# diku-kmc/kleenexlang

Hardware: AMD Instinct MI355X
Metric: input GB/s + % HBM-read roofline, apache_log.kex over 10 GiB synthetic log (higher is better)
Workload: dtype u8

## Files before the change

kleenexlang_amd/csrc/engine/kx_dfkernels.inc:

```

struct DfDev {
  const uint32_t* img; uint32_t words;
  uint32_t off_pool, deadh, esch, starth, K, C;
  const uint16_t* start_of_state;
  uint32_t orig_c4, hshift;
  uint32_t short_consts, debug;
  uint32_t nstates;
  uint32_t J;
  uint32_t wide;
  const uint4* sl_fmap;
  const uint32_t* sl_back; const uint8_t* sl_nleaves; const uint8_t* sl_fin_leaf; const uint8_t* sl_cls;
  const uint32_t* sl_pcoff; const uint8_t* sl_pcpool; const uint32_t* sl_pend; const uint32_t* sl_defoff; const uint32_t* sl_defpc; const uint16_t* sl_q;
  uint32_t sl_Lm, sl_npc, sl_on;
};
constexpr uint32_t DFREC_HOLE = 0xFFFF0000u, DF_HOLE_MAX = 4096, DF_HOLE_FIRST = 1024, DF_SL_LEAVES = 32;
struct __attribute__((aligned(16))) DfRec { uint32_t hh, cum, info, kc; };
constexpr uint32_t DFREC_OWN = 0x80000000u;

struct DfLds {
  const uint8_t* base; uint32_t csh;
  __device__ __forceinline__ uint32_t c8(uint32_t byte) const { return (uint32_t)base[byte] << csh; }
  __device__ __forceinline__ uint2 ent(uint32_t a) const { return *reinterpret_cast<const uint2*>(base + a); }
};
__device__ __forceinline__ DfLds df_stage(const DfDev& D, uint32_t* smem) {
  for (uint32_t i = threadIdx.x; i < D.words; i += blockDim.x) smem[i] = D.img[i];
  __syncthreads();
  return DfLds{reinterpret_cast<const uint8_t*>(smem), D.wide ? 3u : 0u};
}

__device__ __forceinline__ void df_run_piece(const uint32_t (&w)[16], uint32_t& h, uint32_t& mid, uint32_t& lenA, uint32_t& len, const DfLds& L) {
  uint32_t c[8], cn[8], sum = 0;
  static_for<0, 8>([&](auto ic) { constexpr int i = decltype(ic)::value; c[i] = L.c8(BYTE_AT_DEP(w, i, h)); });
  static_for<0, PIECE / 8>([&](auto gc) {
    constexpr int g = decltype(gc)::value;
    if constexpr (g + 1 < PIECE / 8)
      static_for<0, 8>([&](auto ic) { constexpr int i = decltype(ic)::value; cn[i] = L.c8(BYTE_AT_DEP(w, 8 * (g + 1) + i, h)); });
    static_for<0, 8>([&](auto ic) {
      constexpr int i = decltype(ic)::value;
      const uint2 e = L.ent(h + c[i]);
      h = e.x & 0xFFFFu; sum += e.y >> 24; tie(h, sum);
    });
    if constexpr (g == HALF / 8 - 1) { mid = h; lenA = sum; }
    if constexpr (g + 1 < PIECE / 8)
      static_for<0, 8>([&](auto ic) { constexpr int i = decltype(ic)::value; c[i] = cn[i]; });
  });
  len = sum;
}

__device__ __forceinline__ uint64_t df_own_start(uint32_t j, uint64_t n, uint64_t seg, int first_known, const uint64_t* __restrict__ seg_pos,
                                                 const uint16_t* __restrict__ seg_state, const DfDev& D) {
  if (j == 0 && first_known) return 0;
  const uint64_t p = seg_pos[j];
  if (p == UNSYNC) return UNSYNC;
  const uint32_t q = (((uint32_t)seg_state[j] << D.hshift) - OFF_FWD) / D.orig_c4;
  if (q >= D.nstates || D.start_of_state[q] == 0xFFFFu) return UNSYNC;
  const uint64_t b = (p + D.K + D.J + 63) & ~63ull;
  const uint64_t lim = ((uint64_t)j + 1) * seg < n ? ((uint64_t)j + 1) * seg : n;
  return b < lim ? b : UNSYNC;
}

struct DfSlowIO {
  const uint8_t* in; uint64_t n, a, end; uint32_t h0, last, is_last;
  uint32_t h_behind; uint32_t* side; uint32_t side_cap; Flags* flags; const uint8_t* lds; uint32_t clsh; uint8_t* lmap; uint32_t max_steps;
  uint32_t base, nd, h_next; uint64_t e_out;
};
__device__ __noinline__ int df_slow_resolve(DfSlowIO& io, const DfDev& D) {
  const uint8_t* __restrict__ in = io.in;
  const uint64_t n = io.n, a = io.a, end = io.end;
  const uint32_t h0 = io.h0;
  const bool last = io.last != 0, is_last = io.is_last != 0;
  uint32_t* side = io.side; const uint32_t side_cap = io.side_cap; Flags* flags = io.flags;
  if (!D.sl_on || !side) return 1;
  const uint32_t C = D.C, Lm = D.sl_Lm, K = D.K, NONE = D.sl_npc << 1;
  const uint32_t i0 = (h0 - 256u) / (C * 8u);
  uint32_t q = D.sl_q[i0];
  const uint32_t nd = D.sl_defoff[i0 + 1] - D.sl_defoff[i0];
  const uint64_t hard = a + io.max_steps < n ? a + io.max_steps : n;
  const uint32_t need = nd + K + (uint32_t)(hard - a) + 64u;
  const uint32_t base = atomicAdd(&flags->side_used, need);
  if ((uint64_t)base + need > side_cap) return 1;
  uint32_t* const E = side + base;
  uint32_t* const R = E + nd + K;
  for (uint32_t d = 0; d < nd; ++d) E[d] = 0x80000000u | (D.sl_defpc[D.sl_defoff[i0] + d] << 1);
  uint8_t *M = io.lmap, *M2 = io.lmap + 32;
  uint16_t qb[DF_HOLE_MAX / 64 + 2];
  uint32_t nl = D.sl_nleaves[q];
  for (uint32_t l = 0; l < DF_SL_LEAVES; ++l) M[l] = (uint8_t)l;
  uint64_t t = a, anchor = a, prev = a, inw = 0;
  auto back_to = [&](uint64_t from, uint64_t to, uint32_t leaf) {
    uint64_t u = to;
    while (u > from) {
      const uint32_t cnt = u - from < 8 ? (uint32_t)(u - from) : 8u;
      uint32_t rr[8];
#pragma unroll
      for (uint32_t k2 = 0; k2 < 8; ++k2) rr[k2] = k2 < cnt ? R[u - 1 - k2 - a] : 0u;
#pragma unroll
      for (uint32_t k2 = 0; k2 < 8; ++k2) if (k2 < cnt) {
        const uint32_t e = D.sl_back[(size_t)rr[k2] * Lm + leaf];
        R[u - 1 - k2 - a] = ((e >> 8) & 1u) | ((e >> 9) << 1);
        leaf = e & 0xFFu;
      }
      u -= cnt;
    }
    return leaf;
  };
  bool pend_done = false;
  auto anchor_known = [&](uint32_t leaf) {
    if (anchor == a) { for (uint32_t jj = 0; jj < K; ++jj) E[nd + jj] = D.sl_pend[((size_t)i0 * K + jj) * Lm + leaf]; pend_done = true; }
    else back_to(prev, anchor, leaf);
  };
  auto agree_at = [&](uint64_t tt, uint32_t nlv) -> bool {
    uint32_t l0 = 0, l1 = 0, l2 = 0, l3 = 0, nlive = 0;
    for (uint32_t l = 0; l < nlv; ++l) if (M[l] != 0xFFu) {
      if (nlive == 4) return false;
      if (nlive == 0) l0 = l1 = l2 = l3 = l; else if (nlive == 1) l1 = l; else if (nlive == 2) l2 = l; else l3 = l;
      ++nlive;
    }
    if (nlive == 0) return false;
    const uint32_t lv[1] = {l0};
    if (nlive > 1) {
      uint32_t cur[4] = {l0, l1, l2, l3};
      for (uint64_t u = tt; u-- > prev;) {
        const uint32_t* row = D.sl_back + (size_t)R[u - a] * Lm;
        const uint32_t e0 = row[cur[0]], e1 = row[cur[1]], e2 = row[cur[2]], e3 = row[cur[3]];
        if ((e0 >> 8) != (e1 >> 8) || (e0 >> 8) != (e2 >> 8) || (e0 >> 8) != (e3 >> 8)) return false;
        cur[0] = e0 & 0xFFu; cur[1] = e1 & 0xFFu; cur[2] = e2 & 0xFFu; cur[3] = e3 & 0xFFu;
      }
      if (!pend_done)
        for (uint32_t jj = 0; jj < K; ++jj) {
          const uint32_t* pr = D.sl_pend + ((size_t)i0 * K + jj) * Lm;
          if (pr[cur[0]] != pr[cur[1]] || pr[cur[0]] != pr[cur[2]] || pr[cur[0]] != pr[cur[3]]) return false;
        }
    }
    const uint32_t la = back_to(prev, tt, lv[0]);
    if (!pend_done) { for (uint32_t jj = 0; jj < K; ++jj) E[nd + jj] = D.sl_pend[((size_t)i0 * K + jj) * Lm + la]; pend_done = true; }
    return true;
  };
  uint64_t e_out = 0; int mode = 0;
  for (;;) {
    if (((t - a) & 63u) == 0) qb[(t - a) >> 6] = (uint16_t)q;
    if (t >= hard) {
      if (t != n) return 3;
      if (!is_last) return 1;
      if (D.sl_fin_leaf[q] == 0xFFu) { atomicMin(&flags->fail_pos, (unsigned long long)n); return 2; }
      const uint32_t fl = D.sl_fin_leaf[q];
      const uint32_t la = back_to(anchor, n, fl);
      anchor_known(la);
      if (last) { mode = 3; e_out = n; } else { mode = 2; e_out = end; }
      break;
    }
    if ((t & 7u) == 0 || t == a) {
      const uint64_t a8 = t & ~7ull;
      if (a8 + 8 <= n) { const uint2 w8 = *reinterpret_cast<const uint2*>(in + a8); inw = (uint64_t)w8.x | ((uint64_t)w8.y << 32); }
      else { inw = 0; for (uint64_t i = a8; i < n; ++i) inw |= (uint64_t)in[i] << (8 * (i - a8)); }
    }
    const uint32_t c = (uint32_t)io.lds[(uint32_t)(inw >> (8 * (t & 7u))) & 0xFFu] >> io.clsh;
    const uint4* fm = D.sl_fmap + ((size_t)q * C + c) * 3;
    const uint4 f0 = fm[0], f1 = fm[1], f2v = fm[2];
    const uint32_t nq = f0.x & 0xFFFFu;
    if (nq == 0xFFFFu) { atomicMin(&flags->fail_pos, (unsigned long long)t); return 2; }
    const uint32_t r = f0.y;
    R[t - a] = r;
    const uint32_t nnl = f0.x >> 16;
    uint32_t v = 0xFFu; bool same = true;
    const uint32_t par[8] = {f1.x, f1.y, f1.z, f1.w, f2v.x, f2v.y, f2v.z, f2v.w};
#pragma unroll
    for (uint32_t l = 0; l < DF_SL_LEAVES; ++l) {
      const uint32_t pl = (par[l >> 2] >> (8 * (l & 3u))) & 0xFFu;
      const uint32_t x = l >= nnl || pl == 0xFFu ? 0xFFu : M[pl];
      if (l < nnl) M2[l] = (uint8_t)x;
      if (x != 0xFFu) { if (v == 0xFFu) v = x; else same = same && x == v; }
    }
    { uint8_t* tmp = M; M = M2; M2 = tmp; }
    q = nq; nl = nnl; ++t;
    if ((!same || v == 0xFFu) && ((t - a) & 63u) == 0 && t + PIECE <= end && D.start_of_state[q] != 0xFFFFu && agree_at(t, nl)) {
      qb[(t - a) >> 6] = (uint16_t)q;
      mode = 1; e_out = t;
      break;
    }
    if (!same || v == 0xFFu) continue;
    anchor_known(v);
    const uint64_t decided = anchor;
    prev = anchor; anchor = t;
    for (uint32_t l = 0; l < DF_SL_LEAVES; ++l) M[l] = (uint8_t)l;
    const uint64_t e = decided & ~63ull;
    if (e > a && e + PIECE <= end && D.start_of_state[qb[(e - a) >> 6]] != 0xFFFFu) { mode = 1; e_out = e; break; }
    if (!last && decided + K >= end) { mode = 2; e_out = end; break; }
  }
  (void)nl;
  uint32_t h_next = h0;
  if (mode == 1) h_next = D.start_of_state[qb[(e_out - a) >> 6]];
  if (mode == 3) {
    if (D.start_of_state[q] == 0xFFFFu) return 1;
    h_next = D.start_of_state[q];
  }
  if (mode == 2) {
    for (uint64_t u = end - K; u < end; ++u) if (u >= a) R[u - a] = NONE; else E[nd + K - (a - u)] = NONE;
    const uint32_t ix = (io.h_behind - 256u) / (C * 8u);
    uint32_t due = D.sl_defoff[ix + 1] - D.sl_defoff[ix];
    for (uint32_t idx = nd + K + (uint32_t)(end - K - a); due && idx-- > 0;) {
      const uint32_t pc = (E[idx] >> 1) & 0x3FFFFFFFu;
      if (pc < D.sl_npc && D.sl_pcoff[pc + 1] > D.sl_pcoff[pc]) { E[idx] = (E[idx] & 0x80000001u) | NONE; --due; }
    }
    if (due) return 1;
  }
  io.base = base; io.nd = nd; io.h_next = h_next; io.e_out = e_out;
  return 0;
}

template <int BT, uint32_t DF_STAGE, int MINW, bool SLOW>
__global__ __launch_bounds__(BT, MINW) void k_dforward(const uint8_t* __restrict__ in, uint64_t n, uint64_t seg, uint32_t nseg, int first_known,
                           const uint64_t* __restrict__ seg_pos, const uint16_t* __restrict__ seg_state,
                           DfRec* __restrict__ rec, uint32_t* __restrict__ own, uint32_t* __restrict__ spill, Flags* flags,
                           uint32_t* __restrict__ side, uint32_t side_cap, int is_last, DfDev D) {
  extern __shared__ __attribute__((aligned(16))) uint32_t smem[];
  DfLds L = df_stage(D, smem);
  uint4* lrec = reinterpret_cast<uint4*>(smem + ((D.words + 3) & ~3u)) + (size_t)threadIdx.x * DF_STAGE;
  const uint32_t k = blockIdx.x * blockDim.x + threadIdx.x;
  const uint32_t lane = threadIdx.x & 63;
  const uint64_t B = k < nseg ? df_own_start(k, n, seg, first_known, seg_pos, seg_state, D) : UNSYNC;
  bool alive = B != UNSYNC;
  const uint32_t dead = D.deadh, esc = D.esch;
  auto warm = [&](uint32_t jj, uint64_t Bj) -> uint32_t {
    if (jj == 0 && first_known) return D.starth;
    uint32_t hw = D.start_of_state[(((uint32_t)seg_state[jj] << D.hshift) - OFF_FWD) / D.orig_c4];
    for (uint64_t pw = seg_pos[jj]; pw < Bj;) {
      const uint2 v = *reinterpret_cast<const uint2*>(in + (pw & ~7ull));
      const uint64_t x = (uint64_t)v.x | ((uint64_t)v.y << 32);
      for (uint32_t b = (uint32_t)pw & 7u; b < 8u && pw < Bj; ++b, ++pw) hw = L.ent(hw + L.c8((uint32_t)(x >> (8 * b)) & 0xFFu)).x & 0xFFFFu;
    }
    if (hw == esc && jj == k) atomicAdd(&flags->warm_esc, 1u);
    return hw == esc || hw == dead ? 0xFFFFFFFFu : hw;
  };
  uint32_t h = dead, h_behind = 0;
  if (alive) { h = warm(k, B); if (h == 0xFFFFFFFFu) { alive = false; h = dead; } }
  uint32_t j = k + 1;
  uint64_t end = n;
  if (alive) for (; j < nseg; ++j) {
    const uint64_t b = df_own_start(j, n, seg, first_known, seg_pos, seg_state, D);
    if (b == UNSYNC) continue;
    h_behind = warm(j, b);
    if (h_behind != 0xFFFFFFFFu) { end = b; break; }
  }
  const bool last = alive && j >= nseg;
  uint64_t pos = alive ? B : 0;
  if (alive) atomicMin(&flags->df_first_own, (unsigned long long)B);
  bool failed = !alive;
  if (!alive) { end = 0; pos = 0; }
  uint32_t m = (uint32_t)(pos / seg), cum = 0, flag = DFREC_OWN;
  uint64_t block_end = ((uint64_t)m + 1) * seg;
  auto fail_in = [&](uint32_t h0, uint64_t p0, uint32_t plen) -> int {
    uint32_t hh = h0;
    for (uint32_t t = 0; t < plen; ++t) {
      const uint32_t nh = L.ent(hh + L.c8(in[p0 + t])).x & 0xFFFFu;
      if (nh == dead) { atomicMin(&flags->fail_pos, (unsigned long long)(p0 + t)); failed = true; return 1; }
      if (nh == esc) return 2;
      hh = nh;
    }
    failed = true;
    return 1;
  };
  uint32_t nst = 0; uint64_t gfirst = 0;
  auto flush_group = [&]() {
    uint4* dst = reinterpret_cast<uint4*>(rec + gfirst);
    for (uint32_t i = 0; i < nst; ++i) dst[i] = lrec[(gfirst + i) & (DF_STAGE - 1)];
    nst = 0;
  };
  const bool coop = !(D.debug & 256u);
  bool in_trip = false;
  auto stage_rec = [&](uint64_t pc, uint4 r) {
    if (nst == 0) gfirst = pc;
    lrec[pc & (DF_STAGE - 1)] = r; ++nst;
    if (!in_trip && (pc & (DF_STAGE - 1)) == DF_STAGE - 1) flush_group();
  };
  uint4* const lrec_wave = reinterpret_cast<uint4*>(smem + ((D.words + 3) & ~3u)) + (size_t)(threadIdx.x & ~63u) * DF_STAGE;
  auto coop_flush = [&]() {
    const bool full = nst == DF_STAGE && (gfirst & (DF_STAGE - 1)) == 0;
    const uint32_t glo = (uint32_t)gfirst, ghi = (uint32_t)(gfirst >> 32) | (full ? 0u : 0x80000000u);
    const uint32_t team = lane / DF_STAGE * DF_STAGE, r = lane % DF_STAGE;
    static_for<0, (int)DF_STAGE>([&](auto ic) {
      constexpr uint32_t i = decltype(ic)::value;
      const uint32_t slo = (uint32_t)__shfl((int)glo, (int)(team + i)), shi = (uint32_t)__shfl((int)ghi, (int)(team + i));
      if (!(shi & 0x80000000u)) {
        const uint64_t g = ((uint64_t)shi << 32) | slo;
        reinterpret_cast<uint4*>(rec + g)[r] = lrec_wave[(size_t)(team + i) * DF_STAGE + r];
      }
    });
    if (full) nst = 0;
  };
  auto cross = [&]() { if (pos == block_end) { (flag ? own : spill)[m] = cum; cum = 0; flag = 0; ++m; block_end += seg; } };
  uint32_t kc_sum = 0, kc_max = 0, kc_n = 0;
  auto slow = [&](const uint64_t a, const uint32_t h0) -> int {
    flush_group();
    DfSlowIO io{in, n, a, end, h0, last ? 1u : 0u, (uint32_t)is_last, h_behind, side, side_cap, flags, L.base, D.wide ? 0u : 3u, reinterpret_cast<uint8_t*>(lrec), DF_HOLE_FIRST, 0, 0, 0, 0};
    {
      int rc = df_slow_resolve(io, D);
      if (rc == 3) { io.max_steps = DF_HOLE_MAX; rc = df_slow_resolve(io, D); }
      if (rc) return rc == 3 ? 1 : rc;
    }
    const uint32_t base = io.base, nd = io.nd, K = D.K;
    const uint64_t e_out = io.e_out;
    const uint32_t* const E = side + base;
    const uint64_t pend = (e_out + 63) & ~63ull;
    uint32_t idx = 0;
    for (uint64_t pp = a; pp < pend; pp += PIECE) {
      cross();
      const bool first = pp == a;
      const uint32_t steps = (uint32_t)((e_out - pp) < PIECE ? e_out - pp : PIECE);
      const uint32_t cnt = first ? nd + K + steps : steps;
      uint32_t len = 0;
      for (uint32_t x = 0; x < cnt; ++x) {
        const uint32_t ee = E[idx + x], pc = (ee >> 1) & 0x3FFFFFFFu;
        len += (ee & 1u) + (pc < D.sl_npc ? D.sl_pcoff[pc + 1] - D.sl_pcoff[pc] : 0u);
      }
      if (len > 0xFFFFu) return 1;
      rec[pp >> 6] = DfRec{base + idx, cum, len | flag, DFREC_HOLE | (first ? 0x8000u : 0u) | cnt};
      idx += cnt; cum += len; pos = pp + steps;
    }
    h = io.h_next;
    atomicAdd(&flags->slow_steps, (uint32_t)(e_out - a));
    return 0;
  };
  bool need_slow = false;
  auto run_slow = [&]() {
    need_slow = false;
    int r = 1;
    if constexpr (SLOW) r = slow(pos, h);
    if (r) { if (r == 1) atomicAdd(&flags->df_esc, 1u); failed = true; }
  };
  auto do_piece = [&](const uint32_t (&w)[16]) -> bool {
    cross();
    const uint32_t h0 = h;
    uint32_t mid, sumA, sum = 0;
    if (D.wide) piece_dfrun1w(w, h, mid, sumA, sum); else piece_dfrun1(w, h, mid, sumA, sum);
    if (h == dead || h == esc) {
      if (fail_in(h0, pos, PIECE) == 2) { need_slow = true; h = h0; }
      return false;
    }
    const uint32_t kA = (sumA & 0xFFu) >> 2, kB = (sum & 0xFFu) >> 2;
    kc_sum += kA + kB; kc_max = kA + kB > kc_max ? kA + kB : kc_max; ++kc_n;
    stage_rec(pos >> 6, make_uint4(h0 | (mid << 16), cum, (sumA >> 8) | flag, kA | (kB << 8)));
    cum += sum >> 8; pos += PIECE;
    return true;
  };
  auto single_piece = [&]() {
    uint32_t w[16];
    load_piece(in, n, pos, w);
    do_piece(w);
  };
  for (;;) {
  if (need_slow) run_slow();
  while (!failed && !need_slow && pos + PIECE <= end && (pos & (8 * PIECE - 1))) single_piece();
  for (;;) {
    const bool can = !failed && !need_slow && pos + 8 * PIECE <= end && !(pos & (8 * PIECE - 1));
    if (!__any(can) || __any(need_slow)) break;
    uint32_t line[8];
    {
      const uint32_t mine = can ? (uint32_t)(pos >> 7) : 0xFFFFFFFFu;
      static_for<0, 8>([&](auto ic) { constexpr int i = decltype(ic)::value; line[i] = __shfl(mine, (int)((lane & ~7u) + i)); });
    }
    auto issue = [&](uint32_t k2, uint4 (&dst)[8]) {
      static_for<0, 8>([&](auto ic) {
        constexpr int i = decltype(ic)::value;
        const uint64_t ln = line[i] != 0xFFFFFFFFu ? line[i] : 0u;
        dst[i] = *reinterpret_cast<const uint4*>(in + ((ln + k2) << 7) + (lane & 7u) * 16);
      });
    };
    uint4 v[8];
    issue(0, v);
    bool died = false;
    in_trip = coop;
#pragma nounroll
    for (uint32_t k2 = 0; k2 < 4; ++k2) {
      transpose8(v, lane);
      uint32_t wa[16], wb[16];
      static_for<0, 8>([&](auto ic) {
        constexpr int w = decltype(ic)::value;
        uint32_t (&dst)[16] = w < 4 ? wa : wb;
        dst[4 * (w & 3)] = v[w].x; dst[4 * (w & 3) + 1] = v[w].y; dst[4 * (w & 3) + 2] = v[w].z; dst[4 * (w & 3) + 3] = v[w].w;
      });
      bool go = can && !died;
      if (go && !do_piece(wa)) { died = true; go = false; }
      if (k2 < 3) issue(k2 + 1, v);
      if (go && !do_piece(wb)) died = true;
      if (coop && ((k2 + 1) * 2) % DF_STAGE == 0) coop_flush();
    }
    in_trip = false;
  }
  if (!__any(!failed && (need_slow || pos + 8 * PIECE <= end))) break;
  }
  if (!alive) return;
  for (;;) {
  if (need_slow) run_slow();
  while (!failed && !need_slow && pos + PIECE <= end) single_piece();
  if (need_slow) continue;
  if (!failed && pos < end) {
    cross();
    const uint32_t plen = (uint32_t)(end - pos), h0 = h;
    uint32_t mid = h, lenA = 0, len = 0, kA = 0, kc = 0;
    for (uint32_t t = 0; t < plen; ++t) {
      if (t == HALF) { mid = h; lenA = len; kA = kc; }
      const uint2 e = L.ent(h + L.c8(in[pos + t]));
      h = e.x & 0xFFFFu; len += e.y >> 24; kc += (e.y >> 23) & 1u;
    }
    if (plen <= HALF) { mid = h; lenA = len; kA = kc; }
    if (h == dead || h == esc) {
      if (fail_in(h0, pos, plen) == 2) { h = h0; need_slow = true; continue; }
    }
    else { stage_rec(pos >> 6, make_uint4(h0 | (mid << 16), cum, lenA | flag, kA | ((kc - kA) << 8))); cum += len; pos = end; }
  }
  break;
  }
  flush_group();
  if (failed) return;
  (flag ? own : spill)[m] = cum;
  if (last) flags->end_state = h;
  if (kc_n) { if ((k & 15u) == 0) { atomicAdd(&flags->emit_ksum, kc_sum); atomicAdd(&flags->emit_kn, kc_n); } atomicMax(&flags->emit_kmax, kc_max); }
}

__global__ void k_dhead(const uint8_t* __restrict__ in, uint64_t n, uint64_t seg, uint64_t head_len, uint32_t h,
                        DfRec* __restrict__ rec, uint32_t* __restrict__ own, uint32_t* __restrict__ spill, Flags* flags, DfDev D) {
  extern __shared__ __attribute__((aligned(16))) uint32_t smem[];
  DfLds L = df_stage(D, smem);
  if (blockIdx.x || threadIdx.x) return;
  const uint32_t dead = D.deadh, esc = D.esch;
  uint32_t m = 0, cum = 0;
  uint64_t block_end = seg;
  for (uint64_t pos = 0; pos < head_len;) {
    if (pos == block_end) { spill[m] = cum; cum = 0; ++m; block_end += seg; }
    const uint32_t plen = (uint32_t)(head_len - pos < PIECE ? head_len - pos : PIECE);
    const uint32_t h0 = h;
    uint32_t mid = h, lenA = 0, len = 0, kA = 0, kc = 0;
    for (uint32_t t = 0; t < plen; ++t) {
      if (t == HALF) { mid = h; lenA = len; kA = kc; }
      const uint2 e = L.ent(h + L.c8(in[pos + t]));
      const uint32_t nh = e.x & 0xFFFFu;
      if (nh == dead) { atomicMin(&flags->fail_pos, (unsigned long long)(pos + t)); return; }
      if (nh == esc) { flags->df_esc = 1; return; }
      h = nh; len += e.y >> 24; kc += (e.y >> 23) & 1u;
    }
    if (plen <= HALF) { mid = h; lenA = len; kA = kc; }
    if (kc > 0) atomicMax(&flags->emit_kmax, kc);
    rec[pos >> 6] = DfRec{h0 | (mid << 16), cum, lenA, kA | ((kc - kA) << 8)};
    cum += len; pos += plen;
  }
  spill[m] = cum;
  if (head_len == n) flags->end_state = h;
}

__global__ void k_dlen(uint32_t nblk, const uint32_t* __restrict__ own, const uint32_t* __restrict__ spill, uint32_t* __restrict__ len,
                       unsigned long long* __restrict__ wsum) {
  __shared__ unsigned long long red[1024];
  const uint32_t m = blockIdx.x * blockDim.x + threadIdx.x;
  uint32_t mylen = 0;
  if (m < nblk) { mylen = own[m] + spill[m]; len[m] = mylen; }
  red[threadIdx.x] = mylen;
  __syncthreads();
  for (uint32_t s = blockDim.x >> 1; s > 0; s >>= 1) {
    if (threadIdx.x < s) red[threadIdx.x] += red[threadIdx.x + s];
    __syncthreads();
  }
  if (threadIdx.x == 0) wsum[blockIdx.x] = red[0];
}

template <bool GENERAL>
__global__ void k_dmap(const uint8_t* __restrict__ in, uint64_t n, uint32_t q_in, uint64_t cap, uint8_t* __restrict__ map_out,
                       uint32_t* __restrict__ status, DevTables T) {
  extern __shared__ __attribute__((aligned(16))) uint32_t smem[];
  Lds L = stage_tables<GENERAL>(T, smem);
  if (blockIdx.x || threadIdx.x) return;
  __shared__ uint8_t M[2][256];
  const uint32_t C = T.nclasses;
  uint32_t h = (OFF_FWD + q_in * C * 4) >> T.hshift, cur = 0;
  uint32_t nl = T.nleaves[q_in];
  for (uint32_t l = 0; l < nl; ++l) M[0][l] = (uint8_t)l;
  uint64_t pos = 0;
  bool constant = nl == 1, dead = false;
  while (pos < n && pos < cap && !constant && !dead) {
    const uint64_t a8 = pos & ~7ull;
    uint64_t x = 0;
    if (a8 + 8 <= n) { const uint2 v = *reinterpret_cast<const uint2*>(in + a8); x = (uint64_t)v.x | ((uint64_t)v.y << 32); }
    else for (uint64_t i = a8; i < n; ++i) x |= (uint64_t)in[i] << (8 * (i - a8));
    for (uint32_t b = (uint32_t)pos & 7u; b < 8u && pos < n && pos < cap && !constant; ++b, ++pos) {
      const uint32_t e = L.next(h, (uint32_t)(x >> (8 * b)) & 0xFFu);
      const uint32_t nh = e & 0xFFFFu;
      if (nh == T.deadh) { dead = true; break; }
      const uint32_t row = L.ra(e >> 16);
      const uint32_t nq = ((nh << T.hshift) - OFF_FWD) / (C * 4);
      const uint32_t nnl = T.nleaves[nq];
      constant = true;
      for (uint32_t l = 0; l < nnl; ++l) {
        const uint32_t p = (L.w(row + l * 4) >> 2) & 0xFFu;
        M[cur ^ 1][l] = M[cur][p < nl ? p : 0];
        constant = constant && M[cur ^ 1][l] == M[cur ^ 1][0];
      }
      cur ^= 1; h = nh; nl = nnl;
    }
  }
  for (uint32_t l = 0; l < 256; ++l) map_out[l] = constant ? M[cur][0] : l < nl ? M[cur][l] : 0;
  *status = constant ? 1u : pos >= n ? 2u : 0u;
}

template <int S>
__device__ __forceinline__ uint32_t df_byte_src(const uint32_t (&w)[16], uint32_t wp) {
  if constexpr (S >= 0) return w[S >> 2] >> ((S & 3) * 8);
  else return wp >> ((4 + S) * 8);
}

__device__ __forceinline__ void put_bytes3(uint32_t r, uint32_t d, uint32_t v) {
  uint32_t t; unsigned long long sv;
  asm volatile("s_mov_b64 %[sv], exec\n"
               "v_cmpx_lt_u32_e32 vcc, 0, %[r]\n"
               "ds_write_b8 %[d], %[v]\n"
               "v_cmpx_lt_u32_e32 vcc, 1, %[r]\n"
               "v_lshrrev_b32 %[t], 8, %[v]\n"
               "ds_write_b8 %[d], %[t] offset:1\n"
               "v_cmpx_lt_u32_e32 vcc, 2, %[r]\n"
               "ds_write_b8_d16_hi %[d], %[v] offset:2\n"
               "s_mov_b64 exec, %[sv]\n"
               : [t] "=&v"(t), [sv] "=&s"(sv) : [r] "v"(r), [d] "v"(d), [v] "v"(v) : "vcc", "memory");
}
__device__ __forceinline__ void put_dwords4(uint32_t m, uint32_t d, const uint32_t (&w)[4]) {
  unsigned long long sv;
  asm volatile("s_mov_b64 %[sv], exec\n"
               "v_cmpx_lt_u32_e32 vcc, 0, %[m]\n"
               "ds_write_b32 %[d], %[w0]\n"
               "v_cmpx_lt_u32_e32 vcc, 1, %[m]\n"
               "ds_write_b32 %[d], %[w1] offset:4\n"
               "v_cmpx_lt_u32_e32 vcc, 2, %[m]\n"
               "ds_write_b32 %[d], %[w2] offset:8\n"
               "v_cmpx_lt_u32_e32 vcc, 3, %[m]\n"
               "ds_write_b32 %[d], %[w3] offset:12\n"
               "s_mov_b64 exec, %[sv]\n"
               : [sv] "=&s"(sv) : [m] "v"(m), [d] "v"(d), [w0] "v"(w[0]), [w1] "v"(w[1]), [w2] "v"(w[2]), [w3] "v"(w[3]) : "vcc", "memory");
}

#ifndef KX_PRIO_CONSTANTS
#define KX_PRIO_CONSTANTS 2
#endif
#ifndef KX_PRIO_FLUSH
#define KX_PRIO_FLUSH 1
#endif
constexpr int HALF_BYTES = HALF;

template <int CONSTS>
__device__ __forceinline__ void df_step_gen(uint32_t& h, uint32_t byte_now, uint32_t byte_out, uint64_t& o, uint8_t* __restrict__ dst,
                                            const DfLds& L, const DfDev& D) {
  const uint2 e = L.ent(h + L.c8(byte_now));
  h = e.x & 0xFFFFu;
  const uint32_t cp = E_COPY(e.y), dl = e.y >> 24;
  if (cp) dst[o] = (uint8_t)byte_out;
  if (dl > cp) { const uint32_t src = D.off_pool + (E_AID(e.y) << 4); for (uint32_t i = 0; i < dl - cp; ++i) dst[o + cp + i] = L.base[src + i]; }
  o += dl;
}

template <int WAVES, int K, bool HALF = false>
__global__ __launch_bounds__(WAVES * 64) void k_demit(const uint8_t* __restrict__ in, uint64_t n, uint64_t blk, uint64_t blk_inv,
                                                      uint64_t npieces_total, const DfRec* __restrict__ rec,
                                                      const uint32_t* __restrict__ spill, const unsigned long long* __restrict__ off,
                                                      Flags* __restrict__ flags, uint32_t stgb, uint32_t jbytes, uint32_t maxcnt,
                                                      uint8_t* __restrict__ out, const uint32_t* __restrict__ side, DfDev D) {
  extern __shared__ __attribute__((aligned(16))) uint32_t smem[];
  DfLds L = df_stage(D, smem);
  if ((uint32_t)(uintptr_t)smem != 0u) __builtin_trap();
  constexpr int NB = HALF ? HALF_BYTES : PIECE, NW = NB / 4;
  const uint32_t wave = threadIdx.x >> 6, lane = threadIdx.x & 63;
  const uint32_t stga = ((D.words + 3) & ~3u) * 4 + wave * (stgb + 16 + jbytes);
  uint8_t* stg = (uint8_t*)smem + stga;
  const uint32_t jarea = stga + stgb + 16;
  const uint64_t nunits = HALF ? npieces_total * 2 : npieces_total;
  const uint64_t nwi = (nunits + 63) / 64;
  const uint64_t oend_all = flags->total_len;
  const uint64_t one_piece_blocks = (uint64_t)__builtin_amdgcn_readfirstlane(blk == (uint64_t)PIECE ? 1 : 0);
  struct Operands { uint32_t w[NW]; uint32_t wp; uint4 r; uint64_t off0; uint32_t sp0; uint4 r1; uint64_t off1; uint32_t sp1; };
  auto request = [&](uint64_t it_, Operands& o) {
    if (it_ >= nwi) return;
    const uint64_t u = it_ * 64 + lane;
    const bool ok = u < nunits;
    const uint64_t pc = HALF ? u >> 1 : u;
    const uint64_t ustart = ok ? (HALF ? pc * PIECE + (u & 1) * HALF_BYTES : pc * PIECE) : n;
    if constexpr (HALF) {
      if (ustart + HALF_BYTES <= n) {
        const uint4* p = reinterpret_cast<const uint4*>(in + ustart);
        const uint4 v0 = p[0], v1 = p[1];
        o.w[0] = v0.x; o.w[1] = v0.y; o.w[2] = v0.z; o.w[3] = v0.w; o.w[4] = v1.x; o.w[5] = v1.y; o.w[6] = v1.z; o.w[7] = v1.w;
      } else {
#pragma unroll
        for (int i = 0; i < NW; ++i) {
          uint32_t x = 0;
#pragma unroll
          for (int bb = 0; bb < 4; ++bb) { const uint64_t a = ustart + 4 * i + bb; if (a < n) x |= (uint32_t)in[a] << (8 * bb); }
          o.w[i] = x;
        }
      }
    } else load_piece(in, n, ustart, o.w);
    o.wp = *reinterpret_cast<const uint32_t*>(ok && ustart >= 4 ? in + ustart - 4 : reinterpret_cast<const uint8_t*>(D.img));
    const uint64_t pc0 = ok ? pc : 0;
    const uint64_t m0 = __umul64hi(pc0, blk_inv) + pc0 * one_piece_blocks;
    o.r = *reinterpret_cast<const uint4*>(rec + pc0);
    o.off0 = off[m0]; o.sp0 = spill[m0];
    {
      const uint64_t pc1 = pc0 + 1 < npieces_total ? pc0 + 1 : pc0, m1 = __umul64hi(pc1, blk_inv) + pc1 * one_piece_blocks;
      o.r1 = *reinterpret_cast<const uint4*>(rec + pc1); o.off1 = off[m1]; o.sp1 = spill[m1];
    }
  };
  Operands nx, cur;
  request((uint64_t)blockIdx.x * WAVES + wave, nx);
  cur = nx;
  unsigned long long tk[6] = {0, 0, 0, 0, 0, 0};
  auto stamp = [&]() -> unsigned long long {
    if (!(D.debug & 64u)) return 0ull;
    asm volatile("s_waitcnt vmcnt(0) lgkmcnt(0)" ::: "memory");
    return __builtin_amdgcn_s_memtime();
  };
  for (uint64_t it = (uint64_t)blockIdx.x * WAVES + wave; it < nwi; it += (uint64_t)gridDim.x * WAVES) {
    const unsigned long long t0 = stamp();
    const uint64_t unit = it * 64 + lane;
    const bool valid = unit < nunits;
    const uint64_t piece = HALF ? unit >> 1 : unit;
    const uint32_t half = HALF ? (uint32_t)unit & 1u : 0u;
    const uint64_t ustart = piece * PIECE + half * HALF_BYTES;
    const int plen = valid ? (int)(n <= ustart ? 0 : n - ustart < (uint64_t)NB ? n - ustart : NB) : 0;
    uint32_t w[NW];
#pragma unroll
    for (int i = 0; i < NW; ++i) w[i] = cur.w[i];
    const uint32_t wp = cur.wp, lenA = cur.r.z & 0xFFFFu;
    const uint32_t kA = HALF ? (half ? (cur.r.w >> 8) & 0xFFu : cur.r.w & 0xFFu) : cur.r.w & 0xFFu, kB = HALF ? 0u : (cur.r.w >> 8) & 0xFFu;
    const uint32_t hh = HALF ? (half ? cur.r.x >> 16 : cur.r.x & 0xFFFFu) : cur.r.x;
    uint64_t ostart = valid ? cur.off0 + cur.r.y + ((cur.r.z & DFREC_OWN) ? cur.sp0 : 0u) + (half ? lenA : 0u) : oend_all;
    const uint64_t onext63 = piece + 1 < npieces_total ? cur.off1 + cur.r1.y + ((cur.r1.z & DFREC_OWN) ? cur.sp1 : 0u) : oend_all;
    uint64_t oend;
    {
      const uint32_t lo = (uint32_t)__builtin_amdgcn_update_dpp(0, (int)(uint32_t)ostart, 0x130, 0xF, 0xF, false);
      const uint32_t hi = (uint32_t)__builtin_amdgcn_update_dpp(0, (int)(uint32_t)(ostart >> 32), 0x130, 0xF, 0xF, false);
      oend = lane == 63 ? onext63 : ((uint64_t)hi << 32) | lo;
      if (!valid) oend = oend_all;
    }
    const unsigned long long vmask = __ballot(valid);
    const uint32_t nvalid = (uint32_t)__popcll(vmask);
    uint32_t first = 0;
    bool taken = false;
    unsigned long long t2 = stamp();
    tk[0] += t2 - t0;
    if (valid && (cur.r.w & DFREC_HOLE) == DFREC_HOLE && half == 0) {
      const uint32_t cntE = cur.r.w & 0x7FFFu;
      uint64_t u = (cur.r.w & 0x8000u) ? piece * PIECE - K : piece * PIECE, o = ostart;
      for (uint32_t x = 0; x < cntE; ++x) {
        const uint32_t ee = side[cur.r.x + x], pc = (ee >> 1) & 0x3FFFFFFFu;
        if (ee & 1u) out[o++] = in[u];
        if (pc < D.sl_npc) for (uint32_t b = D.sl_pcoff[pc]; b < D.sl_pcoff[pc + 1]; ++b) out[o++] = D.sl_pcpool[b];
        if (!(ee >> 31)) ++u;
      }
    }
    while (first < nvalid) {
      if (first == 0) request(it + (uint64_t)gridDim.x * WAVES, nx);
      const uint64_t gs = wave_read64(ostart, first);
      const uint64_t abase = gs & ~15ull;
      const bool hole = (cur.r.w & DFREC_HOLE) == DFREC_HOLE;
      const bool fits = valid && lane >= first && (oend - abase) <= (uint64_t)stgb && plen == NB && !hole;
      const unsigned long long fm = __ballot(fits) >> first;
      uint32_t cnt = fm == ~0ull ? 64u - first : (uint32_t)__builtin_ctzll(~fm);
      if (cnt > maxcnt) cnt = maxcnt;
      if (cnt == 0) {
        if (lane == first && hole) {
        } else
        if (lane == first) {
          uint32_t h = hh & 0xFFFFu;
          uint64_t o = ostart;
          for (int t = 0; t < plen; ++t) {
            const int ts = t - K;
            const uint32_t bn = (w[t >> 2] >> ((t & 3) * 8)) & 0xFFu;
            const uint32_t bo_ = ts >= 0 ? (w[ts >> 2] >> ((ts & 3) * 8)) & 0xFFu : (wp >> ((4 + ts) * 8)) & 0xFFu;
            df_step_gen<0>(h, bn, bo_, o, out, L, D);
          }
        }
        first += 1;
        continue;
      }
      const uint32_t lastl = first + cnt - 1;
      const bool active = lane >= first && lane <= lastl;
      const uint32_t o0 = stga + (uint32_t)(ostart - abase);
      const bool inplace = jbytes == 0;
      const uint32_t need = active ? (kA + kB) * 4u : 0u;
      const uint32_t incl = wave_scan_incl(need);
      const uint32_t jtotal = (uint32_t)__builtin_amdgcn_readlane((int)incl, 63);
      const bool jfit = !inplace && jtotal <= jbytes;
      const unsigned long long t3 = stamp();
      tk[2] += t3 - t2;
      if (active && jfit) {
        uint32_t oA = o0, pA = jarea + incl - need;
        if constexpr (HALF) {
          if (D.wide) { if constexpr (K == 1) piece_dfwalk1cw_k1(w, wp, hh & 0xFFFFu, oA, pA); else piece_dfwalk1cw_k2(w, wp, hh & 0xFFFFu, oA, pA); }
          else { if constexpr (K == 1) piece_dfwalk1c_k1(w, wp, hh & 0xFFFFu, oA, pA); else piece_dfwalk1c_k2(w, wp, hh & 0xFFFFu, oA, pA); }
        } else {
          uint32_t oB = o0 + lenA, pB = pA + 4u * kA;
          if (D.wide) {
            if constexpr (K == 1) piece_dfwalk2cw_k1(w, wp, hh & 0xFFFFu, oA, hh >> 16, oB, pA, pB);
            else piece_dfwalk2cw_k2(w, wp, hh & 0xFFFFu, oA, hh >> 16, oB, pA, pB);
          } else {
            if constexpr (K == 1) piece_dfwalk2c_k1(w, wp, hh & 0xFFFFu, oA, hh >> 16, oB, pA, pB);
            else piece_dfwalk2c_k2(w, wp, hh & 0xFFFFu, oA, hh >> 16, oB, pA, pB);
          }
        }
      }
      uint32_t njobs = jfit ? jtotal >> 2 : 0u;
      if (!jfit) {
        if (!inplace && lane == first) atomicAdd(&flags->emit_ovf, cnt);
        if (active) {
          for (int ch = 0; ch < (HALF ? 1 : 2); ++ch) {
            uint32_t h = ch ? hh >> 16 : hh & 0xFFFFu;
            uint64_t o = (uint64_t)(o0 - stga) + (ch ? lenA : 0u);
            for (int t = ch * HALF_BYTES; t < (ch + 1) * HALF_BYTES; ++t) {
              const int ts = t - K;
              const uint32_t bn = (w[t >> 2] >> ((t & 3) * 8)) & 0xFFu;
              const uint32_t bo_ = ts >= 0 ? (w[ts >> 2] >> ((ts & 3) * 8)) & 0xFFu : (wp >> ((4 + ts) * 8)) & 0xFFu;
              df_step_gen<1>(h, bn, bo_, o, stg, L, D);
            }
          }
        }
      }
      wave_lds_fence();
      const unsigned long long t4 = stamp();
      tk[3] += t4 - t3;
      __builtin_amdgcn_s_setprio(KX_PRIO_CONSTANTS);
      for (uint32_t j0 = 0; j0 < njobs; j0 += 64) {
        const uint32_t j = j0 + lane;
        uint32_t l = 0, d = 0, off0 = 0;
        if (j < njobs) {
          const uint32_t jw = *reinterpret_cast<const uint32_t*>((const uint8_t*)smem + jarea + 4 * j);
          const uint32_t e = *reinterpret_cast<const uint32_t*>(L.base + (jw & 0xFFFFu) + 4);
          const uint32_t cp = E_COPY(e);
          l = (e >> 24) - cp;
          d = stga + (((jw >> 16) - stga) & 0xFFFFu) + cp;
          off0 = D.off_pool + (E_AID(e) << 4);
        }
        const uint32_t tob = (0u - d) & 3u, nh = l < tob ? l : tob, rem = l - nh;
        const uint32_t src = off0 + nh * ((l + 15u) & ~15u), d1 = d + nh;
        const uint32_t v0 = *reinterpret_cast<const uint32_t*>(L.base + off0);
        uint4 wv = *reinterpret_cast<const uint4*>(L.base + src);
        put_bytes3(nh, d, v0);
        for (uint32_t base = 0;; base += 16) {
          const uint32_t left = rem > base ? rem - base : 0u, m = left >> 2 < 4u ? left >> 2 : 4u;
          const uint32_t w4[4] = {wv.x, wv.y, wv.z, wv.w};
          put_dwords4(m, d1 + base, w4);
          const uint32_t nt = left < 16u ? left & 3u : 0u;
          const uint32_t tw = m == 0 ? wv.x : m == 1 ? wv.y : m == 2 ? wv.z : wv.w;
          put_bytes3(nt, d1 + base + 4u * m, tw);
          if (!__any(rem > base + 16u)) break;
          wv = *reinterpret_cast<const uint4*>(L.base + src + base + 16u);
        }
      }
      wave_lds_fence();
      __builtin_amdgcn_s_setprio(KX_PRIO_FLUSH);
      const unsigned long long t5 = stamp();
      tk[4] += t5 - t4;
      if (lastl + 1 >= nvalid) { cur = nx; taken = true; }
      const uint64_t ge = wave_read64(oend, lastl);
      const uint64_t fs = (gs + 15) & ~15ull, fe = ge & ~15ull;
      if (fs >= fe) {
        for (uint64_t x = gs + lane; x < ge; x += 64) out[x] = stg[x - abase];
      } else {
        if (gs + lane < fs) out[gs + lane] = stg[gs + lane - abase];
        if (fe + lane < ge) out[fe + lane] = stg[fe + lane - abase];
        for (uint64_t x = fs + (uint64_t)lane * 16; x < fe; x += 1024)
          *reinterpret_cast<uint4*>(out + x) = *reinterpret_cast<const uint4*>(stg + (x - abase));
      }
      wave_lds_fence();
      __builtin_amdgcn_s_setprio(0);
      t2 = stamp();
      tk[5] += t2 - t5;
      first = lastl + 1;
    }
    if (!taken) cur = nx;
  }
  if ((D.debug & 64u) && lane == 0)
    for (int i = 0; i < 6; ++i) atomicAdd(&flags->dbg[i], tk[i]);
}
```

kleenexlang_amd/csrc/engine/kx_engine.hip:

```cpp
#include <hip/hip_runtime.h>
#include <fcntl.h>
#include <sys/stat.h>
#include <unistd.h>

#include <cerrno>
#include <condition_variable>
#include <cstdint>
#include <algorithm>
#include <deque>
#include <mutex>
#include <chrono>
#include <thread>
#include <cstdio>
#include <cstdlib>
#include <cstring>
#include <string>
#include <type_traits>
#include <vector>

#include "../../../include/kxhip.h"
#include "../../../include/kxp_format.h"
#include "kx_delayed.h"

namespace {
// ... 1528 lines not shown
                             uint8_t* __restrict__ out) {
  const unsigned long long o = offs[blockIdx.x], len = offs[blockIdx.x + 1] - o;
  const uint8_t* src = tmp + chunks[blockIdx.x].start;
  for (unsigned long long i = threadIdx.x; i < len; i += blockDim.x) out[o + i] = src[i];
}

__global__ void k_copy_bytes(uint8_t* __restrict__ d, const uint8_t* __restrict__ s, unsigned long long n) {
  const unsigned long long tid = (unsigned long long)blockIdx.x * blockDim.x + threadIdx.x, nt = (unsigned long long)gridDim.x * blockDim.x;
  if ((((uintptr_t)d | (uintptr_t)s) & 15u) == 0) {
    const unsigned long long n16 = n >> 4;
    for (unsigned long long i = tid; i < n16; i += nt) reinterpret_cast<uint4*>(d)[i] = reinterpret_cast<const uint4*>(s)[i];
    for (unsigned long long i = (n16 << 4) + tid; i < n; i += nt) d[i] = s[i];
  } else for (unsigned long long i = tid; i < n; i += nt) d[i] = s[i];
}

#include "kx_batch.inc"
#include "kx_batch_actions.inc"
#include "kx_records.inc"
#include "kx_records_quoted.inc"
#include "kx_records_escaped.inc"
#include "kx_records_rs.inc"
#include "kx_fields.inc"
#include "kx_field_list.inc"

struct Stage {
  uint32_t nstates = 0, nclasses = 0, q0 = 0, maxleaves = 1;
  std::vector<uint8_t> h_nleaves, h_fin_leaf;
  std::vector<uint32_t> h_init_off, h_init_len;
  std::vector<uint8_t> h_pool;
  void* d_all = nullptr;
  DevTables T{};
  size_t lds_bytes = 0;
  size_t sync_lds_bytes = 0;
  uint32_t emit_nup = 1;
  uint32_t max_const_len = 0;
  bool general = false;
  bool big = false;
  uint32_t handleOf(uint32_t state) const { return (OFF_FWD + state * nclasses * 4) >> (big ? 2 : 0); }
  uint32_t stateOf(uint32_t handle) const { return ((handle << (big ? 2 : 0)) - OFF_FWD) / (nclasses * 4); }
  bool act = false; uint32_t act_regs = 0;
  void* d_all_alt = nullptr; DevTables Talt{}; bool has_alt = false; int use_alt = 0;
  kxdf::DfBuild df; DfDev D{}; void* d_df = nullptr; void* d_slow = nullptr; bool has_df = false;
  uint32_t df_streak = 0, df_skip = 0;
  bool df_slow_armed = false;
  bool df_given_up = false;
  std::vector<uint32_t> df_pc_off, df_pc_len;
  std::string df_why;
};

struct Arena {
  char* base = nullptr; size_t cap = 0, used = 0;
  int reserve(size_t bytes) {
    if (bytes <= cap) return 0;
    if (base) (void)hipFree(base);
    base = nullptr; cap = 0;
    size_t want = bytes + bytes / 8 + (1 << 20);
    HIPCHECK(hipMalloc((void**)&base, want));
    cap = want;
    return 0;
  }
  void reset() { used = 0; }
  template <typename Ty> Ty* take(size_t count) {
    used = (used + 255) & ~(size_t)255;
    Ty* p = reinterpret_cast<Ty*>(base + used);
    used += count * sizeof(Ty);
    return p;
  }
};

}

struct ActionRunner {
  const kx_config* cfg = nullptr;
  ActState* d_st = nullptr; uint8_t *scratch = nullptr, *heap = nullptr;
  size_t scap = 0, hcap = 0, live = 0; uint32_t nregs = 0;
  ~ActionRunner() { if (d_st) (void)hipFree(d_st); if (scratch) (void)hipFree(scratch); if (heap) (void)hipFree(heap); freeBufs(); }
  int reset() {
    HIPCHECK(hipMemset(d_st, 0, sizeof(ActState)));
    const unsigned long long caps[2] = {scap, hcap};
    HIPCHECK(hipMemcpy(&d_st->scratch_cap, &caps[0], 8, hipMemcpyHostToDevice));
    HIPCHECK(hipMemcpy(&d_st->heap_cap, &caps[1], 8, hipMemcpyHostToDevice));
    live = 0;
    return 0;
  }
  int init(uint32_t regs) {
    nregs = regs; scap = hcap = (size_t)1 << 20;
    HIPCHECK(hipMalloc((void**)&d_st, sizeof(ActState)));
    HIPCHECK(hipMemset(d_st, 0, sizeof(ActState)));
    HIPCHECK(hipMalloc((void**)&scratch, scap)); HIPCHECK(hipMalloc((void**)&heap, hcap));
    const unsigned long long caps[2] = {scap, hcap};
    HIPCHECK(hipMemcpy(&d_st->scratch_cap, &caps[0], 8, hipMemcpyHostToDevice));
    HIPCHECK(hipMemcpy(&d_st->heap_cap, &caps[1], 8, hipMemcpyHostToDevice));
    return 0;
  }
  size_t slack() const { return live + 16; }
  static int grow(uint8_t*& buf, size_t& cap, size_t used, size_t want) {
    size_t nc = cap * 2 > want ? cap * 2 : want;
    uint8_t* nb = nullptr;
    HIPCHECK(hipMalloc((void**)&nb, nc));
    if (used) HIPCHECK(hipMemcpy(nb, buf, used, hipMemcpyDeviceToDevice));
    (void)hipFree(buf);
    buf = nb; cap = nc;
    return 0;
  }
  struct DBuf { void* p = nullptr; size_t cap = 0; };
  DBuf b_summ, b_pre, b_cuts, b_chunks, b_states, b_offs, b_tmp, b_pscr, b_pheap, b_flag, b_lres, b_gpart, b_gpre;
  static int ensureBuf(DBuf& b, size_t bytes) {
    if (b.cap >= bytes) return 0;
    if (b.p) (void)hipFree(b.p);
    b.p = nullptr; b.cap = 0;
    HIPCHECK(hipMalloc(&b.p, bytes + bytes / 8 + 4096));
    b.cap = bytes + bytes / 8 + 4096;
    return 0;
  }
  void freeBufs() { for (int k = 0; k < 2; ++k) if (h_pin[k]) (void)hipHostFree(h_pin[k]); for (DBuf* b : {&b_summ, &b_pre, &b_cuts, &b_chunks, &b_states, &b_offs, &b_tmp, &b_pscr, &b_pheap, &b_flag, &b_lres, &b_gpart, &b_gpre}) if (b->p) (void)hipFree(b->p); }
  void* h_pin[2] = {nullptr, nullptr}; size_t h_pin_cap[2] = {0, 0};
  int ensurePin(int k, size_t bytes) {
    if (h_pin_cap[k] >= bytes) return 0;
    if (h_pin[k]) (void)hipHostFree(h_pin[k]);
    h_pin[k] = nullptr; h_pin_cap[k] = 0;
    HIPCHECK(hipHostMalloc(&h_pin[k], bytes + bytes / 4 + 4096, hipHostMallocDefault));
    h_pin_cap[k] = bytes + bytes / 4 + 4096;
    return 0;
  }
  uint32_t par_chunks = 0;
  bool no_lanes = false;

  int run(const uint8_t* d_in, size_t n, uint8_t* d_out, size_t* out_len, hipStream_t stream) {
    par_chunks = 0;
    static const kx_config defaults{};
    const kx_config& C = cfg ? *cfg : defaults;
    const size_t par_min = C.act_par_min ? (size_t)C.act_par_min : ((size_t)1 << 20);
    if (n < par_min || n < 4 * (size_t)ACT_BLK || nregs > 32 || (C.force & KX_FORCE_ACT_SEQ)) return run_seq(d_in, n, d_out, out_len, stream);
    ActState h;
    HIPCHECK(hipMemcpyAsync(&h, d_st, sizeof(ActState), hipMemcpyDeviceToHost, stream));
    HIPCHECK(hipStreamSynchronize(stream));
    if (h.carry_n) return run_seq(d_in, n, d_out, out_len, stream);
    unsigned long long mask0 = 0;
    for (uint32_t r = 0; r < 256; ++r) if (h.reg[r].len) { if (r >= 64) return run_seq(d_in, n, d_out, out_len, stream); mask0 |= 1ull << r; }
    const bool dbg = getenv("KX_DEBUG") != nullptr;
    auto tick = [&]() { if (dbg) (void)hipStreamSynchronize(stream); return std::chrono::steady_clock::now(); };
    auto msSince = [](std::chrono::steady_clock::time_point a, std::chrono::steady_clock::time_point b) { return std::chrono::duration<double, std::milli>(b - a).count(); };
    const auto t_begin = tick();
    const uint32_t nblk = (uint32_t)((n + ACT_BLK - 1) / ACT_BLK);
    int rc = ensureBuf(b_summ, (size_t)nblk * sizeof(ActSumm)); if (rc) return rc;
    rc = ensureBuf(b_pre, (size_t)nblk * sizeof(ActSumm)); if (rc) return rc;
    rc = ensureBuf(b_flag, 16); if (rc) return rc;
    HIPCHECK(hipMemsetAsync(b_flag.p, 0, 16, stream));
    hipLaunchKernelGGL(k_act_summary, dim3((nblk + 255) / 256), dim3(256), 0, stream, d_in, (unsigned long long)n, nblk, (ActSumm*)b_summ.p,
                       (unsigned long long*)b_flag.p + 1);
    if (nblk >= (C.act_prefix3_min ? C.act_prefix3_min : 65536u)) {
      const uint32_t ng = (nblk + 63) / 64;
      rc = ensureBuf(b_gpart, (size_t)ng * sizeof(ActSumm)); if (rc) return rc;
      rc = ensureBuf(b_gpre, (size_t)ng * sizeof(ActSumm)); if (rc) return rc;
      hipLaunchKernelGGL(k_act_wave_reduce, dim3(ng), dim3(64), 0, stream, nblk, (const ActSumm*)b_summ.p, (ActSumm*)b_gpart.p);
      hipLaunchKernelGGL(k_act_prefix, dim3(1), dim3(1024), 0, stream, ng, (const ActSumm*)b_gpart.p, (int32_t)h.depth, mask0, (ActSumm*)b_gpre.p);
      hipLaunchKernelGGL(k_act_wave_scan, dim3(ng), dim3(64), 0, stream, nblk, (const ActSumm*)b_summ.p, (const ActSumm*)b_gpre.p, (ActSumm*)b_pre.p);
    } else
    hipLaunchKernelGGL(k_act_prefix, dim3(1), dim3(1024), 0, stream, nblk, (const ActSumm*)b_summ.p, (int32_t)h.depth, mask0, (ActSumm*)b_pre.p);
    unsigned long long ntok_sample = 0;
    HIPCHECK(hipMemcpyAsync(&ntok_sample, (unsigned long long*)b_flag.p + 1, 8, hipMemcpyDeviceToHost, stream));
    HIPCHECK(hipStreamSynchronize(stream));
    const auto t_summ = tick();
    const double bytes_per_token = ntok_sample ? (double)((nblk + 63) / 64) * ACT_BLK / (double)ntok_sample : 1e9;
    const bool lanes = !no_lanes && nregs <= LANE_REGS && (C.act_lanes ? C.act_lanes == 2 : bytes_per_token < 24.0);
    size_t want = C.act_chunk ? (size_t)C.act_chunk : (lanes ? 2048 : 4096);
    const size_t slots = lanes ? (size_t)8192 * 64 : 8192;
    if (want < (n + slots - 1) / slots) want = (n + slots - 1) / slots;
    want = (want + ACT_BLK - 1) / ACT_BLK * ACT_BLK;
    rc = ensurePin(0, (n / want + 4) * 8); if (rc) return rc;
    unsigned long long* cuts = (unsigned long long*)h_pin[0];
    uint32_t ncut = 0;
    cuts[ncut++] = ACT_BLK;
    for (unsigned long long t = want; t + ACT_BLK < n; t += want) cuts[ncut++] = t;
    if (n > 6 * (size_t)ACT_BLK && cuts[ncut - 1] < n - 4 * ACT_BLK) cuts[ncut++] = n - 4 * ACT_BLK;
    if (ncut < 3) return run_seq(d_in, n, d_out, out_len, stream);
    rc = ensureBuf(b_cuts, (size_t)ncut * 8); if (rc) return rc;
    HIPCHECK(hipMemcpyAsync(b_cuts.p, cuts, (size_t)ncut * 8, hipMemcpyHostToDevice, stream));
    const auto t_up = tick();
    hipLaunchKernelGGL(k_act_cuts, dim3((ncut + 63) / 64), dim3(64), 0, stream, d_in, (unsigned long long)n, nblk, (const ActSumm*)b_pre.p,
                       ncut, 16u, (unsigned long long*)b_cuts.p);
    HIPCHECK(hipGetLastError());
    HIPCHECK(hipMemcpyAsync(cuts, b_cuts.p, (size_t)ncut * 8, hipMemcpyDeviceToHost, stream));
    HIPCHECK(hipStreamSynchronize(stream));
    std::vector<unsigned long long> bnd{0};
    for (uint32_t i = 0; i < ncut; ++i) { const unsigned long long c = cuts[i]; if (c != ~0ull && c > bnd.back() && c < n) bnd.push_back(c); }
    bnd.push_back(n);
    const size_t K = bnd.size() - 1;
    if (K < 3) return run_seq(d_in, n, d_out, out_len, stream);
    const auto t_cuts = tick();
    size_t ol0 = 0;
    rc = run_seq(d_in, (size_t)bnd[1], d_out, &ol0, stream);
    if (rc) return rc;
    const auto t_first = tick();
    const uint32_t M = (uint32_t)(K - 2);
    rc = ensurePin(1, (size_t)M * sizeof(ActChunk)); if (rc) return rc;
    ActChunk* ch = (ActChunk*)h_pin[1];
    for (uint32_t i = 0; i < M; ++i) ch[i] = ActChunk{bnd[i + 1], bnd[i + 2] - bnd[i + 1]};
    rc = ensureBuf(b_chunks, (size_t)M * sizeof(ActChunk)); if (rc) return rc;
    rc = ensureBuf(lanes ? b_lres : b_states, (size_t)M * (lanes ? sizeof(ActLaneOut) : sizeof(ActState))); if (rc) return rc;
    rc = ensureBuf(b_offs, ((size_t)M + 1) * 8); if (rc) return rc;
    rc = ensureBuf(b_tmp, n); if (rc) return rc;
    rc = ensureBuf(b_pscr, n + 64 * (size_t)M + 64); if (rc) return rc;
    rc = ensureBuf(b_pheap, 2 * n + 1024 * (size_t)M + 1024); if (rc) return rc;
    HIPCHECK(hipMemcpyAsync(b_chunks.p, ch, (size_t)M * sizeof(ActChunk), hipMemcpyHostToDevice, stream));
    HIPCHECK(hipMemsetAsync(b_flag.p, 0, 4, stream));
    if (lanes) {
      hipLaunchKernelGGL(k_actions_lanes, dim3((M + 63) / 64), dim3(64), 0, stream, d_in, M, (const ActChunk*)b_chunks.p, (uint8_t*)b_pscr.p,
                         (uint8_t*)b_pheap.p, (uint8_t*)b_tmp.p, nregs, (ActLaneOut*)b_lres.p, (uint32_t*)b_flag.p);
      hipLaunchKernelGGL(k_act_lane_offsets, dim3(1), dim3(1024), 0, stream, M, (const ActLaneOut*)b_lres.p, (unsigned long long*)b_offs.p);
    } else {
      HIPCHECK(hipMemsetAsync(b_states.p, 0, (size_t)M * sizeof(ActState), stream));
      hipLaunchKernelGGL(k_act_init, dim3((M + 255) / 256), dim3(256), 0, stream, M, (const ActChunk*)b_chunks.p, (ActState*)b_states.p);
      hipLaunchKernelGGL(k_actions_chunks, dim3(M), dim3(64), 0, stream, d_in, (const ActChunk*)b_chunks.p, (ActState*)b_states.p,
                         (uint8_t*)b_pscr.p, (uint8_t*)b_pheap.p, (uint8_t*)b_tmp.p, nregs, (uint32_t*)b_flag.p);
      hipLaunchKernelGGL(k_act_offsets, dim3(1), dim3(64), 0, stream, M, (const ActState*)b_states.p, (unsigned long long*)b_offs.p);
    }
    HIPCHECK(hipGetLastError());
    uint32_t bad = 0; unsigned long long mid = 0;
    HIPCHECK(hipMemcpyAsync(&bad, b_flag.p, 4, hipMemcpyDeviceToHost, stream));
    HIPCHECK(hipMemcpyAsync(&mid, (unsigned long long*)b_offs.p + M, 8, hipMemcpyDeviceToHost, stream));
    HIPCHECK(hipStreamSynchronize(stream));
    if (bad) {
      size_t rest = 0;
      if (lanes) { no_lanes = true; rc = run(d_in + bnd[1], n - (size_t)bnd[1], d_out + ol0, &rest, stream); no_lanes = false; }
      else rc = run_seq(d_in + bnd[1], n - (size_t)bnd[1], d_out + ol0, &rest, stream);
      *out_len = ol0 + rest;
      return rc;
    }
    const auto t_chunks = tick();
    hipLaunchKernelGGL(k_act_gather, dim3(M), dim3(lanes ? 64 : 256), 0, stream, (const ActChunk*)b_chunks.p, (const unsigned long long*)b_offs.p,
                       (const uint8_t*)b_tmp.p, d_out + ol0);
    HIPCHECK(hipGetLastError());
    const auto t_gather = tick();
    size_t olt = 0;
    rc = run_seq(d_in + bnd[K - 1], n - (size_t)bnd[K - 1], d_out + ol0 + (size_t)mid, &olt, stream);
    *out_len = ol0 + (size_t)mid + olt;
    par_chunks = M;
    if (dbg) {
      const auto t_end = tick();
      fprintf(stderr, "[kx] actions: %u chunks of about %zu bytes in parallel (one %s each, %.1f bytes per token), %zu + %zu bytes on the stream's own state; ms: summaries %.2f, wanted cuts up %.2f, cuts %.2f, first %.2f, chunks %.2f, gather %.2f, last %.2f\n",
              M, want, lanes ? "lane" : "wave", bytes_per_token, (size_t)bnd[1], n - (size_t)bnd[K - 1], msSince(t_begin, t_summ), msSince(t_summ, t_up), msSince(t_up, t_cuts), msSince(t_cuts, t_first), msSince(t_first, t_chunks), msSince(t_chunks, t_gather), msSince(t_gather, t_end));
    }
    return rc;
  }

  int run_seq(const uint8_t* d_in, size_t n, uint8_t* d_out, size_t* out_len, hipStream_t stream) {
    size_t pos = 0, olen = 0;
    for (;;) {
      hipLaunchKernelGGL(k_actions, dim3(1), dim3(64), 0, stream, d_in + pos, (unsigned long long)(n - pos), d_st, scratch, heap, d_out + olen, nregs);
      HIPCHECK(hipGetLastError());
      ActState h;
      HIPCHECK(hipMemcpyAsync(&h, d_st, offsetof(ActState, frame_start), hipMemcpyDeviceToHost, stream));
      HIPCHECK(hipStreamSynchronize(stream));
      pos += h.consumed; olen += h.out_len;
      live = h.scratch_len + h.heap_len;
      if (h.status == 0) break;
      if (h.status == 3) return setErr(KX_E_ARG, "register redirections nested deeper than 64");
      if (h.status == 1) {
        int rc = grow(scratch, scap, h.scratch_len, h.scratch_len + (n - pos) + h.heap_len + 4096);
        if (rc) return rc;
        const unsigned long long c = scap;
        HIPCHECK(hipMemcpy(&d_st->scratch_cap, &c, 8, hipMemcpyHostToDevice));
      } else {
        int rc = grow(heap, hcap, h.heap_len, h.heap_len * 2 + 2 * h.scratch_len + 4096);
        if (rc) return rc;
        const unsigned long long c = hcap;
        HIPCHECK(hipMemcpy(&d_st->heap_cap, &c, 8, hipMemcpyHostToDevice));
      }
    }
    *out_len = olen;
    return 0;
  }
};

struct kx_program {
  std::vector<Stage> stages;
  void* actbuf[2][2] = {{nullptr, nullptr}, {nullptr, nullptr}};
  size_t actcap[2][2] = {{0, 0}, {0, 0}};
  kx_config cfg = [] { kx_config c{}; c.block_threads = 512; return c; }();
  std::vector<Arena*> arenas;
  void* stagebuf[2] = {nullptr, nullptr};
  size_t stagecap[2] = {0, 0};
  hipEvent_t ev[KX_NKERNELS + 1] = {};
  bool have_events = false;
  int ncu = 256;
  std::vector<ActionRunner*> act_runners;
  BatchWs* batch = nullptr;
  FieldWs* fields = nullptr;
  FieldListWs* field_list = nullptr;
};

struct kx_shard {
  kx_program* prog; Stage* st; uint32_t stage; Arena* arena = nullptr;
  const DevTables* T = nullptr;
  const uint8_t* in; uint64_t n; int is_first, is_last; hipStream_t stream;
  uint64_t seg; uint32_t nseg, nblk, Lc, ngroups;
  uint64_t* seg_pos; uint16_t* seg_state; uint16_t* chk; Flags* flags;
  uint8_t *bs_start, *bs_merged, *bs_mstart, *E, *d_map; uint32_t *bs_len, *len, *d_const, *ctot;
  PieceRec* prec; uint16_t* merge_piece;
  unsigned long long *off, *wsum, *woff;
  Flags hflags{}; uint64_t head_len = 0; bool have_end = false; uint64_t out_len = 0; uint32_t init_shift = 0, init_leaf = 0;
  uint32_t df_qin = 0;
  bool df = false; DfRec* dfrec = nullptr; uint32_t *df_own = nullptr, *df_spill = nullptr, *side = nullptr; uint32_t side_cap = 0; std::vector<uint8_t> df_tail; uint64_t df_body = 0;
  uint32_t endId() const {
    if (!df) return st->stateOf(hflags.end_state);
    const uint32_t i = st->df.indexOf(hflags.end_state);
    return i < st->df.states.size() ? st->df.states[i].q : st->q0;
  }
  kx_stats stats{};
};

namespace {

size_t pad4(size_t x) { return (x + 3) & ~(size_t)3; }

thread_local int g_force_jl = -1;

int parseStage(const uint8_t*& c, const uint8_t* end, Stage& S, const kx_config& cfg, bool dry = false) {
  if (end < c || (size_t)(end - c) < 64) return setErr(KX_E_BLOB, "truncated stage header");
  uint32_t h[16];
  memcpy(h, c, 64); c += 64;
  if (h[0] != KXP_STAGE_MAGIC) return setErr(KX_E_BLOB, "bad stage magic");
  const uint32_t nstates = h[1], C = h[2], q0 = h[3], nactions = h[5], nops = h[6], nconsts = h[7], cpl = h[8];
  const uint32_t Lm = h[9], nback = h[10], npc = h[11], pcpl = h[12], nsync = h[13];
  const size_t sc = (size_t)nstates * C;
  {
    const unsigned long long need = 256ull + pad4(sc * 2) + sc * 4 + (unsigned long long)nstates * 4 + ((unsigned long long)nactions + 1) * 4 +
                                    (unsigned long long)nops * 8 + ((unsigned long long)nconsts + 1) * 4 + pad4(cpl) + sc * 4 + 2 * pad4(nstates) +
                                    (unsigned long long)nback * Lm * 4 + ((unsigned long long)npc + 1) * 4 + pad4(pcpl) + (unsigned long long)Lm * 4 +
                                    (unsigned long long)nsync * C * 4 + (unsigned long long)nsync * 4;
    if (nstates > 0xFFFFu || C > 256 || Lm > 256 || need > (unsigned long long)(end - c)) return setErr(KX_E_BLOB, "truncated stage body");
  }
  const uint8_t* cls = c; c += 256;
  const uint16_t* delta = (const uint16_t*)c; c += pad4(sc * 2);
  c += sc * 4;
  c += (size_t)nstates * 4;
  c += ((size_t)nactions + 1) * 4;
  c += (size_t)nops * 8;
  c += ((size_t)nconsts + 1) * 4; c += pad4(cpl);
  const uint32_t* pback = (const uint32_t*)c; c += sc * 4;
  const uint8_t* nleaves = c; c += pad4(nstates);
  const uint8_t* fin_leaf = c; c += pad4(nstates);
  const uint32_t* back = (const uint32_t*)c; c += (size_t)nback * Lm * 4;
  const uint32_t* pcoff = (const uint32_t*)c; c += ((size_t)npc + 1) * 4;
  const uint8_t* pcpool = c; c += pad4(pcpl);
  const uint32_t* init_const = (const uint32_t*)c; c += (size_t)Lm * 4;
  const uint32_t* sync_next = (const uint32_t*)c; c += (size_t)nsync * C * 4;
  const uint32_t* sync_state = (const uint32_t*)c; c += (size_t)nsync * 4;
  if (c > end) return setErr(KX_E_BLOB, "truncated stage body");
  const bool has_tbl = (h[15] & KXP_STAGE_HAS_TABLES) != 0;
  uint32_t ntables = 0; const uint8_t* tables = nullptr;
  if (has_tbl) {
    if ((size_t)(end - c) < 4) return setErr(KX_E_BLOB, "truncated symbol tables");
    memcpy(&ntables, c, 4); c += 4;
    if (ntables == 0 || ntables > KXP_MAX_TABLES || (size_t)(end - c) < (size_t)ntables * 256) return setErr(KX_E_BLOB, "truncated symbol tables");
    tables = c; c += (size_t)ntables * 256;
  }
  auto pcOf = [&](uint32_t e) { return has_tbl ? (e >> 9) & 0x7FFFu : e >> 9; };
  auto tbOf = [&](uint32_t e) { return has_tbl ? e >> 24 : 0u; };
  if (q0 >= nstates) return setErr(KX_E_BLOB, "start state out of range");
  for (size_t i = 0; i < sc; ++i) {
    if (delta[i] != KXP_NO_STATE && delta[i] >= nstates) return setErr(KX_E_BLOB, "transition target out of range");
    if (delta[i] != KXP_NO_STATE && pback[i] >= nback) return setErr(KX_E_BLOB, "backward row out of range");
  }
  for (uint32_t i = 0; i <= npc; ++i) if (pcoff[i] > pcpl || (i && pcoff[i] < pcoff[i - 1])) return setErr(KX_E_BLOB, "path constant pool offsets out of order");
  for (size_t i = 0; i < (size_t)nback * Lm; ++i) if (back[i] != KXP_DEAD_LEAF && (pcOf(back[i]) >= npc || (back[i] & 0xFF) >= Lm || tbOf(back[i]) > ntables || (tbOf(back[i]) && !((back[i] >> 8) & 1)))) return setErr(KX_E_BLOB, "backward entry out of range");
  for (uint32_t j = 0; j < Lm; ++j) if (init_const[j] >= npc) return setErr(KX_E_BLOB, "initial constant out of range");
  for (uint32_t q = 0; q < nstates; ++q)
    if (nleaves[q] == 0 || nleaves[q] > Lm || (fin_leaf[q] != KXP_NO_LEAF && fin_leaf[q] >= nleaves[q])) return setErr(KX_E_BLOB, "leaf count out of range");
  for (int b = 0; b < 256; ++b) if (cls[b] >= C) return setErr(KX_E_BLOB, "byte class out of range");
  for (size_t i = 0; i < (size_t)nsync * C; ++i) if (sync_next[i] != KXP_SYNC_UNKNOWN && sync_next[i] >= nsync) return setErr(KX_E_BLOB, "synchronising automaton target out of range");
  for (uint32_t i = 0; i < nsync; ++i) if (sync_state[i] < KXP_SYNC_UNKNOWN && sync_state[i] >= nstates) return setErr(KX_E_BLOB, "synchronising automaton state out of range");
  if (nstates == 0 || C == 0 || Lm == 0 || Lm > 254 || (size_t)(nstates + 1) * C * 4 + OFF_FWD > 0x3FFF0)
    return setErr(KX_E_BLOB, "program outside engine limits (states x classes > 256 KiB, or more than 254 leaves)");

  S.nstates = nstates; S.nclasses = C; S.q0 = q0; S.maxleaves = Lm;
  S.act = (h[15] & 1u) != 0; S.act_regs = h[15] >> 8;
  uint32_t xlat_tb = 0; bool tblmode = false;
  if (has_tbl) {
    bool any = false, plain = false, several = false;
    for (size_t i = 0; i < (size_t)nback * Lm; ++i) {
      if (back[i] == KXP_DEAD_LEAF || !((back[i] >> 8) & 1)) continue;
      const uint32_t tb = tbOf(back[i]);
      if (!tb) plain = true;
      else { if (any && tb != xlat_tb) several = true; any = true; xlat_tb = tb; }
    }
    tblmode = any && (plain || several || (cfg.force & KX_FORCE_TBLMODE));
    if (!any || tblmode) xlat_tb = 0;
    if (tblmode) {
      uint32_t top = 0;
      for (size_t i = 0; i < (size_t)nback * Lm; ++i) if (back[i] != KXP_DEAD_LEAF && tbOf(back[i]) > top) top = tbOf(back[i]);
      if (top > 7) return setErr(KX_E_BLOB, "program outside engine limits (more than 7 symbol tables beside plain copies)");
      S.general = true;
    }
  }
  if (S.act && S.act_regs > KXP_MAX_ACTION_REGS) return setErr(KX_E_BLOB, "too many action registers");
  if (S.act && has_tbl) return setErr(KX_E_BLOB, "symbol tables in a stage with register actions (a table could write the escape byte)");
  std::vector<uint32_t> apoff(npc + 1, 0);
  std::vector<uint8_t> apool;
  for (uint32_t pc = 0; pc < npc; ++pc) {
    apoff[pc] = (uint32_t)apool.size();
    apool.insert(apool.end(), pcpool + pcoff[pc], pcpool + pcoff[pc + 1]);
    apool.resize((apool.size() + 15) & ~(size_t)15, 0);
  }
  apoff[npc] = (uint32_t)apool.size();
  apool.resize(apool.size() + 16, 0);
  {
    kxdf::DfInput di{nstates, C, q0, Lm, nback, npc, cls, delta, pback, nleaves, back, pcoff, pcpool, init_const, apoff.data(), apool.data(), (uint32_t)apool.size(), has_tbl};
    S.has_df = false;
    auto acceptable = [&](const kxdf::DfBuild& b) { return (uint64_t)b.nesc_start * 4 <= (uint64_t)b.ntrans_start || cfg.delayed_form == 2; };
    if (cfg.delayed_form == 1) S.df_why = "switched off (kx_config::delayed_form = 1)";
    else if (nstates > 0 && C > 0 && Lm > 0 && Lm <= 254) {
      const uint32_t k0 = cfg.delay;
      auto build = [&](uint32_t K, kxdf::DfBuild& b) {
        std::string w = "-";
        if (cfg.merge_window) { const uint32_t J = cfg.merge_window - 1; if (J) w = kxdf::buildDelayed(di, K, J, 40 * 1024, b); }
        else
          for (uint32_t J : {8u, 6u, 4u, 3u, 2u, 1u}) {
            b = kxdf::DfBuild();
            w = kxdf::buildDelayed(di, K, J, 40 * 1024, b);
            if (w.empty() && !b.capped && b.img.size() * 4 + 64 * 1024 <= 80 * 1024) break;
            w = "-";
          }
        if (!w.empty() || b.capped) { b = kxdf::DfBuild(); w = kxdf::buildDelayed(di, K, 0, 40 * 1024, b); }
        return w;
      };
      if (k0 == 1 || k0 == 2) S.df_why = build(k0, S.df);
      else {
        kxdf::DfBuild b1, b2;
        const std::string w1 = build(1, b1);
        if (w1.empty() && b1.nesc_start == 0) { S.df = std::move(b1); S.df_why = w1; }
        else {
          const std::string w2 = build(2, b2);
          if (w2.empty() && (acceptable(b2) || !w1.empty() || !acceptable(b1))) { S.df = std::move(b2); S.df_why = w2; }
          else { S.df = std::move(b1); S.df_why = w1; }
        }
      }
      if (S.df_why.empty() && !acceptable(S.df)) S.df_why = "too many contexts that need more lookahead";
      S.has_df = S.df_why.empty();
    }
    S.df_pc_off.assign(apoff.begin(), apoff.begin() + npc); S.df_pc_len.resize(npc);
    for (uint32_t pc = 0; pc < npc; ++pc) S.df_pc_len[pc] = pcoff[pc + 1] - pcoff[pc];
  }
  std::vector<uint32_t> aid_of(npc, 0), adesc(2, 0);
  std::vector<uint32_t> rowoff(nback), ent, wlen;
  bool too_many_actions = false;
  bool inl = false;
  {
    size_t one = 0, longer = 0; bool anywide = false;
    for (size_t i = 0; i < (size_t)nback * Lm; ++i) {
      if (back[i] == KXP_DEAD_LEAF) continue;
      const uint32_t cl = pcoff[pcOf(back[i]) + 1] - pcoff[pcOf(back[i])];
      if (cl == 1) ++one; else if (cl > 1) ++longer;
      anywide = anywide || cl + ((back[i] >> 8) & 1) >= 127;
    }
    inl = (cfg.inline_consts ? cfg.inline_consts == 2 : one > 0 && one >= longer) && !tblmode && !anywide && C <= 64 && Lm <= 64 && !(cfg.force & KX_FORCE_BIG);
  }
  bool jl = false;
  {
    bool anywide = false;
    for (size_t i = 0; i < (size_t)nback * Lm; ++i)
      if (back[i] != KXP_DEAD_LEAF) anywide = anywide || pcoff[pcOf(back[i]) + 1] - pcoff[pcOf(back[i])] + ((back[i] >> 8) & 1) >= 127;
    jl = (g_force_jl >= 0 ? g_force_jl != 0 : cfg.job_stride == 2) && !inl && !tblmode && !xlat_tb && !anywide && C <= 64 && Lm <= 64 && apoff[npc] <= 64 * 16 && !(cfg.force & KX_FORCE_BIG);
  }
  bool direct = false;
  {
    bool anywide = false;
    for (size_t i = 0; i < (size_t)nback * Lm; ++i)
      if (back[i] != KXP_DEAD_LEAF) anywide = anywide || pcoff[pcOf(back[i]) + 1] - pcoff[pcOf(back[i])] + ((back[i] >> 8) & 1) >= 127;
    direct = !inl && !jl && !tblmode && !xlat_tb && !anywide && C <= 64 && apoff[npc] < (1u << 17) && !(cfg.disable & KX_OFF_DIRECT);
  }
  auto pushEnt = [&](uint32_t parent, uint32_t copy, uint32_t dlen, uint32_t pc, uint32_t tb = 0) {
    if (jl) {
      if (dlen - copy > S.max_const_len) S.max_const_len = dlen - copy;
      ent.push_back((copy ? 0u : 1u) | (parent << 2) | (dlen > copy ? ((apoff[pc] >> 4) << 10) | (4u << 16) : 0u) | (dlen << 24));
      wlen.push_back(dlen);
      return;
    }
    if (inl) {
      if (dlen == copy + 1) { ent.push_back((copy ? 0u : 1u) | (parent << 2) | ((uint32_t)pcpool[pcoff[pc]] << 16) | (dlen << 24)); wlen.push_back(dlen); return; }
      uint32_t aid = 0;
      if (dlen > copy) {
        if (!aid_of[pc]) { aid_of[pc] = (uint32_t)adesc.size() / 2; adesc.push_back(apoff[pc]); adesc.push_back(dlen - copy); }
        aid = aid_of[pc];
        if (aid >= (1u << 12)) too_many_actions = true;
      }
      if (dlen - copy > S.max_const_len) S.max_const_len = dlen - copy;
      ent.push_back((copy ? 0u : 1u) | (parent << 2) | 0x8000u | ((aid & 0x1Fu) << 10) | (((aid >> 5) & 0x7Fu) << 16) | (dlen > copy ? 1u << 23 : 0u) | (dlen << 24));
      wlen.push_back(dlen);
      return;
    }
    const bool wide = dlen >= 127;
    if (wide) S.general = true;
    if (dlen - copy > S.max_const_len) S.max_const_len = dlen - copy;
    uint32_t aid = 0;
    if (dlen > copy) {
      if (!aid_of[pc]) { aid_of[pc] = (uint32_t)adesc.size() / 2; adesc.push_back(apoff[pc]); adesc.push_back(dlen - copy); }
      aid = direct ? apoff[pc] >> 4 : aid_of[pc];
      if (aid >= (tblmode ? 1u << 10 : 1u << 13)) too_many_actions = true;
    }
    ent.push_back((copy ? 0u : 1u) | (parent << 2) | ((aid & 0x1FFFu) << 10) | (tblmode ? (tb & 7u) << 20 : 0u) | (dlen > copy ? 1u << 23 : 0u) | ((wide ? 127u : dlen) << 24));
    wlen.push_back(dlen);
  };
  const uint32_t off_fwd = OFF_FWD, fwd_bytes = (nstates + 1) * C * 4;
  const uint32_t off_ent = off_fwd + fwd_bytes;
  size_t ent_words = 2 * (size_t)Lm, pool_bytes = apool.size(), nconst_used = 0;
  for (uint32_t b = 0; b < nback; ++b) {
    uint32_t rl = 1;
    for (uint32_t j = 0; j < Lm; ++j) if (back[(size_t)b * Lm + j] != KXP_DEAD_LEAF) rl = j + 1;
    ent_words += rl;
  }
  nconst_used = npc;
  const bool big = (cfg.force & KX_FORCE_BIG) != 0  || (size_t)off_ent + ent_words * 4 > 65532 || (size_t)off_ent + ent_words * 4 + pool_bytes + 8 * (nconst_used + 1) + 64 + (size_t)ntables * 256 > 150 * 1024;
  if (big) { S.general = true; inl = false; }
  if (big || S.general) { jl = false; direct = false; }
  S.big = big;
  const uint32_t rpad = big ? 4u : 1u;
  for (uint32_t b = 0; b < nback; ++b) {
    uint32_t rl = 1;
    for (uint32_t j = 0; j < Lm; ++j) if (back[(size_t)b * Lm + j] != KXP_DEAD_LEAF) rl = j + 1;
    while (ent.size() % rpad) pushEnt(0, 0, 0, 0);
    rowoff[b] = (uint32_t)ent.size();
    for (uint32_t j = 0; j < rl; ++j) {
      uint32_t e = back[(size_t)b * Lm + j];
      if (e == KXP_DEAD_LEAF) { pushEnt(0, 0, 0, 0); continue; }
      uint32_t parent = e & 0xFF, copy = (e >> 8) & 1, pc = pcOf(e);
      uint32_t clen = pcoff[pc + 1] - pcoff[pc];
      if (clen + copy >= (1u << 23)) return setErr(KX_E_BLOB, "path constant too long");
      pushEnt(parent, copy, clen + copy, pc, tbOf(e));
    }
  }
  if (too_many_actions) return setErr(KX_E_BLOB, inl ? "internal: inline-constant layout with more than 4095 longer constants (KX_INL=0 loads the program)" : tblmode ? "program outside engine limits (more than 1023 distinct path constants beside symbol tables)" : "program has more than 8191 distinct path constants");
  for (uint32_t b = 0; b < nback; ++b) {
    const uint32_t rl = (b + 1 < nback ? rowoff[b + 1] : (uint32_t)ent.size()) - rowoff[b];
    for (uint32_t j = 0; j < rl && j < Lm; ++j) {
      uint32_t& e = ent[rowoff[b] + j];
      if (back[(size_t)b * Lm + j] == KXP_DEAD_LEAF) continue;
      const uint32_t pl = (e >> 2) & 0xFFu;
      if (pl >= rl || pl >= Lm || back[(size_t)b * Lm + pl] == KXP_DEAD_LEAF) continue;
      const uint32_t ep = ent[rowoff[b] + pl];
      if (!inl && ((ep >> 2) & 0xFFu) == pl && (ep & 1u) == 0 && ((ep >> (jl ? 18 : 23)) & 1u) == 0 && (ep >> 24) == 1u) e |= 2u;
    }
  }
  while (ent.size() % rpad) pushEnt(0, 0, 0, 0);
  const uint32_t nullrow_idx = (uint32_t)ent.size();
  for (uint32_t j = 0; j < Lm; ++j) pushEnt(j, 0, 0, 0);
  for (uint32_t j = 0; j < Lm; ++j) pushEnt(0, 0, 0, 0);
  if (!big && (size_t)off_ent + ent.size() * 4 > 65532) return setErr(KX_E_BLOB, "internal: table sizing");
  if (big && ent.size() * 4 > 0xFFFF0u)
    return setErr(KX_E_BLOB, "program outside engine limits (path table > 1 MiB)");
  const uint32_t hshift = big ? 2u : 0u, rshift = big ? 4u : 0u, rbase = big ? off_ent : 0u;
  const uint32_t deadh = (off_fwd + nstates * C * 4) >> hshift;
  auto rowHandle = [&](uint32_t row_word) { return big ? (row_word * 4) >> 4 : off_ent + row_word * 4; };
  const uint32_t cshift = C <= 64 ? 0u : 2u;
  if (cshift) S.general = true;
  std::vector<uint32_t> packed(OFF_FWD / 4 + (size_t)(nstates + 1) * C);
  for (int b = 0; b < 256; ++b) ((uint8_t*)packed.data())[b] = (uint8_t)(cshift ? cls[b] : cls[b] * 4);
  {
    uint32_t* fwd = packed.data() + OFF_FWD / 4;
    for (uint32_t q = 0; q < nstates; ++q)
      for (uint32_t k = 0; k < C; ++k) {
        uint16_t d = delta[(size_t)q * C + k];
        fwd[(size_t)q * C + k] = d == KXP_NO_STATE ? deadh
                                 : (((off_fwd + (uint32_t)d * C * 4) >> hshift) | (rowHandle(rowoff[pback[(size_t)q * C + k]]) << 16));
      }
    for (uint32_t k = 0; k < C; ++k) fwd[(size_t)nstates * C + k] = deadh;
  }
  std::vector<uint16_t> pairtab;
  uint32_t pair_magic = 0;
  {
    const uint64_t CC = (uint64_t)C * C, rows = (uint64_t)nstates + 1;
    bool ok = !S.general && !big && !(cfg.disable & KX_OFF_PAIR) && rows * CC <= 65535 && off_ent <= PAIR_CLS2 && C <= 63;
    if (ok) {
      pair_magic = (uint32_t)((1ull << 32) / CC) + 1;
      for (uint64_t q = 0; q < rows && ok; ++q) ok = (uint32_t)((q * CC * pair_magic) >> 32) == q;
    }
    if (ok) {
      pairtab.assign((rows * CC + 1) & ~(uint64_t)1, (uint16_t)(nstates * CC));
      for (uint32_t q = 0; q < nstates; ++q)
        for (uint32_t c1 = 0; c1 < C; ++c1) {
          const uint16_t d1 = delta[(size_t)q * C + c1];
          if (d1 == KXP_NO_STATE) continue;
          for (uint32_t c2 = 0; c2 < C; ++c2) {
            const uint16_t d2 = delta[(size_t)d1 * C + c2];
            if (d2 != KXP_NO_STATE) pairtab[((size_t)q * C + c1) * C + c2] = (uint16_t)(d2 * CC);
          }
        }
    }
  }
  packed.insert(packed.end(), ent.begin(), ent.end());
  packed.resize((packed.size() + 3) & ~(size_t)3, 0);
  const uint32_t off_pool = (uint32_t)packed.size() * 4;
  packed.resize(packed.size() + apool.size() / 4, 0);
  memcpy((char*)packed.data() + off_pool, apool.data(), apool.size());
  const uint32_t off_adesc = (uint32_t)packed.size() * 4;
  packed.insert(packed.end(), adesc.begin(), adesc.end());
  packed.resize((packed.size() + 3) & ~(size_t)3, 0);
  const uint32_t off_tbl = (uint32_t)packed.size() * 4;
  if (ntables) { packed.resize(packed.size() + (size_t)ntables * 64, 0); memcpy((char*)packed.data() + off_tbl, tables, (size_t)ntables * 256); }
  const uint32_t off_cls = 0;
  S.lds_bytes = big ? 0 : packed.size() * 4;
  if (S.lds_bytes > 150 * 1024) return setErr(KX_E_BLOB, "internal: table sizing (LDS budget)");
  const uint32_t nullrow = rowHandle(nullrow_idx);

  S.h_nleaves.assign(nleaves, nleaves + nstates); S.h_nleaves.push_back(1);
  S.h_fin_leaf.assign(fin_leaf, fin_leaf + nstates); S.h_fin_leaf.push_back(KXP_NO_LEAF);
  S.h_pool = apool;
  S.h_init_off.resize(Lm); S.h_init_len.resize(Lm);
  for (uint32_t j = 0; j < Lm; ++j) { S.h_init_off[j] = apoff[init_const[j]]; S.h_init_len[j] = pcoff[init_const[j] + 1] - pcoff[init_const[j]]; }

  if (nsync == 0 || nsync >= 0xFFF0) return setErr(KX_E_BLOB, "bad synchronising automaton");
  std::vector<uint32_t> newid(nsync);
  uint32_t nmulti = 0;
  for (uint32_t i = 0; i < nsync; ++i) if (sync_state[i] == KXP_SYNC_MULTI) newid[i] = nmulti++;
  { uint32_t t = nmulti; for (uint32_t i = 0; i < nsync; ++i) if (sync_state[i] != KXP_SYNC_MULTI) newid[i] = t++; }
  std::vector<uint16_t> sync16(((size_t)(nsync + 1) * (C + 1) + 1) & ~(size_t)1, 0);
  for (uint32_t i = 0; i < nsync; ++i) {
    const bool multi = sync_state[i] == KXP_SYNC_MULTI;
    for (uint32_t k = 0; k < C; ++k) {
      uint32_t nx = sync_next[(size_t)i * C + k];
      sync16[(size_t)newid[i] * C + k] = (uint16_t)(!multi ? newid[i] : nx == KXP_SYNC_UNKNOWN ? nsync : newid[nx]);
    }
    uint32_t st = sync_state[i];
    sync16[(size_t)(nsync + 1) * C + newid[i]] = (uint16_t)(st == KXP_SYNC_MULTI ? 0xFFFF : st == KXP_SYNC_EMPTY ? 0xFFFE : st);
  }
  for (uint32_t k = 0; k < C; ++k) sync16[(size_t)nsync * C + k] = (uint16_t)nsync;
  sync16[(size_t)(nsync + 1) * C + nsync] = 0xFFFD;
  const size_t sync_bytes = sync16.size() * 2;
  S.sync_lds_bytes = sync_bytes + 256 <= 64 * 1024 ? sync_bytes + 256 : 0;

  auto al = [](size_t x) { return (x + 255) & ~(size_t)255; };
  size_t o_packed = 0, o_cls = o_packed + al(packed.size() * 4), o_nl = o_cls + 256, o_fl = o_nl + al(nstates + 1),
         o_sn = o_fl + al(nstates + 1), o_io = o_sn + al(sync_bytes),
         o_il = o_io + al(Lm * 4), o_wl = o_il + al(Lm * 4), o_pr = o_wl + al(wlen.size() * 4), total = o_pr + al(pairtab.size() * 2);
  std::vector<uint8_t> img(total, 0);
  memcpy(&img[o_packed], packed.data(), packed.size() * 4);
  memcpy(&img[o_cls], cls, 256);
  memcpy(&img[o_nl], S.h_nleaves.data(), nstates + 1);
  memcpy(&img[o_fl], S.h_fin_leaf.data(), nstates + 1);
  memcpy(&img[o_sn], sync16.data(), sync_bytes);
  memcpy(&img[o_io], S.h_init_off.data(), Lm * 4);
  memcpy(&img[o_il], S.h_init_len.data(), Lm * 4);
  memcpy(&img[o_wl], wlen.data(), wlen.size() * 4);
  if (!pairtab.empty()) memcpy(&img[o_pr], pairtab.data(), pairtab.size() * 2);
  if (dry) return 0;
  HIPCHECK(hipMalloc(&S.d_all, total));
  HIPCHECK(hipMemcpy(S.d_all, img.data(), total, hipMemcpyHostToDevice));
  char* d = (char*)S.d_all;
  DevTables& T = S.T;
  T.packed = (const uint32_t*)(d + o_packed); T.packed_words = (uint32_t)packed.size();
  T.off_ent = off_ent; T.off_pool = off_pool; T.off_cls = off_cls;
  T.pair = (const uint32_t*)(d + o_pr); T.pair_words = (uint32_t)(pairtab.size() / 2); T.pair_magic = pair_magic;
  T.wlen = (const uint32_t*)(d + o_wl); T.off_adesc = off_adesc; T.naid = (uint32_t)adesc.size() / 2;
  T.nstates = nstates; T.nclasses = C; T.off_fwd = off_fwd; T.q0h = (off_fwd + q0 * C * 4) >> hshift; T.maxleaves = Lm; T.deadh = deadh; T.nullrow = nullrow; T.cshift = cshift;
  T.big = big ? 1u : 0u; T.hshift = hshift; T.rshift = rshift; T.rbase = rbase; T.stage_words = big ? 0u : (uint32_t)packed.size();
  T.cls = (const uint8_t*)(d + o_cls); T.nleaves = (const uint8_t*)(d + o_nl); T.fin_leaf = (const uint8_t*)(d + o_fl);
  T.sync16 = (const uint16_t*)(d + o_sn); T.nsync = nsync; T.sync_multi = nmulti; T.sync_words = (uint32_t)(sync_bytes / 4);
  T.init_off = (const uint32_t*)(d + o_io); T.init_len = (const uint32_t*)(d + o_il);
  T.off_tbl = off_tbl; T.xlat = xlat_tb ? off_tbl + ((xlat_tb - 1) << 8) : 0u; T.tblmode = tblmode ? 1u : 0u; T.aid_mask = tblmode ? 0x3FFu : 0x1FFFu; T.inl = inl && !big && !S.general ? 1u : 0u;
  T.jl = jl ? 1u : 0u; T.direct = direct ? 1u : 0u; T.short_consts = S.max_const_len <= 16 && !(cfg.disable & KX_OFF_CMPX) ? 1u : 0u;
  T.debug = cfg.debug_flags;
  if (S.has_df) {
    const size_t ib = (S.df.img.size() * 4 + 255) & ~(size_t)255;
    HIPCHECK(hipMalloc(&S.d_df, ib + (size_t)nstates * 2 + 16));
    HIPCHECK(hipMemcpy(S.d_df, S.df.img.data(), S.df.img.size() * 4, hipMemcpyHostToDevice));
    HIPCHECK(hipMemcpy((char*)S.d_df + ib, S.df.start_of_state.data(), (size_t)nstates * 2, hipMemcpyHostToDevice));
    DfDev& D = S.D;
    D.img = (const uint32_t*)S.d_df; D.words = (uint32_t)S.df.img.size();
    D.off_pool = S.df.off_pool; D.deadh = S.df.deadh; D.esch = S.df.esch; D.starth = S.df.starth; D.K = S.df.K; D.C = C;
    D.start_of_state = (const uint16_t*)((char*)S.d_df + ib);
    D.orig_c4 = C * 4; D.hshift = hshift; D.nstates = nstates; D.J = S.df.J;
    uint32_t mx = 0; for (uint32_t pc = 0; pc < npc; ++pc) mx = S.df_pc_len[pc] > mx ? S.df_pc_len[pc] : mx;
    D.short_consts = mx <= 16 && !(cfg.disable & KX_OFF_CMPX) ? 1u : 0u; D.debug = T.debug; D.wide = S.df.wide ? 1u : 0u;
    D.sl_on = 0;
    if (Lm <= 32 && !(cfg.disable & KX_OFF_SLOW)) {
      const uint32_t nP = S.df.nP, K = S.df.K;
      std::vector<uint32_t> pend((size_t)nP * K * Lm, 0), defoff(nP + 1, 0), defpc;
      std::vector<uint16_t> stq(nP);
      for (uint32_t i = 0; i < nP; ++i) {
        const kxdf::DfState& st = S.df.states[i];
        stq[i] = (uint16_t)st.q;
        for (uint32_t j = 0; j < K; ++j)
          for (uint32_t l = 0; l < Lm; ++l) pend[((size_t)i * K + j) * Lm + l] = st.pend[j].size() == 1 ? st.pend[j][0] : l < st.pend[j].size() ? st.pend[j][l] : st.pend[j][0];
        for (const auto& d : st.def) defpc.push_back(d.first);
        defoff[i + 1] = (uint32_t)defpc.size();
      }
      defpc.push_back(0);
      auto al = [](size_t x) { return (x + 255) & ~(size_t)255; };
      std::vector<uint32_t> fwd2(sc * 12, 0xFFFFFFFFu);
      for (size_t i = 0; i < sc; ++i) {
        uint32_t* f = &fwd2[12 * i];
        f[2] = f[3] = 0;
        if (delta[i] == KXP_NO_STATE) { f[0] = 0xFFFFu; f[1] = 0; continue; }
        f[0] = (uint32_t)delta[i] | ((uint32_t)nleaves[delta[i]] << 16); f[1] = pback[i];
        uint8_t* par = (uint8_t*)(f + 4);
        for (uint32_t l = 0; l < nleaves[delta[i]] && l < 32; ++l) { const uint32_t e = back[(size_t)pback[i] * Lm + l]; par[l] = e == KXP_DEAD_LEAF ? 0xFF : (uint8_t)(e & 0xFF); }
      }
      const size_t o_delta = 0, o_pback = o_delta + al(sc * 48), o_back = o_pback, o_pcoff = o_back + al((size_t)nback * Lm * 4),
                   o_pool = o_pcoff + al(((size_t)npc + 1) * 4), o_pend = o_pool + al(pcpl + 16), o_doff = o_pend + al(pend.size() * 4),
                   o_dpc = o_doff + al(defoff.size() * 4), o_q = o_dpc + al(defpc.size() * 4), tot = o_q + al((size_t)nP * 2);
      std::vector<uint8_t> sl(tot, 0);
      memcpy(&sl[o_delta], fwd2.data(), sc * 48); memcpy(&sl[o_back], back, (size_t)nback * Lm * 4);
      memcpy(&sl[o_pcoff], pcoff, ((size_t)npc + 1) * 4); memcpy(&sl[o_pool], pcpool, pcpl);
      memcpy(&sl[o_pend], pend.data(), pend.size() * 4); memcpy(&sl[o_doff], defoff.data(), defoff.size() * 4);
      memcpy(&sl[o_dpc], defpc.data(), defpc.size() * 4); memcpy(&sl[o_q], stq.data(), (size_t)nP * 2);
      HIPCHECK(hipMalloc(&S.d_slow, tot));
      HIPCHECK(hipMemcpy(S.d_slow, sl.data(), tot, hipMemcpyHostToDevice));
      const char* b0 = (const char*)S.d_slow;
      D.sl_fmap = (const uint4*)(b0 + o_delta); D.sl_back = (const uint32_t*)(b0 + o_back);
      D.sl_pcoff = (const uint32_t*)(b0 + o_pcoff); D.sl_pcpool = (const uint8_t*)(b0 + o_pool); D.sl_pend = (const uint32_t*)(b0 + o_pend);
      D.sl_defoff = (const uint32_t*)(b0 + o_doff); D.sl_defpc = (const uint32_t*)(b0 + o_dpc); D.sl_q = (const uint16_t*)(b0 + o_q);
      D.sl_nleaves = T.nleaves; D.sl_fin_leaf = T.fin_leaf; D.sl_cls = T.cls;
      D.sl_Lm = Lm; D.sl_npc = npc; D.sl_on = 1;
    }
  }
  return 0;
}

int setLds(const void* fn, size_t bytes) {
  HIPCHECK(hipFuncSetAttribute(fn, hipFuncAttributeMaxDynamicSharedMemorySize, (int)bytes));
  return 0;
}

float evMs(hipEvent_t a, hipEvent_t b) { float ms = 0; (void)hipEventElapsedTime(&ms, a, b); return ms; }

}

extern "C" {

const char* kx_last_error(void) { return g_err.c_str(); }
void kx_internal_set_error(const char* m) { g_err = m ? m : ""; }

int kx_validate(const void* blob, size_t blob_len) {
  if (!blob) return setErr(KX_E_ARG, "null argument");
  const uint8_t* b = (const uint8_t*)blob;
  if (blob_len < 20 || memcmp(b, KXP_MAGIC, 8)) return setErr(KX_E_BLOB, "not a KXP blob");
  uint32_t ver, ns, il;
  memcpy(&ver, b + 8, 4); memcpy(&ns, b + 12, 4); memcpy(&il, b + 16, 4);
  if (ver != KXP_VERSION || ns == 0 || ns > 64) return setErr(KX_E_BLOB, "unsupported KXP version");
  if ((unsigned long long)20 + pad4(il) > blob_len) return setErr(KX_E_BLOB, "truncated blob header");
  const uint8_t* c = b + 20 + pad4(il);
  for (uint32_t s = 0; s < ns; ++s) {
    Stage S;
    static const kx_config defaults{};
    int rc = parseStage(c, b + blob_len, S, defaults, true);
    if (rc) return rc;
  }
  return 0;
}

static int parseOneStage(const void* blob, size_t blob_len, uint32_t stage, const kx_config* cfgp, Stage& S) {
  static const kx_config defaults{};
  const kx_config& cfg = cfgp ? *cfgp : defaults;
  if (!blob) return setErr(KX_E_ARG, "null argument");
  const uint8_t* b = (const uint8_t*)blob;
  if (blob_len < 20 || memcmp(b, KXP_MAGIC, 8)) return setErr(KX_E_BLOB, "not a KXP blob");
  uint32_t ver, ns, il;
  memcpy(&ver, b + 8, 4); memcpy(&ns, b + 12, 4); memcpy(&il, b + 16, 4);
  if (ver != KXP_VERSION || ns == 0 || ns > 64) return setErr(KX_E_BLOB, "unsupported KXP version");
  if ((unsigned long long)20 + pad4(il) > blob_len) return setErr(KX_E_BLOB, "truncated blob header");
  if (stage >= ns) return setErr(KX_E_ARG, "no such stage");
  const uint8_t* c = b + 20 + pad4(il);
  for (uint32_t st = 0; st <= stage; ++st) {
    Stage T;
    int rc = parseStage(c, b + blob_len, st == stage ? S : T, cfg, true);
    if (rc) return rc;
  }
  return 0;
}

int kx_df_describe(const void* blob, size_t blob_len, uint32_t stage, kx_df_info* info, void* image, size_t image_cap) {
  return kx_df_describe_cfg(blob, blob_len, stage, nullptr, info, image, image_cap);
}

int kx_df_describe_cfg(const void* blob, size_t blob_len, uint32_t stage, const kx_config* cfg, kx_df_info* info, void* image, size_t image_cap) {
  if (!info) return setErr(KX_E_ARG, "null argument");
  Stage S;
  int rc = parseOneStage(blob, blob_len, stage, cfg, S);
  if (rc) return rc;
  memset(info, 0, sizeof *info);
  info->available = S.has_df ? 1u : 0u;
  snprintf(info->reason, sizeof info->reason, "%s", S.df_why.c_str());
  if (S.df.nP) {
    info->delay = S.df.K; info->nstates = S.df.nP; info->nclasses = S.df.C; info->image_bytes = (uint32_t)S.df.img.size() * 4;
    info->off_pool = S.df.off_pool; info->start_handle = S.df.starth; info->dead_handle = S.df.deadh; info->escape_handle = S.df.esch;
    info->transitions = S.df.ntrans; info->escapes = S.df.nesc; info->transitions_start = S.df.ntrans_start; info->escapes_start = S.df.nesc_start;
    info->merge_window = S.df.J;
    if (image) memcpy(image, S.df.img.data(), image_cap < S.df.img.size() * 4 ? image_cap : S.df.img.size() * 4);
  }
  return 0;
}

int kx_df_pending(const void* blob, size_t blob_len, uint32_t stage, uint32_t state, uint32_t slot, uint32_t* sst_state,
                  uint32_t* kinds, uint32_t* n_out) {
  return kx_df_pending_cfg(blob, blob_len, stage, nullptr, state, slot, sst_state, kinds, n_out);
}

int kx_df_pending_cfg(const void* blob, size_t blob_len, uint32_t stage, const kx_config* cfg, uint32_t state, uint32_t slot,
                      uint32_t* sst_state, uint32_t* kinds, uint32_t* n_out) {
  if (!kinds || !n_out || !sst_state) return setErr(KX_E_ARG, "null argument");
  Stage S;
  int rc = parseOneStage(blob, blob_len, stage, cfg, S);
  if (rc) return rc;
  if (state >= S.df.states.size() || slot >= S.df.K) return setErr(KX_E_ARG, "no such product state / slot");
  const kxdf::Slot& g = S.df.states[state].pend[slot];
  *sst_state = S.df.states[state].q;
  *n_out = (uint32_t)g.size();
  for (size_t i = 0; i < g.size() && i < KX_MAX_LEAVES; ++i) kinds[i] = g[i];
  return 0;
}

int kx_df_deferred(const void* blob, size_t blob_len, uint32_t stage, const kx_config* cfg, uint32_t state, void* bytes, size_t cap, size_t* n_out) {
  if (!n_out || (cap && !bytes)) return setErr(KX_E_ARG, "null argument");
  Stage S;
  int rc = parseOneStage(blob, blob_len, stage, cfg, S);
  if (rc) return rc;
  if (state >= S.df.states.size()) return setErr(KX_E_ARG, "no such product state");
  std::string t;
  for (const auto& d : S.df.states[state].def)
    if (d.first < S.df_pc_len.size()) t.append((const char*)S.h_pool.data() + S.df_pc_off[d.first], S.df_pc_len[d.first]);
  *n_out = t.size();
  if (cap) memcpy(bytes, t.data(), t.size() < cap ? t.size() : cap);
  return 0;
}

int kx_df_start_of_state(const void* blob, size_t blob_len, uint32_t stage, const kx_config* cfg, uint32_t sst_state, uint32_t* handle) {
  if (!handle) return setErr(KX_E_ARG, "null argument");
  Stage S;
  int rc = parseOneStage(blob, blob_len, stage, cfg, S);
  if (rc) return rc;
  if (sst_state >= S.df.start_of_state.size()) return setErr(KX_E_ARG, "no such state");
  *handle = S.df.start_of_state[sst_state];
  return 0;
}

int kx_stage_delayed_form(const kx_program* p, uint32_t stage) {
  if (!p || stage >= p->stages.size()) return 0;
  const Stage& S = p->stages[stage];
  return !S.has_df ? 0 : S.df_given_up ? 3 : S.df_skip ? 2 : 1;
}

void kx_stage_reset_delayed_form(kx_program* p, uint32_t stage) {
  if (!p || stage >= p->stages.size()) return;
  p->stages[stage].df_streak = 0; p->stages[stage].df_skip = 0; p->stages[stage].df_given_up = false; p->stages[stage].df_slow_armed = false;
}

static bool sameLoadFields(const kx_config& a, const kx_config& b) {
  const uint32_t load_off = KX_OFF_DIRECT | KX_OFF_PAIR | KX_OFF_CMPX | KX_OFF_SLOW, load_force = KX_FORCE_BIG | KX_FORCE_TBLMODE;
  return a.delayed_form == b.delayed_form && a.delay == b.delay && a.merge_window == b.merge_window && a.inline_consts == b.inline_consts &&
         a.job_stride == b.job_stride && (a.disable & load_off) == (b.disable & load_off) && (a.force & load_force) == (b.force & load_force) &&
         a.debug_flags == b.debug_flags;
}
static int checkConfig(kx_config& c) {
  if (c.block_threads == 0) c.block_threads = 512;
  if (c.segment_bytes % PIECE || c.segment_bytes > MAX_SEG || c.block_threads % 64 || c.block_threads > 1024 ||
      (c.block_threads & (c.block_threads - 1)))
    return setErr(KX_E_ARG, "segment_bytes: multiple of 64 (≤ 256 KiB); block_threads: power of two in [64, 1024]");
  if (c.delayed_form > 2 || c.delay > 2 || c.merge_window > 64 || c.inline_consts > 2 || c.job_stride > 2 || c.emit_half > 2 || c.emit_inplace > 2 ||
      c.act_lanes > 2 || c.df_backoff > 1 || (c.emit_waves && c.emit_waves != 4 && c.emit_waves != 8 && c.emit_waves != 12 && c.emit_waves != 16) ||
      c.batch_actions > 2 || c.reserved[0] || c.reserved[1] || c.reserved[2])
    return setErr(KX_E_ARG, "kx_config: a field is outside its range (include/kxhip.h)");
  return 0;
}

int kx_load(const void* blob, size_t blob_len, kx_program** prog) { return kx_load_config(blob, blob_len, nullptr, prog); }

int kx_load_config(const void* blob, size_t blob_len, const kx_config* cfgp, kx_program** prog) {
  if (!blob || !prog) return setErr(KX_E_ARG, "null argument");
  kx_config lc{};
  if (cfgp) lc = *cfgp;
  { int rc = checkConfig(lc); if (rc) return rc; }
  const uint8_t* b = (const uint8_t*)blob;
  if (blob_len < 20 || memcmp(b, KXP_MAGIC, 8)) return setErr(KX_E_BLOB, "not a KXP blob");
  uint32_t ver, ns, il;
  memcpy(&ver, b + 8, 4); memcpy(&ns, b + 12, 4); memcpy(&il, b + 16, 4);
  if (ver != KXP_VERSION || ns == 0 || ns > 64) return setErr(KX_E_BLOB, "unsupported KXP version");
  if ((unsigned long long)20 + pad4(il) > blob_len) return setErr(KX_E_BLOB, "truncated blob header");
  int ndev = 0;
  if (hipGetDeviceCount(&ndev) != hipSuccess || ndev == 0)
    return setErr(KX_E_HIP, "no HIP device available: the engine has no CPU fallback");
  const uint8_t* c = b + 20 + pad4(il);
  auto* p = new kx_program;
  p->cfg = lc;
  p->stages.resize(ns);
  for (uint32_t s = 0; s < ns; ++s) {
    const uint8_t* c0 = c;
    int rc = parseStage(c, b + blob_len, p->stages[s], lc);
    if (rc) { kx_free(p); return rc; }
    Stage& S = p->stages[s];
    if (lc.job_stride == 0 && !S.general && !S.big && !S.T.inl && !S.T.xlat && !S.T.jl) {
      Stage alt;
      g_force_jl = 1;
      const uint8_t* c1 = c0;
      rc = parseStage(c1, b + blob_len, alt, lc);
      g_force_jl = -1;
      if (rc == 0 && alt.T.jl && alt.lds_bytes <= S.lds_bytes && !alt.general) { S.d_all_alt = alt.d_all; S.Talt = alt.T; S.has_alt = true; alt.d_all = nullptr; }
      if (alt.d_all) (void)hipFree(alt.d_all);
      if (alt.d_df) (void)hipFree(alt.d_df);
      if (alt.d_slow) (void)hipFree(alt.d_slow);
    }
  }
  size_t lds = 0, slds = 0;
  for (auto& s : p->stages) { lds = s.lds_bytes > lds ? s.lds_bytes : lds; slds = s.sync_lds_bytes > slds ? s.sync_lds_bytes : slds; }
  hipDeviceProp_t prop;
  int dev = 0;
  if (hipGetDevice(&dev) == hipSuccess && hipGetDeviceProperties(&prop, dev) == hipSuccess) p->ncu = prop.multiProcessorCount;
  const size_t lds_cap = 160 * 1024;
  const size_t tab = (lds + 15) & ~(size_t)15;
  if (tab + 4 * (size_t)EMIT_WAVE_LDS_MIN > lds_cap) { kx_free(p); return setErr(KX_E_BLOB, "program tables leave no LDS for the output stage"); }
  int rc = setLds((const void*)k_forward<false>, 160 * 1024); if (rc) { kx_free(p); return rc; }
  rc = setLds((const void*)k_forward<true>, lds); if (rc) { kx_free(p); return rc; }
  rc = setLds((const void*)(k_forward<false, true>), 160 * 1024); if (rc) { kx_free(p); return rc; }
  rc = setLds((const void*)k_head<false>, lds); if (rc) { kx_free(p); return rc; }
  rc = setLds((const void*)k_head<true>, lds); if (rc) { kx_free(p); return rc; }
  rc = setLds((const void*)k_backlen<32, false>, tab + 1024 * 80); if (rc) { kx_free(p); return rc; }
  rc = setLds((const void*)k_backlen<32, true>, tab + 1024 * 80); if (rc) { kx_free(p); return rc; }
  rc = setLds((const void*)k_backlen<256, false>, tab + 1024 * 80); if (rc) { kx_free(p); return rc; }
  rc = setLds((const void*)k_backlen<256, true>, tab + 1024 * 80); if (rc) { kx_free(p); return rc; }
  rc = setLds((const void*)(k_backlen<32, false, true>), tab + 1024 * 80); if (rc) { kx_free(p); return rc; }
  rc = setLds((const void*)(k_backlen<256, false, true>), tab + 1024 * 80); if (rc) { kx_free(p); return rc; }
  rc = setLds((const void*)k_fixtail<false>, lds); if (rc) { kx_free(p); return rc; }
  rc = setLds((const void*)k_fixtail<true>, lds); if (rc) { kx_free(p); return rc; }
  if (slds) { rc = setLds((const void*)k_sync<true>, slds); if (rc) { kx_free(p); return rc; } }
  const size_t elds = lds_cap;
  bool anywide = false, anyext = false;
  for (auto& s : p->stages) { anywide = anywide || s.general; anyext = anyext || (!s.general && (s.T.inl || s.T.xlat)); }
#define KX_EMIT_ATTR(WV) (rc = setLds((const void*)k_emit<WV, false>, elds), rc = rc ? rc : (anywide ? setLds((const void*)k_emit<WV, true>, elds) : 0), \
                          rc = rc ? rc : (anyext ? setLds((const void*)k_emit<WV, false, true>, elds) : 0), \
                          rc ? rc : setLds((const void*)k_emit<WV, false, false, true>, elds))
  rc = KX_EMIT_ATTR(12); rc = rc ? rc : KX_EMIT_ATTR(8); rc = rc ? rc : KX_EMIT_ATTR(4);
#undef KX_EMIT_ATTR
  if (rc) { kx_free(p); return rc; }
  bool anydf = false;
  for (auto& s : p->stages) anydf = anydf || s.has_df;
  if (anydf) {
    rc = setLds((const void*)(k_dforward<512, 8, 4, false>), lds_cap); rc = rc ? rc : setLds((const void*)(k_dforward<512, 4, 4, false>), lds_cap);
    rc = rc ? rc : setLds((const void*)(k_dforward<512, 8, 4, true>), lds_cap); rc = rc ? rc : setLds((const void*)(k_dforward<512, 4, 4, true>), lds_cap); rc = rc ? rc : setLds((const void*)k_dhead, lds_cap);
    rc = rc ? rc : setLds((const void*)k_dmap<false>, 152 * 1024); rc = rc ? rc : setLds((const void*)k_dmap<true>, 152 * 1024);
#define KX_DEMIT_ATTR(WV) (rc = rc ? rc : setLds((const void*)k_demit<WV, 1>, lds_cap), rc = rc ? rc : setLds((const void*)k_demit<WV, 2>, lds_cap))
    KX_DEMIT_ATTR(16); KX_DEMIT_ATTR(12); KX_DEMIT_ATTR(8); KX_DEMIT_ATTR(4);
    rc = rc ? rc : setLds((const void*)(k_demit<12, 1, true>), lds_cap); rc = rc ? rc : setLds((const void*)(k_demit<12, 2, true>), lds_cap);
    rc = rc ? rc : setLds((const void*)(k_demit<16, 1, true>), lds_cap); rc = rc ? rc : setLds((const void*)(k_demit<16, 2, true>), lds_cap);
#undef KX_DEMIT_ATTR
    if (rc) { kx_free(p); return rc; }
  }
  *prog = p;
  return 0;
}

void kx_free(kx_program* p) {
  if (!p) return;
  for (auto& s : p->stages) { if (s.d_all) (void)hipFree(s.d_all); if (s.d_all_alt) (void)hipFree(s.d_all_alt); if (s.d_df) (void)hipFree(s.d_df); if (s.d_slow) (void)hipFree(s.d_slow); }
  for (Arena* a : p->arenas) { if (a->base) (void)hipFree(a->base); delete a; }
  for (int i = 0; i < 2; ++i) if (p->stagebuf[i]) (void)hipFree(p->stagebuf[i]);
  for (auto& a : p->actbuf) for (auto& b : a) if (b) (void)hipFree(b);
  for (ActionRunner* r : p->act_runners) delete r;
  delete p->batch;
  delete p->fields;
  delete p->field_list;
  if (p->have_events) for (auto& e : p->ev) (void)hipEventDestroy(e);
  delete p;
}

int kx_set_config(kx_program* p, const kx_config* cfg) {
  if (!p || !cfg) return setErr(KX_E_ARG, "null argument");
  kx_config c = *cfg;
  int rc = checkConfig(c);
  if (rc) return rc;
  if (!sameLoadFields(c, p->cfg)) return setErr(KX_E_ARG, "kx_set_config: a load-time field (delayed_form, delay, merge_window, inline_consts, job_stride, the load-time bits of disable / force, debug_flags) differs from what the program was loaded with: use kx_load_config");
  p->cfg = c;
  return 0;
}

uint32_t kx_num_stages(const kx_program* p) { return p ? (uint32_t)p->stages.size() : 0; }
int kx_stage_has_actions(const kx_program* p, uint32_t stage) { return p && stage < p->stages.size() && p->stages[stage].act ? 1 : 0; }

static int shardBegin(kx_program* p, uint32_t stage, const void* d_in, size_t n, int is_first, int is_last,
                      void* stream, kx_shard** out, bool internal) {
  if (!p || !out || stage >= p->stages.size()) return setErr(KX_E_ARG, "bad program/stage");
  if (!internal && p->stages[stage].act) return setErr(KX_E_ARG, "a stage with register actions cannot be sharded (kx_stage_has_actions)");
  if (n && (!d_in || ((uintptr_t)d_in & 15))) return setErr(KX_E_ARG, "input must be 16-byte aligned");
  if ((uint64_t)n >> 38) return setErr(KX_E_ARG, "a shard holds at most 256 GiB (piece indices are 32-bit); stream larger inputs in windows");
  auto* s = new kx_shard;
  s->prog = p; s->st = &p->stages[stage]; s->stage = stage;
  s->T = s->st->has_alt && s->st->use_alt ? &s->st->Talt : &s->st->T;
  s->in = (const uint8_t*)d_in; s->n = n; s->is_first = is_first; s->is_last = is_last; s->stream = (hipStream_t)stream;
  s->seg = p->cfg.segment_bytes;
  if (s->seg == 0) {
    const uint64_t slots = (uint64_t)p->ncu * 1024;
    const uint64_t m = (n + slots * 65536 - 1) / (slots * 65536) ? (n + slots * 65536 - 1) / (slots * 65536) : 1;
    s->seg = ((n + m * slots - 1) / (m * slots) + 511) & ~(uint64_t)511;
    if (s->seg < 4096) s->seg = 4096;
  }
  uint64_t ns = n ? (n + s->seg - 1) / s->seg : 1;
  if (ns > 0x7FFFFFF0ull) { delete s; return setErr(KX_E_ARG, "input too large for the configured segment size"); }
  s->nseg = (uint32_t)ns; s->nblk = s->nseg; s->Lc = s->st->maxleaves;
  const uint32_t bt = p->cfg.block_threads;
  s->ngroups = (s->nblk + bt - 1) / bt;
  if (p->arenas.empty()) p->arenas.push_back(new Arena);
  s->arena = p->arenas.back(); p->arenas.pop_back();
  Arena& A = *s->arena;
  s->df = s->st->has_df && n > 0;
  if (s->df && s->st->df_given_up) s->df = false;
  if (s->df && s->st->df_skip) { s->df = false; --s->st->df_skip; }
  s->side_cap = s->df && s->st->D.sl_on ? (uint32_t)(n / 8 < (1u << 22) ? (n / 8 > (1u << 18) ? n / 8 : (1u << 18)) : (1u << 22)) : 0u;
  size_t need = 4096 + (s->df ? (n / PIECE + 16) * sizeof(DfRec) + (size_t)s->nseg * 8 + 512 + (size_t)s->side_cap * 4 + 256 : 0) + (size_t)s->nseg * (8 + 2) + (n / HALF + 32) * 2 + sizeof(Flags) +
                (size_t)s->nblk * ((size_t)s->Lc * 5 + 3 + 4 + 8 + 2 + 4) + (size_t)s->ngroups * 16 + KX_MAX_LEAVES + 64 +
                (n / PIECE + 16) * 8 + 256 * 32;
  int rc = A.reserve(need);
  if (rc) { p->arenas.push_back(s->arena); delete s; return rc; }
  A.reset();
  s->seg_pos = A.take<uint64_t>(s->nseg); s->seg_state = A.take<uint16_t>(s->nseg);
  s->chk = A.take<uint16_t>(n / HALF + 32); s->flags = A.take<Flags>(1);
  s->bs_start = A.take<uint8_t>((size_t)s->nblk * s->Lc); s->bs_len = A.take<uint32_t>((size_t)s->nblk * s->Lc);
  s->bs_merged = A.take<uint8_t>(s->nblk); s->bs_mstart = A.take<uint8_t>(s->nblk); s->E = A.take<uint8_t>(s->nblk);
  s->len = A.take<uint32_t>(s->nblk); s->off = A.take<unsigned long long>(s->nblk);
  s->wsum = A.take<unsigned long long>(s->ngroups); s->woff = A.take<unsigned long long>(s->ngroups);
  s->d_map = A.take<uint8_t>(KX_MAX_LEAVES); s->d_const = A.take<uint32_t>(4);
  s->prec = A.take<PieceRec>(n / PIECE + 16);
  s->merge_piece = A.take<uint16_t>(s->nblk); s->ctot = A.take<uint32_t>(s->nblk);
  if (s->df) { s->dfrec = A.take<DfRec>(n / PIECE + 16); s->df_own = A.take<uint32_t>(s->nblk); s->df_spill = A.take<uint32_t>(s->nblk); s->side = s->side_cap ? A.take<uint32_t>(s->side_cap) : nullptr; }
  if (!p->have_events) {
    for (auto& e : p->ev) if (hipEventCreate(&e) != hipSuccess) { p->arenas.push_back(s->arena); delete s; return setErr(KX_E_HIP, "hipEventCreate failed"); }
    p->have_events = true;
  }
  s->stats.in_bytes = n;
  *out = s;
  return 0;
}

int kx_shard_begin(kx_program* p, uint32_t stage, const void* d_in, size_t n, int is_first, int is_last,
                   void* stream, kx_shard** out) {
  return shardBegin(p, stage, d_in, n, is_first, is_last, stream, out, false);
}

static int readFlags(kx_shard* s) {
  HIPCHECK(hipMemcpyAsync(&s->hflags, s->flags, sizeof(Flags), hipMemcpyDeviceToHost, s->stream));
  HIPCHECK(hipStreamSynchronize(s->stream));
  return 0;
}

static void fillFwd(kx_shard* s, kx_fwd_summary* out) {
  out->synced = s->have_end ? 1 : 0;
  out->end_state = s->have_end ? s->endId() : 0;
  out->head_len = s->head_len;
  out->fail_pos = s->hflags.fail_pos;
}

static int generalForward(kx_shard* s) {
  kx_program* p = s->prog; Stage& S = *s->st;
  const uint32_t bt = p->cfg.block_threads;
  const bool timing = p->cfg.collect_timing;
  const uint32_t grid = (s->nseg + bt - 1) / bt;
  if (timing) HIPCHECK(hipEventRecord(p->ev[1], s->stream));
  const size_t xoff = ((size_t)(*s->T).off_ent + 15) & ~(size_t)15;
  const size_t xoffp = (PAIR_TAB + (size_t)(*s->T).pair_words * 4 + 15) & ~(size_t)15;
  const bool coop_ok = !S.general && !(p->cfg.disable & KX_OFF_COOP);
  if (coop_ok && (*s->T).pair_words)
    hipLaunchKernelGGL((k_forward<false, true>), dim3((s->nseg + 1023) / 1024), dim3(1024), xoffp, s->stream, s->in, s->n, s->nseg,
                       s->seg_pos, s->seg_state, s->chk, s->flags, 1u, (*s->T));
  else if (coop_ok)
    hipLaunchKernelGGL((k_forward<false, false>), dim3(grid), dim3(bt), xoff, s->stream, s->in, s->n, s->nseg,
                       s->seg_pos, s->seg_state, s->chk, s->flags, 1u, (*s->T));
  else if ((*s->T).pair_words)
    hipLaunchKernelGGL((k_forward<false, true>), dim3((s->nseg + 1023) / 1024), dim3(1024), PAIR_TAB + (size_t)(*s->T).pair_words * 4, s->stream, s->in, s->n, s->nseg,
                       s->seg_pos, s->seg_state, s->chk, s->flags, 0u, (*s->T));
  else
  hipLaunchKernelGGL(S.general ? k_forward<true> : k_forward<false>, dim3(grid), dim3(bt), S.lds_bytes, s->stream, s->in, s->n, s->nseg, s->seg_pos,
                     s->seg_state, s->chk, s->flags, 0u, (*s->T));
  if (timing) HIPCHECK(hipEventRecord(p->ev[2], s->stream));
  HIPCHECK(hipGetLastError());
  int rc = readFlags(s);
  if (rc) return rc;
  if (timing) s->stats.kernel_ms[KX_K_FORWARD] = evMs(p->ev[1], p->ev[2]);
  s->stats.unsynced_segments = s->hflags.unsynced;
  if (s->is_first) { s->head_len = 0; s->have_end = true; }
  else {
    uint64_t hp = UNSYNC;
    if (s->hflags.first_synced != 0xFFFFFFFFu) HIPCHECK(hipMemcpy(&hp, s->seg_pos + s->hflags.first_synced, 8, hipMemcpyDeviceToHost));
    s->head_len = hp == UNSYNC ? s->n : hp;
    s->have_end = hp != UNSYNC;
  }
  return 0;
}

static int dfFallBack(kx_shard* s, const char* why, bool with_head) {
  Stage& S = *s->st;
  if (getenv("KX_DEBUG")) fprintf(stderr, "[kx] delayed form: %s; stage %u falls back to the general engine\n", why, s->stage);
  s->df = false;
  S.df_streak = S.df_streak < 6 ? S.df_streak + 1 : 6;
  S.df_skip = s->prog->cfg.df_backoff == 1 ? 0u : (1u << S.df_streak) - 1u;
  Flags init{}; init.fail_pos = NOFAIL; init.end_state = S.handleOf(S.q0);
  HIPCHECK(hipMemcpyAsync(s->flags, &init, 12, hipMemcpyHostToDevice, s->stream));
  HIPCHECK(hipMemsetAsync(&s->flags->emit_ovf, 0, offsetof(Flags, side_used) - offsetof(Flags, emit_ovf), s->stream));
  int rc = generalForward(s);
  if (rc) return rc;
  if (with_head && !s->is_first && s->head_len > 0) {
    hipLaunchKernelGGL(S.general ? k_head<true> : k_head<false>, dim3(1), dim3(64), S.lds_bytes, s->stream, s->in, s->n, s->head_len,
                       S.handleOf(s->df_qin), s->chk, s->flags, (*s->T));
    HIPCHECK(hipGetLastError());
    rc = readFlags(s);
    if (rc) return rc;
  } else if (with_head && !s->is_first && s->n == 0) s->hflags.end_state = S.handleOf(s->df_qin);
  if (with_head) {
    s->have_end = true;
    if (s->is_last && s->hflags.fail_pos == NOFAIL && S.h_fin_leaf[s->endId()] == KXP_NO_LEAF) s->hflags.fail_pos = s->n;
  }
  return 0;
}

int kx_shard_forward(kx_shard* s, kx_fwd_summary* out) {
  if (!s || !out) return setErr(KX_E_ARG, "null argument");
  kx_program* p = s->prog; Stage& S = *s->st;
  const uint32_t bt = p->cfg.block_threads;
  const bool timing = p->cfg.collect_timing;
  Flags init{}; init.fail_pos = NOFAIL; init.end_state = s->df ? S.df.starth : S.handleOf(S.q0); init.first_synced = 0xFFFFFFFFu; init.df_first_own = ~0ull;
  HIPCHECK(hipMemcpyAsync(s->flags, &init, sizeof(Flags), hipMemcpyHostToDevice, s->stream));
  if (s->n == 0) {
    s->hflags = init; s->head_len = 0; s->have_end = s->is_first != 0;
    fillFwd(s, out);
    return 0;
  }
  const uint32_t grid = (s->nseg + bt - 1) / bt;
  if (timing) HIPCHECK(hipEventRecord(p->ev[0], s->stream));
  if (S.sync_lds_bytes)
    hipLaunchKernelGGL((k_sync<true>), dim3(grid), dim3(bt), S.sync_lds_bytes, s->stream, s->in, s->n, s->seg, s->nseg,
                       s->is_first, s->seg_pos, s->seg_state, s->flags, (*s->T));
  else
    hipLaunchKernelGGL((k_sync<false>), dim3(grid), dim3(bt), 0, s->stream, s->in, s->n, s->seg, s->nseg, s->is_first,
                       s->seg_pos, s->seg_state, s->flags, (*s->T));
  if (timing) HIPCHECK(hipEventRecord(p->ev[1], s->stream));
  if (s->df) {
    HIPCHECK(hipMemsetAsync(s->df_own, 0, (size_t)s->nblk * 4, s->stream));
    HIPCHECK(hipMemsetAsync(s->df_spill, 0, (size_t)s->nblk * 4, s->stream));
    constexpr int DBT = 512;
    const size_t dimg = (((size_t)S.D.words + 3) & ~(size_t)3) * 4;
    auto launchForward = [&](bool slow) {
#define KX_LAUNCH_DFWD(ST, SL) hipLaunchKernelGGL((k_dforward<DBT, ST, 4, SL>), dim3((s->nseg + DBT - 1) / DBT), dim3(DBT), dimg + (size_t)DBT * ST * 16, s->stream, s->in, s->n, s->seg, s->nseg, \
                                                  s->is_first, s->seg_pos, s->seg_state, s->dfrec, s->df_own, s->df_spill, s->flags, s->side, s->side_cap, s->is_last, S.D)
      if (2 * (dimg + (size_t)DBT * 8 * 16) <= 160 * 1024) { if (slow) KX_LAUNCH_DFWD(8, true); else KX_LAUNCH_DFWD(8, false); }
      else { if (slow) KX_LAUNCH_DFWD(4, true); else KX_LAUNCH_DFWD(4, false); }
#undef KX_LAUNCH_DFWD
    };
    launchForward(S.df_slow_armed);
    if (timing) HIPCHECK(hipEventRecord(p->ev[2], s->stream));
    HIPCHECK(hipGetLastError());
    int rc = readFlags(s);
    if (rc) return rc;
    const uint64_t esc_lanes = (uint64_t)s->hflags.df_esc + s->hflags.warm_esc;
    if (s->hflags.df_esc && !S.df_slow_armed && S.D.sl_on && esc_lanes * 16 < s->nseg) {
      if (getenv("KX_DEBUG")) fprintf(stderr, "[kx] delayed form: an undecided context; stage %u arms the slow path of its forward pass\n", s->stage);
      S.df_slow_armed = true;
      Flags again = s->hflags; again.fail_pos = NOFAIL; again.end_state = S.df.starth; again.df_esc = 0; again.side_used = 0; again.slow_steps = 0;
      again.emit_kmax = again.emit_ksum = again.emit_kn = 0; again.df_first_own = ~0ull; again.warm_esc = 0;
      HIPCHECK(hipMemcpyAsync(s->flags, &again, sizeof(Flags), hipMemcpyHostToDevice, s->stream));
      HIPCHECK(hipMemsetAsync(s->df_own, 0, (size_t)s->nblk * 4, s->stream));
      HIPCHECK(hipMemsetAsync(s->df_spill, 0, (size_t)s->nblk * 4, s->stream));
      launchForward(true);
      if (timing) HIPCHECK(hipEventRecord(p->ev[2], s->stream));
      HIPCHECK(hipGetLastError());
      rc = readFlags(s);
      if (rc) return rc;
    }
    if (timing) s->stats.kernel_ms[KX_K_SYNC] = evMs(p->ev[0], p->ev[1]);
    if (getenv("KX_DEBUG") && s->hflags.slow_steps) fprintf(stderr, "[kx] delayed form: the slow path resolved %u input symbols in place (%u side entries handed out)\n", s->hflags.slow_steps, s->hflags.side_used);
    if ((uint64_t)s->hflags.slow_steps * 8 > s->n && s->n >= 4096) S.df_given_up = true;
    if (!s->hflags.df_esc) {
      if (timing) s->stats.kernel_ms[KX_K_FORWARD] = evMs(p->ev[1], p->ev[2]);
      s->stats.unsynced_segments = s->hflags.unsynced;
      if (s->is_first) { s->head_len = 0; s->have_end = true; }
      else { s->have_end = s->hflags.df_first_own != ~0ull; s->head_len = s->have_end ? s->hflags.df_first_own : s->n; }
      fillFwd(s, out);
      return 0;
    }
    if (esc_lanes >= 8 && esc_lanes * 16 >= s->nseg) S.df_given_up = true;
    rc = dfFallBack(s, S.df_given_up ? "the input leaves the form in (nearly) every segment: given up for this program" : "a context that the delay does not decide", false);
    if (rc) return rc;
    fillFwd(s, out);
    return 0;
  }
  int rc = generalForward(s);
  if (rc) return rc;
  if (timing) s->stats.kernel_ms[KX_K_SYNC] = evMs(p->ev[0], p->ev[1]);
  fillFwd(s, out);
  return 0;
}

int kx_shard_fix_head(kx_shard* s, uint32_t incoming_state, kx_fwd_summary* out) {
  if (!s || !out) return setErr(KX_E_ARG, "null argument");
  kx_program* p = s->prog; Stage& S = *s->st;
  if (!s->is_first && incoming_state > S.nstates) return setErr(KX_E_ARG, "incoming state out of range");
  s->df_qin = s->is_first ? S.q0 : incoming_state;
  if (s->df && !s->is_first) {
    const uint32_t hin = incoming_state < S.nstates ? S.df.start_of_state[incoming_state] : 0xFFFFu;
    if (hin == 0xFFFFu) { int rc = dfFallBack(s, "the incoming state is outside the table", false); if (rc) return rc; }
    else if (s->head_len > 0) {
      const bool timing = p->cfg.collect_timing;
      if (timing) HIPCHECK(hipEventRecord(p->ev[0], s->stream));
      hipLaunchKernelGGL(k_dhead, dim3(1), dim3(64), (size_t)S.D.words * 4 + 16, s->stream, s->in, s->n, s->seg, s->head_len, hin,
                         s->dfrec, s->df_own, s->df_spill, s->flags, S.D);
      if (timing) HIPCHECK(hipEventRecord(p->ev[1], s->stream));
      HIPCHECK(hipGetLastError());
      int rc = readFlags(s);
      if (rc) return rc;
      if (timing) s->stats.kernel_ms[KX_K_HEAD] = evMs(p->ev[0], p->ev[1]);
      if (s->hflags.df_esc) { rc = dfFallBack(s, "a context that the delay does not decide (head)", false); if (rc) return rc; }
    }
  }
  if (!s->df && !s->is_first && s->head_len > 0) {
    const bool timing = p->cfg.collect_timing;
    if (timing) HIPCHECK(hipEventRecord(p->ev[0], s->stream));
    hipLaunchKernelGGL(S.general ? k_head<true> : k_head<false>, dim3(1), dim3(64), S.lds_bytes, s->stream, s->in, s->n, s->head_len,
                       S.handleOf(incoming_state), s->chk, s->flags, (*s->T));
    if (timing) HIPCHECK(hipEventRecord(p->ev[1], s->stream));
    HIPCHECK(hipGetLastError());
    int rc = readFlags(s);
    if (rc) return rc;
    if (timing) s->stats.kernel_ms[KX_K_HEAD] = evMs(p->ev[0], p->ev[1]);
  } else if (!s->is_first && s->n == 0) {
    s->hflags.end_state = S.handleOf(incoming_state);
  }
  s->have_end = true;
  if (s->is_last && s->hflags.fail_pos == NOFAIL && S.h_fin_leaf[s->endId()] == KXP_NO_LEAF)
    s->hflags.fail_pos = s->n;
  fillFwd(s, out);
  return 0;
}

int kx_shard_backward(kx_shard* s, kx_bwd_summary* out) {
  if (!s || !out) return setErr(KX_E_ARG, "null argument");
  kx_program* p = s->prog; Stage& S = *s->st;
  memset(out, 0, sizeof *out);
  const uint32_t nle = S.h_nleaves[s->endId()];
  out->nleaves = nle;
  if (s->n == 0) {
    if (s->is_last && S.h_fin_leaf[s->endId()] != KXP_NO_LEAF) {
      out->constant = 1;
      for (uint32_t e = 0; e < nle; ++e) out->start_leaf[e] = S.h_fin_leaf[s->endId()];
    } else {
      out->constant = 0;
      for (uint32_t e = 0; e < nle; ++e) out->start_leaf[e] = (uint8_t)e;
    }
    return 0;
  }
  if (s->df) {
    if (s->is_first) return 0;
    const uint64_t cap = 1u << 16;
    hipLaunchKernelGGL(S.general ? k_dmap<true> : k_dmap<false>, dim3(1), dim3(256), S.lds_bytes, s->stream, s->in, s->n, s->df_qin, cap, s->d_map, s->d_const, (*s->T));
    HIPCHECK(hipGetLastError());
    uint32_t status = 0;
    HIPCHECK(hipMemcpyAsync(out->start_leaf, s->d_map, KX_MAX_LEAVES, hipMemcpyDeviceToHost, s->stream));
    HIPCHECK(hipMemcpyAsync(&status, s->d_const, 4, hipMemcpyDeviceToHost, s->stream));
    HIPCHECK(hipStreamSynchronize(s->stream));
    if (status == 2 && s->is_last && S.h_fin_leaf[s->endId()] != KXP_NO_LEAF) {
      if (getenv("KX_DEBUG")) fprintf(stderr, "[kx] delayed form: the last shard's start-leaf map stays open to the end of the input; taken at the final state's leaf\n");
      const uint8_t v = out->start_leaf[S.h_fin_leaf[s->endId()]];
      for (uint32_t e = 0; e < KX_MAX_LEAVES; ++e) out->start_leaf[e] = v;
      out->constant = 1;
      return 0;
    }
    if (status) { out->constant = status == 1 ? 1u : 0u; return 0; }
    int rc = dfFallBack(s, "the start-leaf map does not settle", true);
    if (rc) return rc;
  }
  uint32_t bt = p->cfg.block_threads;
  if (bt < 1024 && 2 * (((S.lds_bytes + 15) & ~(size_t)15) + (size_t)bt * 80) > 160 * 1024) bt = 1024;
  const uint32_t grid = (s->nblk + bt - 1) / bt;
  const bool timing = p->cfg.collect_timing;
  if (timing) HIPCHECK(hipEventRecord(p->ev[0], s->stream));
  const size_t blds = ((S.lds_bytes + 15) & ~(size_t)15) + (size_t)bt * 80;
#define KX_LAUNCH_BACKLEN(MC, WD, ...)                                                                             \
  hipLaunchKernelGGL((k_backlen<MC, WD, ##__VA_ARGS__>), dim3(grid), dim3(bt), blds, s->stream, s->in, s->n, s->seg, s->nblk, s->chk, \
                     s->flags, s->is_last, s->bs_start, s->bs_len, s->bs_merged, s->bs_mstart, s->Lc, s->prec,        \
                     s->merge_piece, s->ctot, (*s->T))
  if (s->Lc <= 32) { if (S.general) KX_LAUNCH_BACKLEN(32, true); else if ((*s->T).jl) KX_LAUNCH_BACKLEN(32, false, true); else KX_LAUNCH_BACKLEN(32, false); }
  else { if (S.general) KX_LAUNCH_BACKLEN(256, true); else if ((*s->T).jl) KX_LAUNCH_BACKLEN(256, false, true); else KX_LAUNCH_BACKLEN(256, false); }
#undef KX_LAUNCH_BACKLEN
  if (timing) HIPCHECK(hipEventRecord(p->ev[1], s->stream));
  HIPCHECK(hipGetLastError());
  if (!s->is_first) {
    hipLaunchKernelGGL(k_shard_map, dim3(1), dim3(64), 0, s->stream, s->nblk, nle, s->bs_start, s->bs_merged,
                       s->bs_mstart, s->Lc, s->d_map, s->d_const);
    HIPCHECK(hipMemcpyAsync(out->start_leaf, s->d_map, nle, hipMemcpyDeviceToHost, s->stream));
    HIPCHECK(hipMemcpyAsync(&out->constant, s->d_const, 4, hipMemcpyDeviceToHost, s->stream));
  }
  HIPCHECK(hipStreamSynchronize(s->stream));
  if (timing) s->stats.kernel_ms[KX_K_BACKLEN] = evMs(p->ev[0], p->ev[1]);
  return 0;
}

int kx_shard_resolve(kx_shard* s, uint32_t end_leaf, uint64_t* out_len) {
  if (!s || !out_len) return setErr(KX_E_ARG, "null argument");
  kx_program* p = s->prog; Stage& S = *s->st;
  if (s->is_last) end_leaf = S.h_fin_leaf[s->endId()];
  if (end_leaf >= S.h_nleaves[s->endId()]) return setErr(KX_E_ARG, "end leaf out of range");
  if (s->n == 0) {
    s->init_shift = s->is_first ? S.h_init_len[end_leaf] : 0;
    s->out_len = s->init_shift;
    *out_len = s->out_len;
    s->init_leaf = end_leaf;
    return 0;
  }
  const uint32_t bt = p->cfg.block_threads;
  const bool timing = p->cfg.collect_timing;
  if (s->df) {
    if (timing) HIPCHECK(hipEventRecord(p->ev[0], s->stream));
    hipLaunchKernelGGL(k_dlen, dim3(s->ngroups), dim3(bt), 0, s->stream, s->nblk, s->df_own, s->df_spill, s->len, s->wsum);
    hipLaunchKernelGGL(k_scan_groups, dim3(1), dim3(1024), 0, s->stream, s->ngroups, s->wsum, s->woff, s->flags);
    hipLaunchKernelGGL(k_scan_blocks, dim3(s->ngroups), dim3(bt), 0, s->stream, s->nblk, s->len, s->woff, s->off);
    if (timing) HIPCHECK(hipEventRecord(p->ev[1], s->stream));
    HIPCHECK(hipGetLastError());
    const uint32_t K = S.df.K;
    uint8_t lastb[kxdf::DF_MAX_K] = {0, 0, 0, 0};
    const uint32_t nb = s->n < K ? (uint32_t)s->n : K;
    HIPCHECK(hipMemcpyAsync(lastb + (K - nb), s->in + (s->n - nb), nb, hipMemcpyDeviceToHost, s->stream));
    int rc = readFlags(s);
    if (rc) return rc;
    if (timing) s->stats.kernel_ms[KX_K_RESOLVE] = evMs(p->ev[0], p->ev[1]);
    if (S.df.indexOf(s->hflags.end_state) >= S.df.states.size()) return setErr(KX_E_ARG, "internal: the shard did not end in a state of the delayed form");
    const kxdf::DfState& E = S.df.states[S.df.indexOf(s->hflags.end_state)];
    s->df_tail.clear();
    for (const auto& d : E.def)
      if (d.first < S.df_pc_len.size()) s->df_tail.insert(s->df_tail.end(), S.h_pool.begin() + S.df_pc_off[d.first], S.h_pool.begin() + S.df_pc_off[d.first] + S.df_pc_len[d.first]);
    for (uint32_t j = 0; j < K; ++j) {
      const kxdf::Slot& g = E.pend[j];
      const kxdf::Kind kd = g.size() == 1 ? g[0] : g[end_leaf < g.size() ? end_leaf : 0];
      if (kd & 1u) s->df_tail.push_back(lastb[j]);
      const uint32_t pc = kd >> 1;
      if (pc < S.df_pc_len.size()) s->df_tail.insert(s->df_tail.end(), S.h_pool.begin() + S.df_pc_off[pc], S.h_pool.begin() + S.df_pc_off[pc] + S.df_pc_len[pc]);
    }
    s->init_shift = 0; s->init_leaf = 0;
    s->df_body = s->hflags.total_len;
    s->out_len = s->df_body + s->df_tail.size();
    *out_len = s->out_len;
    return 0;
  }
  if (timing) HIPCHECK(hipEventRecord(p->ev[0], s->stream));
  hipLaunchKernelGGL(k_resolve_leaf, dim3(s->ngroups), dim3(bt), 0, s->stream, s->nblk, end_leaf, s->bs_start, s->bs_merged, s->bs_mstart, s->Lc, s->E);
  hipLaunchKernelGGL(k_resolve, dim3(s->ngroups), dim3(bt), 0, s->stream, s->nblk, s->E, s->bs_len, s->Lc, s->len, s->wsum);
  hipLaunchKernelGGL(k_scan_groups, dim3(1), dim3(1024), 0, s->stream, s->ngroups, s->wsum, s->woff, s->flags);
  hipLaunchKernelGGL(k_scan_blocks, dim3(s->ngroups), dim3(bt), 0, s->stream, s->nblk, s->len, s->woff, s->off);
  if (S.general)
    hipLaunchKernelGGL((k_fixtail<true>), dim3(s->ngroups), dim3(bt), S.lds_bytes, s->stream, s->in, s->n, s->seg, s->nblk,
                       s->chk, s->E, s->len, s->merge_piece, s->ctot, s->prec, s->flags, (*s->T));
  else
    hipLaunchKernelGGL((k_fixtail<false>), dim3(s->ngroups), dim3(bt), S.lds_bytes, s->stream, s->in, s->n, s->seg, s->nblk,
                       s->chk, s->E, s->len, s->merge_piece, s->ctot, s->prec, s->flags, (*s->T));
  if (timing) HIPCHECK(hipEventRecord(p->ev[1], s->stream));
  HIPCHECK(hipGetLastError());
  uint8_t e0 = 0;
  HIPCHECK(hipMemcpyAsync(&e0, s->E, 1, hipMemcpyDeviceToHost, s->stream));
  int rc = readFlags(s);
  if (rc) return rc;
  if (timing) s->stats.kernel_ms[KX_K_RESOLVE] = evMs(p->ev[0], p->ev[1]);
  s->init_shift = 0;
  if (s->is_first) {
    uint8_t l0 = 0;
    HIPCHECK(hipMemcpy(&l0, s->bs_start + (size_t)e0, 1, hipMemcpyDeviceToHost));
    s->init_shift = S.h_init_len[l0];
    s->init_leaf = l0;
  }
  s->out_len = s->hflags.total_len + s->init_shift;
  *out_len = s->out_len;
  return 0;
}

int kx_shard_emit(kx_shard* s, void* d_out, size_t cap) {
  if (!s) return setErr(KX_E_ARG, "null argument");
  kx_program* p = s->prog; Stage& S = *s->st;
  if (cap < s->out_len || (s->out_len && !d_out)) return setErr(KX_E_CAPACITY, "output buffer too small");
  if ((uintptr_t)d_out & 15) return setErr(KX_E_ARG, "output buffer must be 16-byte aligned");
  s->stats.out_bytes = s->out_len;
  if (s->n == 0) {
    if (s->init_shift) {
      uint32_t leaf = s->init_leaf;
      HIPCHECK(hipMemcpyAsync(d_out, S.h_pool.data() + S.h_init_off[leaf], s->init_shift, hipMemcpyHostToDevice, s->stream));
      HIPCHECK(hipStreamSynchronize(s->stream));
    }
    return 0;
  }
  const bool timing = p->cfg.collect_timing;
  const uint64_t npieces = (s->n + PIECE - 1) / PIECE;
  const uint64_t nwi = (npieces + 63) / 64;
  if (s->df) {
    const size_t lds_cap = 160 * 1024, tab = ((size_t)S.D.words * 4 + 15) & ~(size_t)15;
    int W = 12;
    { const int v = (int)p->cfg.emit_waves; if (v == 4 || v == 8 || v == 12 || v == 16) W = v; }
    const size_t per_wave = ((lds_cap - tab) / W) & ~(size_t)63;
    const double olen = 64.0 * (double)s->out_len / (double)s->n;
    const uint32_t kmax = s->hflags.emit_kmax < 64 ? s->hflags.emit_kmax : 64;
    double kper = s->hflags.emit_kn ? 1.1 * (double)s->hflags.emit_ksum / (double)s->hflags.emit_kn + 1.0 : (double)kmax + 1;
    if (kper > kmax + 1) kper = kmax + 1;
    size_t stgb = 0, jbytes = 0; uint32_t maxcnt = 64;
    auto plan = [&](double ol, double kp) {
      for (uint32_t R = 1; R <= 64; ++R) {
        const uint32_t c = (64 + R - 1) / R;
        size_t st = (((size_t)(c * ol * 1.05) + 64) + 63) & ~(size_t)63, jb = ((size_t)(c * kp + 16) * 4 + 63) & ~(size_t)63;
        if (st < 1024) st = 1024;
        if (st + 16 + jb <= per_wave || c == 1) { maxcnt = c; jbytes = jb; stgb = per_wave - 16 - jb; break; }
      }
    };
    plan(olen, kper);
    bool halfmode = maxcnt <= 32 && (W == 12 || W == 16);
    if (p->cfg.emit_half) halfmode = p->cfg.emit_half == 2 && (W == 12 || W == 16);
    if (halfmode) plan(olen / 2, kper / 2 + 0.5);
    if (stgb > 49152) stgb = 49152;
    stgb &= ~(size_t)15;
    const uint64_t nwi_df = halfmode ? (npieces * 2 + 63) / 64 : nwi;
    const uint64_t wantg = (nwi_df + W - 1) / W;
    const uint32_t grid = (uint32_t)(wantg < (uint64_t)p->ncu ? wantg : (uint64_t)p->ncu);
    const size_t elds = tab + (size_t)W * (stgb + 16 + jbytes);
    const uint64_t ppb = s->seg / PIECE, blk_inv = ppb > 1 ? ~0ull / ppb + 1 : 0;
    if (timing) HIPCHECK(hipEventRecord(p->ev[0], s->stream));
#define KX_LAUNCH_DEMIT(WV, KK)                                                                                                    \
  hipLaunchKernelGGL((k_demit<WV, KK>), dim3(grid), dim3(WV * 64), elds, s->stream, s->in, s->n, s->seg, blk_inv, npieces, s->dfrec, \
                     s->df_spill, s->off, s->flags, (uint32_t)stgb, (uint32_t)jbytes, maxcnt, (uint8_t*)d_out, s->side, S.D)
#define KX_LAUNCH_DEMIT_K(WV) do { if (S.df.K == 1) KX_LAUNCH_DEMIT(WV, 1); else KX_LAUNCH_DEMIT(WV, 2); } while (0)
#define KX_LAUNCH_DEMIT_H(WV, KK)                                                                                                    \
  hipLaunchKernelGGL((k_demit<WV, KK, true>), dim3(grid), dim3(WV * 64), elds, s->stream, s->in, s->n, s->seg, blk_inv, npieces, s->dfrec, \
                     s->df_spill, s->off, s->flags, (uint32_t)stgb, (uint32_t)jbytes, maxcnt, (uint8_t*)d_out, s->side, S.D)
    if (halfmode) {
      if (W == 16) { if (S.df.K == 1) KX_LAUNCH_DEMIT_H(16, 1); else KX_LAUNCH_DEMIT_H(16, 2); }
      else { if (S.df.K == 1) KX_LAUNCH_DEMIT_H(12, 1); else KX_LAUNCH_DEMIT_H(12, 2); }
    } else
    if (W == 16) KX_LAUNCH_DEMIT_K(16); else if (W == 12) KX_LAUNCH_DEMIT_K(12); else if (W == 8) KX_LAUNCH_DEMIT_K(8); else KX_LAUNCH_DEMIT_K(4);
#undef KX_LAUNCH_DEMIT_H
#undef KX_LAUNCH_DEMIT_K
#undef KX_LAUNCH_DEMIT
    if (timing) HIPCHECK(hipEventRecord(p->ev[1], s->stream));
    HIPCHECK(hipGetLastError());
    if (!s->df_tail.empty())
      HIPCHECK(hipMemcpyAsync((uint8_t*)d_out + s->df_body, s->df_tail.data(), s->df_tail.size(), hipMemcpyHostToDevice, s->stream));
    uint32_t ovf = 0;
    const bool debug = getenv("KX_DEBUG") != nullptr;
    if (timing || debug) HIPCHECK(hipMemcpyAsync(&ovf, &s->flags->emit_ovf, 4, hipMemcpyDeviceToHost, s->stream));
    HIPCHECK(hipStreamSynchronize(s->stream));
    if (timing) s->stats.kernel_ms[KX_K_EMIT] = evMs(p->ev[0], p->ev[1]);
    s->stats.emit_overflow_pieces = ovf;
    S.df_streak = 0;
    if (debug && (S.D.debug & 64u)) {
      Flags hf; HIPCHECK(hipMemcpy(&hf, s->flags, sizeof(Flags), hipMemcpyDeviceToHost));
      double tot = 0; for (int i = 0; i < 6; ++i) tot += (double)hf.dbg[i];
      fprintf(stderr, "[kx] emit timeline, delayed form (share of wave time): operands+logic %.3f round-logic %.3f walk %.3f constants %.3f flush %.3f; ticks/wave-iteration %.0f\n",
              hf.dbg[0] / tot, hf.dbg[2] / tot, hf.dbg[3] / tot, hf.dbg[4] / tot, hf.dbg[5] / tot, tot / (double)nwi);
    }
    if (debug) fprintf(stderr, "[kx] emit (delayed form, K=%u, %u product states, image %zu B)%s: W=%d stg=%zu jobs=%zu maxcnt=%u kmax=%u kavg=%.2f olen=%.1f overflow=%u of %llu pieces\n",
                       S.df.K, S.df.nP, (size_t)S.D.words * 4, halfmode ? ", a lane = half a piece" : "", W, stgb, jbytes, maxcnt, kmax, s->hflags.emit_kn ? (double)s->hflags.emit_ksum / s->hflags.emit_kn : -1.0, olen, ovf, (unsigned long long)npieces);
    return 0;
  }
  const size_t lds_cap = 160 * 1024, tab = (S.lds_bytes + 15) & ~(size_t)15;
  int W = tab + 12 * (size_t)EMIT_WAVE_LDS_MIN <= lds_cap ? 12 : tab + 8 * (size_t)EMIT_WAVE_LDS_MIN <= lds_cap ? 8 : 4;
  { const int v = (int)p->cfg.emit_waves; if ((v == 4 || v == 8 || v == 12) && v <= W) W = v; }
  const size_t per_wave = ((lds_cap - tab) / W) & ~(size_t)255;
  const double olen = 64.0 * (double)s->out_len / (double)(s->n ? s->n : 1);
  const uint32_t kmax = s->hflags.emit_kmax < 64 ? s->hflags.emit_kmax : 64;
  double kper = s->hflags.emit_kn ? 1.25 * (double)s->hflags.emit_ksum / (double)s->hflags.emit_kn + 1.5 : (double)kmax + 1;
  if (S.has_alt && s->hflags.emit_kn) S.use_alt = (double)s->hflags.emit_ksum / (double)s->hflags.emit_kn >= 12.0 ? 1 : 0;
  if (kper > kmax + 1) kper = kmax + 1;
  size_t stgb = 0, jbytes = 0; uint32_t maxcnt = 64, jslots = 0;
  const bool inplace = !S.big && (p->cfg.emit_inplace ? p->cfg.emit_inplace == 2 : S.max_const_len <= 4 && kper >= 24.0);
  for (uint32_t R = 1; R <= 64; ++R) {
    const uint32_t c = (64 + R - 1) / R;
    size_t st = (((size_t)(c * olen * 1.08) + 64) + 255) & ~(size_t)255, jb = inplace ? 0 : ((size_t)(c * kper + 16) * 4 + 255) & ~(size_t)255;
    if (st < 1024) st = 1024;
    uint32_t js = 0;
    if ((*s->T).jl && !inplace)
      jb = ((size_t)(c * (kper + 1.0) + 16) * 4 + 255) & ~(size_t)255;
    if (st + 16 + jb <= per_wave || c == 1) {
      maxcnt = c; jbytes = jb; jslots = js; stgb = per_wave - 16 - jb;
      break;
    }
  }
  if (p->cfg.emit_staging) { size_t v = (size_t)p->cfg.emit_staging & ~(size_t)255; if (v >= 1024 && v + 16 + jbytes <= per_wave) stgb = v; }
  if (stgb > 49152) stgb = 49152;
  stgb &= ~(size_t)15;
  uint64_t wantg = (nwi + W - 1) / W;
  const uint32_t grid = (uint32_t)(wantg < (uint64_t)p->ncu ? wantg : (uint64_t)p->ncu);
  const size_t elds = tab + (size_t)W * (stgb + 16 + jbytes);
  const uint64_t ppb = s->seg / PIECE, blk_inv = ppb > 1 ? ~0ull / ppb + 1 : 0;
  if (timing) HIPCHECK(hipEventRecord(p->ev[0], s->stream));
#define KX_LAUNCH_EMIT(WV, WD, EX, ...)                                                                              \
  hipLaunchKernelGGL((k_emit<WV, WD, EX, ##__VA_ARGS__>), dim3(grid), dim3(WV * 64), elds, s->stream, s->in, s->n, s->seg, blk_inv, npieces, s->chk, \
                     s->prec, s->ctot, s->off, s->flags, (uint32_t)stgb, (uint32_t)jbytes, maxcnt, jslots, s->init_shift, s->init_leaf, s->is_first, (uint8_t*)d_out, (*s->T))
  if ((*s->T).jl && !S.general) { if (W == 12) KX_LAUNCH_EMIT(12, false, false, true); else if (W == 8) KX_LAUNCH_EMIT(8, false, false, true); else KX_LAUNCH_EMIT(4, false, false, true); }
  else if (S.general) { if (W == 12) KX_LAUNCH_EMIT(12, true, false); else if (W == 8) KX_LAUNCH_EMIT(8, true, false); else KX_LAUNCH_EMIT(4, true, false); }
  else if ((*s->T).inl || (*s->T).xlat) { if (W == 12) KX_LAUNCH_EMIT(12, false, true); else if (W == 8) KX_LAUNCH_EMIT(8, false, true); else KX_LAUNCH_EMIT(4, false, true); }
  else { if (W == 12) KX_LAUNCH_EMIT(12, false, false); else if (W == 8) KX_LAUNCH_EMIT(8, false, false); else KX_LAUNCH_EMIT(4, false, false); }
#undef KX_LAUNCH_EMIT
  if (timing) HIPCHECK(hipEventRecord(p->ev[1], s->stream));
  HIPCHECK(hipGetLastError());
  uint32_t ovf = 0;
  const bool debug = getenv("KX_DEBUG") != nullptr;
  if (timing || debug) HIPCHECK(hipMemcpyAsync(&ovf, &s->flags->emit_ovf, 4, hipMemcpyDeviceToHost, s->stream));
  HIPCHECK(hipStreamSynchronize(s->stream));
  if (timing) s->stats.kernel_ms[KX_K_EMIT] = evMs(p->ev[0], p->ev[1]);
  s->stats.emit_overflow_pieces = ovf;
  if (debug && ((*s->T).debug & 64u)) {
    Flags hf; HIPCHECK(hipMemcpy(&hf, s->flags, sizeof(Flags), hipMemcpyDeviceToHost));
    double tot = 0; for (int i = 0; i < 6; ++i) tot += (double)hf.dbg[i];
    fprintf(stderr, "[kx] emit timeline (share of wave time): load+logic %.3f forward %.3f round-logic %.3f sweep %.3f constants %.3f flush %.3f; ticks/wave-iteration %.0f\n",
            hf.dbg[0] / tot, hf.dbg[1] / tot, hf.dbg[2] / tot, hf.dbg[3] / tot, hf.dbg[4] / tot, hf.dbg[5] / tot, tot / (double)nwi);
  }
  if (debug) fprintf(stderr, "[kx] emit: layout=%s next=%s ", (*s->T).jl ? "job-stride" : "vote-and-rank", S.has_alt ? (S.use_alt ? "job-stride" : "vote-and-rank") : "(fixed)");
  if (debug) fprintf(stderr, "[kx] emit: W=%d stg=%zu jobs=%zu maxcnt=%u kmax=%u kavg=%.2f olen=%.1f overflow=%u of %llu pieces\n", W, stgb, jbytes, maxcnt, kmax, s->hflags.emit_kn ? (double)s->hflags.emit_ksum / s->hflags.emit_kn : -1.0, olen, ovf, (unsigned long long)npieces);
  return 0;
}

void kx_shard_stats(kx_shard* s, kx_stats* st) {
  if (!s || !st) return;
  *st = s->stats;
  st->fail_pos = s->hflags.fail_pos; st->fail_stage = s->stage;
}

void kx_shard_end(kx_shard* s) {
  if (!s) return;
  if (s->arena) s->prog->arenas.push_back(s->arena);
  delete s;
}

static int runPipeline(kx_program* p, const void* d_in, size_t n, void* d_out, size_t cap, bool alloc_final,
                       void** d_final, size_t* out_len, kx_stats* stats, void* stream) {
  kx_stats total{}; total.fail_pos = NOFAIL; total.in_bytes = n;
  const void* cur = d_in; size_t curn = n;
  void* aligned_copy = nullptr;
  struct FreeOnExit { void*& p; ~FreeOnExit() { if (p) (void)hipFree(p); } } free_aligned{aligned_copy};
  if (n && ((uintptr_t)d_in & 15)) {
    HIPCHECK(hipMalloc(&aligned_copy, n));
    HIPCHECK(hipMemcpyAsync(aligned_copy, d_in, n, hipMemcpyDeviceToDevice, (hipStream_t)stream));
    cur = aligned_copy;
  }
  int rc = 0;
  const uint32_t ns = (uint32_t)p->stages.size();
  for (uint32_t st = 0; st < ns && rc == 0; ++st) {
    kx_shard* s = nullptr;
    const bool pdbg = getenv("KX_DEBUG") != nullptr;
    auto now = []() { return std::chrono::steady_clock::now(); };
    auto ms = [](std::chrono::steady_clock::time_point a, std::chrono::steady_clock::time_point b) { return std::chrono::duration<double, std::milli>(b - a).count(); };
    const auto pt0 = now();
    rc = shardBegin(p, st, cur, curn, 1, 1, stream, &s, true);
    if (rc) break;
    const auto pt1 = now();
    kx_fwd_summary fs; kx_bwd_summary bs; uint64_t ol = 0;
    rc = kx_shard_forward(s, &fs);
    if (!rc) rc = kx_shard_fix_head(s, 0, &fs);
    if (!rc && fs.fail_pos != NOFAIL) { total.fail_pos = fs.fail_pos; total.fail_stage = st; rc = KX_MATCH_ERROR; }
    const auto pt2 = now();
    if (!rc) rc = kx_shard_backward(s, &bs);
    const auto pt3 = now();
    if (!rc) rc = kx_shard_resolve(s, 0, &ol);
    if (pdbg) fprintf(stderr, "[kx] stage %u host wall: begin %.2f ms, forward %.2f, backward %.2f, resolve %.2f\n", st, ms(pt0, pt1), ms(pt1, pt2), ms(pt2, pt3), ms(pt3, now()));
    Stage& SG = p->stages[st];
    if (!rc && SG.act) {
      const int par = st & 1;
      auto ensure = [&](int k, size_t bytes) -> int {
        if (p->actcap[par][k] >= bytes) return 0;
        if (p->actbuf[par][k]) (void)hipFree(p->actbuf[par][k]);
        p->actbuf[par][k] = nullptr; p->actcap[par][k] = 0;
        if (hipMalloc(&p->actbuf[par][k], bytes + bytes / 8 + 4096) != hipSuccess) return setErr(KX_E_HIP, "hipMalloc(action buffers) failed");
        p->actcap[par][k] = bytes + bytes / 8 + 4096;
        return 0;
      };
      const bool adbg = getenv("KX_DEBUG") != nullptr;
      const auto at0 = std::chrono::steady_clock::now();
      rc = ensure(0, ol + 16);
      if (!rc) rc = kx_shard_emit(s, p->actbuf[par][0], p->actcap[par][0]);
      const auto at1 = std::chrono::steady_clock::now();
      size_t al = 0;
      if (!rc) {
        if (p->act_runners.size() < ns) p->act_runners.resize(ns, nullptr);
        ActionRunner*& ar = p->act_runners[st];
        if (!ar) { ar = new ActionRunner; ar->cfg = &p->cfg; rc = ar->init(SG.act_regs); if (rc) { delete ar; ar = nullptr; } }
        else rc = ar->reset();
        if (!rc) rc = ensure(1, ol + ar->slack());
        if (!rc) rc = ar->run((const uint8_t*)p->actbuf[par][0], ol, (uint8_t*)p->actbuf[par][1], &al, (hipStream_t)stream);
      }
      if (adbg) {
        const auto at2 = std::chrono::steady_clock::now();
        fprintf(stderr, "[kx] action stage %u: emit of the token stream %.2f ms (host wall), post-pass %.2f ms\n", st,
                std::chrono::duration<double, std::milli>(at1 - at0).count(), std::chrono::duration<double, std::milli>(at2 - at1).count());
      }
      if (!rc) {
        if (st + 1 == ns) {
          *out_len = al;
          void* dst = nullptr;
          if (alloc_final) { if (hipMalloc(d_final, al ? al : 16) != hipSuccess) rc = setErr(KX_E_HIP, "hipMalloc(output) failed"); dst = *d_final; }
          else { if (al > cap || (al && !d_out)) rc = setErr(KX_E_CAPACITY, "output buffer too small"); dst = d_out; }
          const auto ct0 = std::chrono::steady_clock::now();
          if (!rc && al) {
            hipLaunchKernelGGL(k_copy_bytes, dim3(p->ncu * 8), dim3(256), 0, (hipStream_t)stream, (uint8_t*)dst, (const uint8_t*)p->actbuf[par][1], (unsigned long long)al);
            HIPCHECK(hipGetLastError()); HIPCHECK(hipStreamSynchronize((hipStream_t)stream));
          }
          if (adbg) fprintf(stderr, "[kx] action stage %u: result to its place (%zu bytes, device to device) %.2f ms\n", st, al, std::chrono::duration<double, std::milli>(std::chrono::steady_clock::now() - ct0).count());
        }
        if (!rc) { cur = p->actbuf[par][1]; curn = al; ol = al; }
      }
    } else
    if (!rc) {
      void* dst = nullptr; size_t dcap = 0;
      if (st + 1 == ns) {
        *out_len = ol;
        if (alloc_final) {
          if (hipMalloc(d_final, ol ? ol : 16) != hipSuccess) rc = setErr(KX_E_HIP, "hipMalloc(output) failed");
          dst = *d_final; dcap = ol;
        } else {
          if (ol > cap || (ol && !d_out)) rc = setErr(KX_E_CAPACITY, "output buffer too small");
          dst = d_out; dcap = cap;
        }
      } else {
        int slot = st & 1;
        if (p->stagecap[slot] < ol + 16) {
          if (p->stagebuf[slot]) (void)hipFree(p->stagebuf[slot]);
          p->stagebuf[slot] = nullptr; p->stagecap[slot] = 0;
          if (hipMalloc(&p->stagebuf[slot], ol + ol / 8 + 4096) != hipSuccess) rc = setErr(KX_E_HIP, "hipMalloc(stage buffer) failed");
          else p->stagecap[slot] = ol + ol / 8 + 4096;
        }
        dst = p->stagebuf[slot]; dcap = p->stagecap[slot];
      }
      if (!rc) rc = kx_shard_emit(s, dst, dcap);
      if (!rc) { cur = dst; curn = ol; }
    }
    kx_stats ss; kx_shard_stats(s, &ss);
    for (int i = 0; i < KX_NKERNELS; ++i) { total.kernel_ms[i] += ss.kernel_ms[i]; total.total_ms += ss.kernel_ms[i]; }
    total.unsynced_segments += ss.unsynced_segments;
    total.out_bytes = ol;
    kx_shard_end(s);
  }
  if (stats) *stats = total;
  return rc;
}

int kx_run_device(kx_program* p, const void* d_in, size_t n, void* d_out, size_t cap, size_t* out_len, kx_stats* stats,
                  void* stream) {
  if (!p || !out_len) return setErr(KX_E_ARG, "null argument");
  return runPipeline(p, d_in, n, d_out, cap, false, nullptr, out_len, stats, stream);
}

int kx_run_host(kx_program* p, const void* in, size_t n, void** out, size_t* out_len, kx_stats* stats) {
  if (!p || !out || !out_len) return setErr(KX_E_ARG, "null argument");
  *out = nullptr; *out_len = 0;
  void* d_in = nullptr; void* d_out = nullptr;
  struct FreeOnExit { void*& p; ~FreeOnExit() { if (p) (void)hipFree(p); } } free_in{d_in}, free_out{d_out};
  if (n) { HIPCHECK(hipMalloc(&d_in, n)); HIPCHECK(hipMemcpy(d_in, in, n, hipMemcpyHostToDevice)); }
  size_t ol = 0;
  int rc = runPipeline(p, d_in, n, nullptr, 0, true, &d_out, &ol, stats, nullptr);
  if (rc == 0) {
    *out = malloc(ol ? ol : 1);
    if (!*out) rc = setErr(KX_E_IO, "out of host memory");
    else if (ol && hipMemcpy(*out, d_out, ol, hipMemcpyDeviceToHost) != hipSuccess) rc = setErr(KX_E_HIP, "D2H copy failed");
    if (!rc) *out_len = ol;
  }
  return rc;
}

void kx_host_free(void* p) { free(p); }

}

namespace {

struct DevBuf { char* d = nullptr; size_t cap = 0; };

struct BufPool {
  std::mutex m; std::vector<DevBuf> idle; std::vector<char*> all;
  int get(size_t bytes, DevBuf* out) {
    {
      std::lock_guard<std::mutex> g(m);
      int best = -1;
      for (size_t i = 0; i < idle.size(); ++i) if (idle[i].cap >= bytes && (best < 0 || idle[i].cap < idle[(size_t)best].cap)) best = (int)i;
      if (best >= 0) { *out = idle[(size_t)best]; idle.erase(idle.begin() + best); return 0; }
    }
    DevBuf b; b.cap = bytes + bytes / 16 + 4096;
    HIPCHECK(hipMalloc((void**)&b.d, b.cap));
    { std::lock_guard<std::mutex> g(m); all.push_back(b.d); }
    *out = b;
    return 0;
  }
  void put(DevBuf b) { if (!b.d) return; std::lock_guard<std::mutex> g(m); idle.push_back(b); }
  ~BufPool() { for (char* d : all) (void)hipFree(d); }
};

template <typename T>
struct BoundedQueue {
  std::mutex m; std::condition_variable cv; std::deque<T> q; size_t cap; bool closed = false;
  explicit BoundedQueue(size_t c) : cap(c) {}
  bool push(T v) {
    std::unique_lock<std::mutex> g(m);
    cv.wait(g, [&] { return q.size() < cap || closed; });
    if (closed) return false;
    q.push_back(std::move(v)); cv.notify_all();
    return true;
  }
  bool pop(T* v) {
    std::unique_lock<std::mutex> g(m);
    cv.wait(g, [&] { return !q.empty() || closed; });
    if (q.empty()) return false;
    *v = std::move(q.front()); q.pop_front(); cv.notify_all();
    return true;
  }
  void close() { std::lock_guard<std::mutex> g(m); closed = true; cv.notify_all(); }
  void finish() { std::unique_lock<std::mutex> g(m); closed = true; cv.notify_all(); }
};

struct FdStream {
  kx_program* p = nullptr; int in_fd = -1, out_fd = -1;
  uint32_t stage0 = 0;
  size_t CH = 64u << 20, window = 0;
  int dev = 0;
  BufPool pool;
  struct InWin { DevBuf b; size_t n; bool last; };
  struct OutWin { DevBuf b; size_t n; };
  BoundedQueue<InWin> inq{2};
  BoundedQueue<OutWin> outq{2};
  std::mutex em; int err = 0; std::string emsg;
  struct Win { kx_shard* sh; DevBuf in; size_t n; kx_bwd_summary bs; };
  struct StageQ { std::vector<Win> pend; uint32_t end_state = 0; bool first = true; uint64_t consumed = 0; ActionRunner* act = nullptr; };
  std::vector<StageQ> q;
  kx_stats total{};
  double t_read = 0, t_h2d_wait = 0, t_in_push = 0, t_in_pop = 0, t_compute = 0, t_out_push = 0, t_out_pop = 0, t_d2h_wait = 0, t_write = 0;
  static double nowMs() { return std::chrono::duration<double, std::milli>(std::chrono::steady_clock::now().time_since_epoch()).count(); }

  void fail(int code) {
    std::lock_guard<std::mutex> g(em);
// ... 273 lines not shown
```

Before: 1105.

## Pack piece records into 8 bytes and derive output offsets via wave scan

```diff
diff --git a/kleenexlang_amd/csrc/engine/kx_dfkernels.inc b/kleenexlang_amd/csrc/engine/kx_dfkernels.inc
--- a/kleenexlang_amd/csrc/engine/kx_dfkernels.inc
+++ b/kleenexlang_amd/csrc/engine/kx_dfkernels.inc
@@ -13,9 +13,50 @@
   const uint32_t* sl_pcoff; const uint8_t* sl_pcpool; const uint32_t* sl_pend; const uint32_t* sl_defoff; const uint32_t* sl_defpc; const uint16_t* sl_q;
   uint32_t sl_Lm, sl_npc, sl_on;
 };
-constexpr uint32_t DFREC_HOLE = 0xFFFF0000u, DF_HOLE_MAX = 4096, DF_HOLE_FIRST = 1024, DF_SL_LEAVES = 32;
-struct __attribute__((aligned(16))) DfRec { uint32_t hh, cum, info, kc; };
-constexpr uint32_t DFREC_OWN = 0x80000000u;
+constexpr uint32_t DF_HOLE_MAX = 4096, DF_HOLE_FIRST = 1024, DF_SL_LEAVES = 32;
+struct __attribute__((aligned(8))) DfRec { uint32_t x, y; };
+constexpr uint32_t DFREC_OWN = 0x80000000u, DFREC_HOLE = 0x80000000u, DFREC_HOLE_FIRST = 0x40000000u;
+constexpr uint32_t DF_MERGE_WINDOW_MAX = 64;
+constexpr uint32_t DF_STEP_MAX = 126, DF_HOLE_LEN_MAX = 0xFFFFu, DF_HOLE_CNT_MAX = 0x3FFFu, DF_WBASE_PIECES = 32;
+constexpr DfRec dfrec_pack(uint32_t start, uint32_t middle, uint32_t lenA, uint32_t len, uint32_t kA, uint32_t kB) {
+  return DfRec{(start >> 3) | ((middle >> 3) << 13) | (kA << 26), len | (lenA << 13) | (kB << 25)};
+}
+constexpr DfRec dfrec_pack_hole(uint32_t side_first, uint32_t entries, bool first, uint32_t len) {
+  return DfRec{side_first, len | (entries << 16) | (first ? DFREC_HOLE_FIRST : 0u) | DFREC_HOLE};
+}
+constexpr bool dfrec_hole(DfRec r) { return (r.y & DFREC_HOLE) != 0; }
+constexpr uint32_t dfrec_start(DfRec r) { return (r.x & 0x1FFFu) << 3; }
+constexpr uint32_t dfrec_middle(DfRec r) { return ((r.x >> 13) & 0x1FFFu) << 3; }
+constexpr uint32_t dfrec_kA(DfRec r) { return r.x >> 26; }
+constexpr uint32_t dfrec_kB(DfRec r) { return (r.y >> 25) & 0x3Fu; }
+constexpr uint32_t dfrec_len(DfRec r) { return r.y & 0x1FFFu; }
+constexpr uint32_t dfrec_lenA(DfRec r) { return (r.y >> 13) & 0xFFFu; }
+constexpr uint32_t dfrec_hole_side(DfRec r) { return r.x; }
+constexpr uint32_t dfrec_hole_len(DfRec r) { return r.y & DF_HOLE_LEN_MAX; }
+constexpr uint32_t dfrec_hole_entries(DfRec r) { return (r.y >> 16) & DF_HOLE_CNT_MAX; }
+constexpr bool dfrec_hole_first(DfRec r) { return (r.y & DFREC_HOLE_FIRST) != 0; }
+namespace dfrec_check {
+constexpr uint32_t H = 65536 - 8, LA = HALF * DF_STEP_MAX, LN = PIECE * DF_STEP_MAX, KH = HALF;
+constexpr DfRec top = dfrec_pack(H, H, LA, LN, KH, KH), one = dfrec_pack(8, 65536 - 16, 1, 2, 0, KH), zero = dfrec_pack(0, 0, 0, 0, 0, 0);
+static_assert(sizeof(DfRec) == 8 && LN < (1u << 13) && LA < (1u << 12) && KH < (1u << 6), "piece record: a field outgrew its width");
+static_assert(!dfrec_hole(top) && dfrec_start(top) == H && dfrec_middle(top) == H && dfrec_lenA(top) == LA && dfrec_len(top) == LN &&
+              dfrec_kA(top) == KH && dfrec_kB(top) == KH, "piece record: every field at its maximum");
+static_assert(!dfrec_hole(one) && dfrec_start(one) == 8 && dfrec_middle(one) == 65536 - 16 && dfrec_lenA(one) == 1 && dfrec_len(one) == 2 &&
+              dfrec_kA(one) == 0 && dfrec_kB(one) == KH, "piece record: neighbouring fields do not bleed");
+static_assert(!dfrec_hole(zero) && zero.x == 0 && zero.y == 0, "piece record: all fields zero");
+constexpr DfRec htop = dfrec_pack_hole(0xFFFFFFFFu, DF_HOLE_CNT_MAX, true, DF_HOLE_LEN_MAX), hlow = dfrec_pack_hole(0, 0, false, 0);
+static_assert(dfrec_hole(htop) && dfrec_hole_side(htop) == 0xFFFFFFFFu && dfrec_hole_entries(htop) == DF_HOLE_CNT_MAX && dfrec_hole_first(htop) &&
+              dfrec_hole_len(htop) == DF_HOLE_LEN_MAX, "hole record: every field at its maximum");
+static_assert(dfrec_hole(hlow) && dfrec_hole_side(hlow) == 0 && dfrec_hole_entries(hlow) == 0 && !dfrec_hole_first(hlow) && dfrec_hole_len(hlow) == 0, "hole record: all fields zero");
+static_assert(PIECE + kxdf::DF_MAX_K + DF_MERGE_WINDOW_MAX <= DF_HOLE_CNT_MAX, "hole record: the entries of a piece fit");
+static_assert((uint64_t)MAX_SEG * DF_STEP_MAX < DFREC_OWN, "wave base: a block part's output stays below the own flag");
+static_assert(DF_WBASE_PIECES == HALF && 2 * DF_WBASE_PIECES == PIECE, "wave base: one word per wave-iteration of half pieces, two per iteration of pieces");
+}
+inline bool dfRecFits(const uint32_t* img, uint32_t nrows, uint32_t C) {
+  if (256u + (uint64_t)nrows * C * 8u > 65536u) return false;
+  for (size_t i = 0; i < (size_t)nrows * C; ++i) if ((img[64 + 2 * i + 1] >> 24) > DF_STEP_MAX) return false;
+  return true;
+}
 
 struct DfLds {
   const uint8_t* base; uint32_t csh;
@@ -211,11 +252,12 @@
 template <int BT, uint32_t DF_STAGE, int MINW, bool SLOW>
 __global__ __launch_bounds__(BT, MINW) void k_dforward(const uint8_t* __restrict__ in, uint64_t n, uint64_t seg, uint32_t nseg, int first_known,
                            const uint64_t* __restrict__ seg_pos, const uint16_t* __restrict__ seg_state,
-                           DfRec* __restrict__ rec, uint32_t* __restrict__ own, uint32_t* __restrict__ spill, Flags* flags,
+                           DfRec* __restrict__ rec, uint32_t* __restrict__ wbase, uint32_t* __restrict__ own, uint32_t* __restrict__ spill, Flags* flags,
                            uint32_t* __restrict__ side, uint32_t side_cap, int is_last, DfDev D) {
+  static_assert(DF_STAGE == 8 || DF_STAGE == 16, "a group of staged records is one or half a 128-byte line, and at least the slow path's 64-byte map");
   extern __shared__ __attribute__((aligned(16))) uint32_t smem[];
   DfLds L = df_stage(D, smem);
-  uint4* lrec = reinterpret_cast<uint4*>(smem + ((D.words + 3) & ~3u)) + (size_t)threadIdx.x * DF_STAGE;
+  uint2* lrec = reinterpret_cast<uint2*>(smem + ((D.words + 3) & ~3u)) + (size_t)threadIdx.x * DF_STAGE;
   const uint32_t k = blockIdx.x * blockDim.x + threadIdx.x;
   const uint32_t lane = threadIdx.x & 63;
   const uint64_t B = k < nseg ? df_own_start(k, n, seg, first_known, seg_pos, seg_state, D) : UNSYNC;
@@ -262,28 +304,34 @@
   };
   uint32_t nst = 0; uint64_t gfirst = 0;
   auto flush_group = [&]() {
-    uint4* dst = reinterpret_cast<uint4*>(rec + gfirst);
+    uint2* dst = reinterpret_cast<uint2*>(rec + gfirst);
     for (uint32_t i = 0; i < nst; ++i) dst[i] = lrec[(gfirst + i) & (DF_STAGE - 1)];
     nst = 0;
   };
   const bool coop = !(D.debug & 256u);
   bool in_trip = false;
-  auto stage_rec = [&](uint64_t pc, uint4 r) {
+  auto stage_rec = [&](uint64_t pc, DfRec r) {
     if (nst == 0) gfirst = pc;
-    lrec[pc & (DF_STAGE - 1)] = r; ++nst;
+    if ((pc & (DF_WBASE_PIECES - 1)) == 0) wbase[pc / DF_WBASE_PIECES] = cum | flag;
+    lrec[pc & (DF_STAGE - 1)] = make_uint2(r.x, r.y); ++nst;
     if (!in_trip && (pc & (DF_STAGE - 1)) == DF_STAGE - 1) flush_group();
   };
-  uint4* const lrec_wave = reinterpret_cast<uint4*>(smem + ((D.words + 3) & ~3u)) + (size_t)(threadIdx.x & ~63u) * DF_STAGE;
+  auto group_aligned = [&]() { return ((uint32_t)(pos >> 6) & (DF_STAGE - 1)) == nst; };
+  uint2* const lrec_wave = reinterpret_cast<uint2*>(smem + ((D.words + 3) & ~3u)) + (size_t)(threadIdx.x & ~63u) * DF_STAGE;
   auto coop_flush = [&]() {
     const bool full = nst == DF_STAGE && (gfirst & (DF_STAGE - 1)) == 0;
+    if (!__any(full)) return;
     const uint32_t glo = (uint32_t)gfirst, ghi = (uint32_t)(gfirst >> 32) | (full ? 0u : 0x80000000u);
-    const uint32_t team = lane / DF_STAGE * DF_STAGE, r = lane % DF_STAGE;
-    static_for<0, (int)DF_STAGE>([&](auto ic) {
+    constexpr uint32_t RPL = DF_STAGE / 8;
+    const uint32_t team = lane & ~7u, r = (lane & 7u) * RPL;
+    static_for<0, 8>([&](auto ic) {
       constexpr uint32_t i = decltype(ic)::value;
       const uint32_t slo = (uint32_t)__shfl((int)glo, (int)(team + i)), shi = (uint32_t)__shfl((int)ghi, (int)(team + i));
       if (!(shi & 0x80000000u)) {
         const uint64_t g = ((uint64_t)shi << 32) | slo;
-        reinterpret_cast<uint4*>(rec + g)[r] = lrec_wave[(size_t)(team + i) * DF_STAGE + r];
+        const uint2* src = lrec_wave + (size_t)(team + i) * DF_STAGE + r;
+        if constexpr (RPL == 2) *reinterpret_cast<uint4*>(rec + g + r) = *reinterpret_cast<const uint4*>(src);
+        else *reinterpret_cast<uint2*>(rec + g + r) = *src;
       }
     });
     if (full) nst = 0;
@@ -313,8 +361,9 @@
         const uint32_t ee = E[idx + x], pc = (ee >> 1) & 0x3FFFFFFFu;
         len += (ee & 1u) + (pc < D.sl_npc ? D.sl_pcoff[pc + 1] - D.sl_pcoff[pc] : 0u);
       }
-      if (len > 0xFFFFu) return 1;
-      rec[pp >> 6] = DfRec{base + idx, cum, len | flag, DFREC_HOLE | (first ? 0x8000u : 0u) | cnt};
+      if (len > DF_HOLE_LEN_MAX || cnt > DF_HOLE_CNT_MAX) return 1;
+      if (((pp >> 6) & (DF_WBASE_PIECES - 1)) == 0) wbase[(pp >> 6) / DF_WBASE_PIECES] = cum | flag;
+      rec[pp >> 6] = dfrec_pack_hole(base + idx, cnt, first, len);
       idx += cnt; cum += len; pos = pp + steps;
     }
     h = io.h_next;
@@ -339,7 +388,7 @@
     }
     const uint32_t kA = (sumA & 0xFFu) >> 2, kB = (sum & 0xFFu) >> 2;
     kc_sum += kA + kB; kc_max = kA + kB > kc_max ? kA + kB : kc_max; ++kc_n;
-    stage_rec(pos >> 6, make_uint4(h0 | (mid << 16), cum, (sumA >> 8) | flag, kA | (kB << 8)));
+    stage_rec(pos >> 6, dfrec_pack(h0, mid, sumA >> 8, sum >> 8, kA, kB));
     cum += sum >> 8; pos += PIECE;
     return true;
   };
@@ -350,9 +399,9 @@
   };
   for (;;) {
   if (need_slow) run_slow();
-  while (!failed && !need_slow && pos + PIECE <= end && (pos & (8 * PIECE - 1))) single_piece();
+  while (!failed && !need_slow && pos + PIECE <= end && ((pos & (8 * PIECE - 1)) || !group_aligned())) single_piece();
   for (;;) {
-    const bool can = !failed && !need_slow && pos + 8 * PIECE <= end && !(pos & (8 * PIECE - 1));
+    const bool can = !failed && !need_slow && pos + 8 * PIECE <= end && !(pos & (8 * PIECE - 1)) && group_aligned();
     if (!__any(can) || __any(need_slow)) break;
     uint32_t line[8];
     {
@@ -383,8 +432,8 @@
       if (go && !do_piece(wa)) { died = true; go = false; }
       if (k2 < 3) issue(k2 + 1, v);
       if (go && !do_piece(wb)) died = true;
-      if (coop && ((k2 + 1) * 2) % DF_STAGE == 0) coop_flush();
-    }
+    }
+    if (coop) coop_flush();
     in_trip = false;
   }
   if (!__any(!failed && (need_slow || pos + 8 * PIECE <= end))) break;
@@ -407,7 +456,7 @@
     if (h == dead || h == esc) {
       if (fail_in(h0, pos, plen) == 2) { h = h0; need_slow = true; continue; }
     }
-    else { stage_rec(pos >> 6, make_uint4(h0 | (mid << 16), cum, lenA | flag, kA | ((kc - kA) << 8))); cum += len; pos = end; }
+    else { stage_rec(pos >> 6, dfrec_pack(h0, mid, lenA, len, kA, kc - kA)); cum += len; pos = end; }
   }
   break;
   }
@@ -419,7 +468,7 @@
 }
 
 __global__ void k_dhead(const uint8_t* __restrict__ in, uint64_t n, uint64_t seg, uint64_t head_len, uint32_t h,
-                        DfRec* __restrict__ rec, uint32_t* __restrict__ own, uint32_t* __restrict__ spill, Flags* flags, DfDev D) {
+                        DfRec* __restrict__ rec, uint32_t* __restrict__ wbase, uint32_t* __restrict__ own, uint32_t* __restrict__ spill, Flags* flags, DfDev D) {
   extern __shared__ __attribute__((aligned(16))) uint32_t smem[];
   DfLds L = df_stage(D, smem);
   if (blockIdx.x || threadIdx.x) return;
@@ -441,7 +490,8 @@
     }
     if (plen <= HALF) { mid = h; lenA = len; kA = kc; }
     if (kc > 0) atomicMax(&flags->emit_kmax, kc);
-    rec[pos >> 6] = DfRec{h0 | (mid << 16), cum, lenA, kA | ((kc - kA) << 8)};
+    if (((pos >> 6) & (DF_WBASE_PIECES - 1)) == 0) wbase[(pos >> 6) / DF_WBASE_PIECES] = cum;
+    rec[pos >> 6] = dfrec_pack(h0, mid, lenA, len, kA, kc - kA);
     cum += len; pos += plen;
   }
   spill[m] = cum;
@@ -556,7 +606,7 @@
 
 template <int WAVES, int K, bool HALF = false>
 __global__ __launch_bounds__(WAVES * 64) void k_demit(const uint8_t* __restrict__ in, uint64_t n, uint64_t blk, uint64_t blk_inv,
-                                                      uint64_t npieces_total, const DfRec* __restrict__ rec,
+                                                      uint64_t npieces_total, const DfRec* __restrict__ rec, const uint32_t* __restrict__ wbase,
                                                       const uint32_t* __restrict__ spill, const unsigned long long* __restrict__ off,
                                                       Flags* __restrict__ flags, uint32_t stgb, uint32_t jbytes, uint32_t maxcnt,
                                                       uint8_t* __restrict__ out, const uint32_t* __restrict__ side, DfDev D) {
@@ -572,9 +622,18 @@
   const uint64_t nwi = (nunits + 63) / 64;
   const uint64_t oend_all = flags->total_len;
   const uint64_t one_piece_blocks = (uint64_t)__builtin_amdgcn_readfirstlane(blk == (uint64_t)PIECE ? 1 : 0);
-  struct Operands { uint32_t w[NW]; uint32_t wp; uint4 r; uint64_t off0; uint32_t sp0; uint4 r1; uint64_t off1; uint32_t sp1; };
+  struct Operands { uint32_t w[NW]; uint32_t wp; uint2 r; uint32_t wb; uint64_t off0; uint32_t sp0; };
   auto request = [&](uint64_t it_, Operands& o) {
     if (it_ >= nwi) return;
+    {
+      const uint64_t itu = ((uint64_t)(uint32_t)__builtin_amdgcn_readfirstlane((int)(uint32_t)(it_ >> 32)) << 32) | (uint32_t)__builtin_amdgcn_readfirstlane((int)(uint32_t)it_);
+      const uint64_t pf = itu * (HALF ? 32u : 64u);
+      const uint64_t mf = __umul64hi(pf, blk_inv) + pf * one_piece_blocks;
+      uint32_t vw, vm;
+      asm("v_mov_b32 %0, %1" : "=v"(vw) : "s"((uint32_t)(pf / DF_WBASE_PIECES)));
+      asm("v_mov_b32 %0, %1" : "=v"(vm) : "s"((uint32_t)mf));
+      o.wb = wbase[vw]; o.off0 = off[vm]; o.sp0 = spill[vm];
+    }
     const uint64_t u = it_ * 64 + lane;
     const bool ok = u < nunits;
     const uint64_t pc = HALF ? u >> 1 : u;
@@ -595,14 +654,7 @@
       }
     } else load_piece(in, n, ustart, o.w);
     o.wp = *reinterpret_cast<const uint32_t*>(ok && ustart >= 4 ? in + ustart - 4 : reinterpret_cast<const uint8_t*>(D.img));
-    const uint64_t pc0 = ok ? pc : 0;
-    const uint64_t m0 = __umul64hi(pc0, blk_inv) + pc0 * one_piece_blocks;
-    o.r = *reinterpret_cast<const uint4*>(rec + pc0);
-    o.off0 = off[m0]; o.sp0 = spill[m0];
-    {
-      const uint64_t pc1 = pc0 + 1 < npieces_total ? pc0 + 1 : pc0, m1 = __umul64hi(pc1, blk_inv) + pc1 * one_piece_blocks;
-      o.r1 = *reinterpret_cast<const uint4*>(rec + pc1); o.off1 = off[m1]; o.sp1 = spill[m1];
-    }
+    o.r = *reinterpret_cast<const uint2*>(rec + (ok ? pc : 0));
   };
   Operands nx, cur;
   request((uint64_t)blockIdx.x * WAVES + wave, nx);
@@ -624,29 +676,27 @@
     uint32_t w[NW];
 #pragma unroll
     for (int i = 0; i < NW; ++i) w[i] = cur.w[i];
-    const uint32_t wp = cur.wp, lenA = cur.r.z & 0xFFFFu;
-    const uint32_t kA = HALF ? (half ? (cur.r.w >> 8) & 0xFFu : cur.r.w & 0xFFu) : cur.r.w & 0xFFu, kB = HALF ? 0u : (cur.r.w >> 8) & 0xFFu;
-    const uint32_t hh = HALF ? (half ? cur.r.x >> 16 : cur.r.x & 0xFFFFu) : cur.r.x;
-    uint64_t ostart = valid ? cur.off0 + cur.r.y + ((cur.r.z & DFREC_OWN) ? cur.sp0 : 0u) + (half ? lenA : 0u) : oend_all;
-    const uint64_t onext63 = piece + 1 < npieces_total ? cur.off1 + cur.r1.y + ((cur.r1.z & DFREC_OWN) ? cur.sp1 : 0u) : oend_all;
-    uint64_t oend;
-    {
-      const uint32_t lo = (uint32_t)__builtin_amdgcn_update_dpp(0, (int)(uint32_t)ostart, 0x130, 0xF, 0xF, false);
-      const uint32_t hi = (uint32_t)__builtin_amdgcn_update_dpp(0, (int)(uint32_t)(ostart >> 32), 0x130, 0xF, 0xF, false);
-      oend = lane == 63 ? onext63 : ((uint64_t)hi << 32) | lo;
-      if (!valid) oend = oend_all;
-    }
+    const uint32_t wp = cur.wp;
+    const DfRec rc{cur.r.x, cur.r.y};
+    const bool hole = valid && dfrec_hole(rc);
+    const uint32_t len = hole ? dfrec_hole_len(rc) : dfrec_len(rc), lenA = hole ? len : dfrec_lenA(rc);
+    const uint32_t kA = HALF ? (half ? dfrec_kB(rc) : dfrec_kA(rc)) : dfrec_kA(rc), kB = HALF ? 0u : dfrec_kB(rc);
+    const uint32_t hA = HALF ? (half ? dfrec_middle(rc) : dfrec_start(rc)) : dfrec_start(rc), hB = dfrec_middle(rc);
+    const uint32_t ulen = valid ? (HALF ? (half ? len - lenA : lenA) : len) : 0u;
+    const uint32_t before = wave_scan_incl(ulen) - ulen;
+    const uint64_t obase = cur.off0 + (cur.wb & ~DFREC_OWN) + ((cur.wb & DFREC_OWN) ? cur.sp0 : 0u);
+    const uint64_t ostart = valid ? obase + before : oend_all, oend = valid ? ostart + ulen : oend_all;
     const unsigned long long vmask = __ballot(valid);
     const uint32_t nvalid = (uint32_t)__popcll(vmask);
     uint32_t first = 0;
     bool taken = false;
     unsigned long long t2 = stamp();
     tk[0] += t2 - t0;
-    if (valid && (cur.r.w & DFREC_HOLE) == DFREC_HOLE && half == 0) {
-      const uint32_t cntE = cur.r.w & 0x7FFFu;
-      uint64_t u = (cur.r.w & 0x8000u) ? piece * PIECE - K : piece * PIECE, o = ostart;
+    if (hole && half == 0) {
+      const uint32_t cntE = dfrec_hole_entries(rc), e0 = dfrec_hole_side(rc);
+      uint64_t u = dfrec_hole_first(rc) ? piece * PIECE - K : piece * PIECE, o = ostart;
       for (uint32_t x = 0; x < cntE; ++x) {
-        const uint32_t ee = side[cur.r.x + x], pc = (ee >> 1) & 0x3FFFFFFFu;
+        const uint32_t ee = side[e0 + x], pc = (ee >> 1) & 0x3FFFFFFFu;
         if (ee & 1u) out[o++] = in[u];
         if (pc < D.sl_npc) for (uint32_t b = D.sl_pcoff[pc]; b < D.sl_pcoff[pc + 1]; ++b) out[o++] = D.sl_pcpool[b];
         if (!(ee >> 31)) ++u;
@@ -656,7 +706,6 @@
       if (first == 0) request(it + (uint64_t)gridDim.x * WAVES, nx);
       const uint64_t gs = wave_read64(ostart, first);
       const uint64_t abase = gs & ~15ull;
-      const bool hole = (cur.r.w & DFREC_HOLE) == DFREC_HOLE;
       const bool fits = valid && lane >= first && (oend - abase) <= (uint64_t)stgb && plen == NB && !hole;
       const unsigned long long fm = __ballot(fits) >> first;
       uint32_t cnt = fm == ~0ull ? 64u - first : (uint32_t)__builtin_ctzll(~fm);
@@ -665,7 +714,7 @@
         if (lane == first && hole) {
         } else
         if (lane == first) {
-          uint32_t h = hh & 0xFFFFu;
+          uint32_t h = hA;
           uint64_t o = ostart;
           for (int t = 0; t < plen; ++t) {
             const int ts = t - K;
@@ -690,16 +739,16 @@
       if (active && jfit) {
         uint32_t oA = o0, pA = jarea + incl - need;
         if constexpr (HALF) {
-          if (D.wide) { if constexpr (K == 1) piece_dfwalk1cw_k1(w, wp, hh & 0xFFFFu, oA, pA); else piece_dfwalk1cw_k2(w, wp, hh & 0xFFFFu, oA, pA); }
-          else { if constexpr (K == 1) piece_dfwalk1c_k1(w, wp, hh & 0xFFFFu, oA, pA); else piece_dfwalk1c_k2(w, wp, hh & 0xFFFFu, oA, pA); }
+          if (D.wide) { if constexpr (K == 1) piece_dfwalk1cw_k1(w, wp, hA, oA, pA); else piece_dfwalk1cw_k2(w, wp, hA, oA, pA); }
+          else { if constexpr (K == 1) piece_dfwalk1c_k1(w, wp, hA, oA, pA); else piece_dfwalk1c_k2(w, wp, hA, oA, pA); }
         } else {
           uint32_t oB = o0 + lenA, pB = pA + 4u * kA;
           if (D.wide) {
-            if constexpr (K == 1) piece_dfwalk2cw_k1(w, wp, hh & 0xFFFFu, oA, hh >> 16, oB, pA, pB);
-            else piece_dfwalk2cw_k2(w, wp, hh & 0xFFFFu, oA, hh >> 16, oB, pA, pB);
+            if constexpr (K == 1) piece_dfwalk2cw_k1(w, wp, hA, oA, hB, oB, pA, pB);
+            else piece_dfwalk2cw_k2(w, wp, hA, oA, hB, oB, pA, pB);
           } else {
-            if constexpr (K == 1) piece_dfwalk2c_k1(w, wp, hh & 0xFFFFu, oA, hh >> 16, oB, pA, pB);
-            else piece_dfwalk2c_k2(w, wp, hh & 0xFFFFu, oA, hh >> 16, oB, pA, pB);
+            if constexpr (K == 1) piece_dfwalk2c_k1(w, wp, hA, oA, hB, oB, pA, pB);
+            else piece_dfwalk2c_k2(w, wp, hA, oA, hB, oB, pA, pB);
           }
         }
       }
@@ -708,7 +757,7 @@
         if (!inplace && lane == first) atomicAdd(&flags->emit_ovf, cnt);
         if (active) {
           for (int ch = 0; ch < (HALF ? 1 : 2); ++ch) {
-            uint32_t h = ch ? hh >> 16 : hh & 0xFFFFu;
+            uint32_t h = ch ? hB : hA;
             uint64_t o = (uint64_t)(o0 - stga) + (ch ? lenA : 0u);
             for (int t = ch * HALF_BYTES; t < (ch + 1) * HALF_BYTES; ++t) {
               const int ts = t - K;
diff --git a/kleenexlang_amd/csrc/engine/kx_engine.hip b/kleenexlang_amd/csrc/engine/kx_engine.hip
--- a/kleenexlang_amd/csrc/engine/kx_engine.hip
+++ b/kleenexlang_amd/csrc/engine/kx_engine.hip
@@ -1854,7 +1854,7 @@
   unsigned long long *off, *wsum, *woff;
   Flags hflags{}; uint64_t head_len = 0; bool have_end = false; uint64_t out_len = 0; uint32_t init_shift = 0, init_leaf = 0;
   uint32_t df_qin = 0;
-  bool df = false; DfRec* dfrec = nullptr; uint32_t *df_own = nullptr, *df_spill = nullptr, *side = nullptr; uint32_t side_cap = 0; std::vector<uint8_t> df_tail; uint64_t df_body = 0;
+  bool df = false; DfRec* dfrec = nullptr; uint32_t *df_wbase = nullptr, *df_own = nullptr, *df_spill = nullptr, *side = nullptr; uint32_t side_cap = 0; std::vector<uint8_t> df_tail; uint64_t df_body = 0;
   uint32_t endId() const {
     if (!df) return st->stateOf(hflags.end_state);
     const uint32_t i = st->df.indexOf(hflags.end_state);
@@ -1990,6 +1990,7 @@
         }
       }
       if (S.df_why.empty() && !acceptable(S.df)) S.df_why = "too many contexts that need more lookahead";
+      if (S.df_why.empty() && !dfRecFits(S.df.img.data(), S.df.nP + 2, C)) S.df_why = "the table image outgrows the piece record's fields";
       S.has_df = S.df_why.empty();
     }
     S.df_pc_off.assign(apoff.begin(), apoff.begin() + npc); S.df_pc_len.resize(npc);
@@ -2409,7 +2410,7 @@
   if (c.segment_bytes % PIECE || c.segment_bytes > MAX_SEG || c.block_threads % 64 || c.block_threads > 1024 ||
       (c.block_threads & (c.block_threads - 1)))
     return setErr(KX_E_ARG, "segment_bytes: multiple of 64 (≤ 256 KiB); block_threads: power of two in [64, 1024]");
-  if (c.delayed_form > 2 || c.delay > 2 || c.merge_window > 64 || c.inline_consts > 2 || c.job_stride > 2 || c.emit_half > 2 || c.emit_inplace > 2 ||
+  if (c.delayed_form > 2 || c.delay > 2 || c.merge_window > DF_MERGE_WINDOW_MAX || c.inline_consts > 2 || c.job_stride > 2 || c.emit_half > 2 || c.emit_inplace > 2 ||
       c.act_lanes > 2 || c.df_backoff > 1 || (c.emit_waves && c.emit_waves != 4 && c.emit_waves != 8 && c.emit_waves != 12 && c.emit_waves != 16) ||
       c.batch_actions > 2 || c.reserved[0] || c.reserved[1] || c.reserved[2])
     return setErr(KX_E_ARG, "kx_config: a field is outside its range (include/kxhip.h)");
@@ -2487,8 +2488,8 @@
   bool anydf = false;
   for (auto& s : p->stages) anydf = anydf || s.has_df;
   if (anydf) {
-    rc = setLds((const void*)(k_dforward<512, 8, 4, false>), lds_cap); rc = rc ? rc : setLds((const void*)(k_dforward<512, 4, 4, false>), lds_cap);
-    rc = rc ? rc : setLds((const void*)(k_dforward<512, 8, 4, true>), lds_cap); rc = rc ? rc : setLds((const void*)(k_dforward<512, 4, 4, true>), lds_cap); rc = rc ? rc : setLds((const void*)k_dhead, lds_cap);
+    rc = setLds((const void*)(k_dforward<512, 16, 4, false>), lds_cap); rc = rc ? rc : setLds((const void*)(k_dforward<512, 8, 4, false>), lds_cap);
+    rc = rc ? rc : setLds((const void*)(k_dforward<512, 16, 4, true>), lds_cap); rc = rc ? rc : setLds((const void*)(k_dforward<512, 8, 4, true>), lds_cap); rc = rc ? rc : setLds((const void*)k_dhead, lds_cap);
     rc = rc ? rc : setLds((const void*)k_dmap<false>, 152 * 1024); rc = rc ? rc : setLds((const void*)k_dmap<true>, 152 * 1024);
 #define KX_DEMIT_ATTR(WV) (rc = rc ? rc : setLds((const void*)k_demit<WV, 1>, lds_cap), rc = rc ? rc : setLds((const void*)k_demit<WV, 2>, lds_cap))
     KX_DEMIT_ATTR(16); KX_DEMIT_ATTR(12); KX_DEMIT_ATTR(8); KX_DEMIT_ATTR(4);
@@ -2557,7 +2558,7 @@
   if (s->df && s->st->df_given_up) s->df = false;
   if (s->df && s->st->df_skip) { s->df = false; --s->st->df_skip; }
   s->side_cap = s->df && s->st->D.sl_on ? (uint32_t)(n / 8 < (1u << 22) ? (n / 8 > (1u << 18) ? n / 8 : (1u << 18)) : (1u << 22)) : 0u;
-  size_t need = 4096 + (s->df ? (n / PIECE + 16) * sizeof(DfRec) + (size_t)s->nseg * 8 + 512 + (size_t)s->side_cap * 4 + 256 : 0) + (size_t)s->nseg * (8 + 2) + (n / HALF + 32) * 2 + sizeof(Flags) +
+  size_t need = 4096 + (s->df ? (n / PIECE + 16) * sizeof(DfRec) + (n / PIECE / DF_WBASE_PIECES + 8) * 4 + 256 + (size_t)s->nseg * 8 + 512 + (size_t)s->side_cap * 4 + 256 : 0) + (size_t)s->nseg * (8 + 2) + (n / HALF + 32) * 2 + sizeof(Flags) +
                 (size_t)s->nblk * ((size_t)s->Lc * 5 + 3 + 4 + 8 + 2 + 4) + (size_t)s->ngroups * 16 + KX_MAX_LEAVES + 64 +
                 (n / PIECE + 16) * 8 + 256 * 32;
   int rc = A.reserve(need);
@@ -2572,7 +2573,7 @@
   s->d_map = A.take<uint8_t>(KX_MAX_LEAVES); s->d_const = A.take<uint32_t>(4);
   s->prec = A.take<PieceRec>(n / PIECE + 16);
   s->merge_piece = A.take<uint16_t>(s->nblk); s->ctot = A.take<uint32_t>(s->nblk);
-  if (s->df) { s->dfrec = A.take<DfRec>(n / PIECE + 16); s->df_own = A.take<uint32_t>(s->nblk); s->df_spill = A.take<uint32_t>(s->nblk); s->side = s->side_cap ? A.take<uint32_t>(s->side_cap) : nullptr; }
+  if (s->df) { s->dfrec = A.take<DfRec>(n / PIECE + 16); s->df_wbase = A.take<uint32_t>(n / PIECE / DF_WBASE_PIECES + 8); s->df_own = A.take<uint32_t>(s->nblk); s->df_spill = A.take<uint32_t>(s->nblk); s->side = s->side_cap ? A.take<uint32_t>(s->side_cap) : nullptr; }
   if (!p->have_events) {
     for (auto& e : p->ev) if (hipEventCreate(&e) != hipSuccess) { p->arenas.push_back(s->arena); delete s; return setErr(KX_E_HIP, "hipEventCreate failed"); }
     p->have_events = true;
@@ -2689,10 +2690,10 @@
     constexpr int DBT = 512;
     const size_t dimg = (((size_t)S.D.words + 3) & ~(size_t)3) * 4;
     auto launchForward = [&](bool slow) {
-#define KX_LAUNCH_DFWD(ST, SL) hipLaunchKernelGGL((k_dforward<DBT, ST, 4, SL>), dim3((s->nseg + DBT - 1) / DBT), dim3(DBT), dimg + (size_t)DBT * ST * 16, s->stream, s->in, s->n, s->seg, s->nseg, \
-                                                  s->is_first, s->seg_pos, s->seg_state, s->dfrec, s->df_own, s->df_spill, s->flags, s->side, s->side_cap, s->is_last, S.D)
-      if (2 * (dimg + (size_t)DBT * 8 * 16) <= 160 * 1024) { if (slow) KX_LAUNCH_DFWD(8, true); else KX_LAUNCH_DFWD(8, false); }
-      else { if (slow) KX_LAUNCH_DFWD(4, true); else KX_LAUNCH_DFWD(4, false); }
+#define KX_LAUNCH_DFWD(ST, SL) hipLaunchKernelGGL((k_dforward<DBT, ST, 4, SL>), dim3((s->nseg + DBT - 1) / DBT), dim3(DBT), dimg + (size_t)DBT * ST * sizeof(DfRec), s->stream, s->in, s->n, s->seg, s->nseg, \
+                                                  s->is_first, s->seg_pos, s->seg_state, s->dfrec, s->df_wbase, s->df_own, s->df_spill, s->flags, s->side, s->side_cap, s->is_last, S.D)
+      if (2 * (dimg + (size_t)DBT * 16 * sizeof(DfRec)) <= 160 * 1024) { if (slow) KX_LAUNCH_DFWD(16, true); else KX_LAUNCH_DFWD(16, false); }
+      else { if (slow) KX_LAUNCH_DFWD(8, true); else KX_LAUNCH_DFWD(8, false); }
 #undef KX_LAUNCH_DFWD
     };
     launchForward(S.df_slow_armed);
@@ -2751,7 +2752,7 @@
       const bool timing = p->cfg.collect_timing;
       if (timing) HIPCHECK(hipEventRecord(p->ev[0], s->stream));
       hipLaunchKernelGGL(k_dhead, dim3(1), dim3(64), (size_t)S.D.words * 4 + 16, s->stream, s->in, s->n, s->seg, s->head_len, hin,
-                         s->dfrec, s->df_own, s->df_spill, s->flags, S.D);
+                         s->dfrec, s->df_wbase, s->df_own, s->df_spill, s->flags, S.D);
       if (timing) HIPCHECK(hipEventRecord(p->ev[1], s->stream));
       HIPCHECK(hipGetLastError());
       int rc = readFlags(s);
@@ -2966,11 +2967,11 @@
     const uint64_t ppb = s->seg / PIECE, blk_inv = ppb > 1 ? ~0ull / ppb + 1 : 0;
     if (timing) HIPCHECK(hipEventRecord(p->ev[0], s->stream));
 #define KX_LAUNCH_DEMIT(WV, KK)                                                                                                    \
-  hipLaunchKernelGGL((k_demit<WV, KK>), dim3(grid), dim3(WV * 64), elds, s->stream, s->in, s->n, s->seg, blk_inv, npieces, s->dfrec, \
+  hipLaunchKernelGGL((k_demit<WV, KK>), dim3(grid), dim3(WV * 64), elds, s->stream, s->in, s->n, s->seg, blk_inv, npieces, s->dfrec, s->df_wbase, \
                      s->df_spill, s->off, s->flags, (uint32_t)stgb, (uint32_t)jbytes, maxcnt, (uint8_t*)d_out, s->side, S.D)
 #define KX_LAUNCH_DEMIT_K(WV) do { if (S.df.K == 1) KX_LAUNCH_DEMIT(WV, 1); else KX_LAUNCH_DEMIT(WV, 2); } while (0)
 #define KX_LAUNCH_DEMIT_H(WV, KK)                                                                                                    \
-  hipLaunchKernelGGL((k_demit<WV, KK, true>), dim3(grid), dim3(WV * 64), elds, s->stream, s->in, s->n, s->seg, blk_inv, npieces, s->dfrec, \
+  hipLaunchKernelGGL((k_demit<WV, KK, true>), dim3(grid), dim3(WV * 64), elds, s->stream, s->in, s->n, s->seg, blk_inv, npieces, s->dfrec, s->df_wbase, \
                      s->df_spill, s->off, s->flags, (uint32_t)stgb, (uint32_t)jbytes, maxcnt, (uint8_t*)d_out, s->side, S.D)
     if (halfmode) {
       if (W == 16) { if (S.df.K == 1) KX_LAUNCH_DEMIT_H(16, 1); else KX_LAUNCH_DEMIT_H(16, 2); }
```

New measurement: 1124 (median of 6 runs). +1.7%, better.
